# piotrmwojcik/GI-GS

Measured on AMD Instinct MI355X. Metric: train-step renders/sec (fwd+bwd, G-buffer+indirect) at 800x800; PSNR vs the CPU oracle, higher is better.
Workload: dtype f32; 1 GPU; C2 (configs[1] TensoIR lego stand-in): 300k surface Gaussians, 800x800, SH deg 2, GI step=16 start=8 delta=0.0625; P=300000, N=640000, M=9, hip_graphs=on, fused_glue=on, gi_march=proj, rasterizer=whole step = 2 hand-captured hipGraphs (fwd, bwd), asynchronous binning

## Files before the change

### gi-gs_amd/csrc/api.hip

```cpp
#include <cstdarg>
#include <cstdio>
#include <cstdlib>
#include <cstring>
#include <map>
#include <algorithm>
#include <new>
#include <mutex>
#include <vector>

#include "../../include/gigs_hip.h"
#include "gigs_common.h"

namespace {

thread_local char g_err[512] = "";

int fail(int code, const char* fmt, ...) {
  va_list ap;
  va_start(ap, fmt);
  vsnprintf(g_err, sizeof(g_err), fmt, ap);
  va_end(ap);
  return code;
}

// ... 110 lines not shown
  hipEventCreate(&e);
  return e;
}

struct StageScope {
  hipStream_t s;
  int stage;
  bool on;
  hipEvent_t a, b;
  StageScope(int stage_, hipStream_t s_) : s(s_), stage(stage_), on(false) {
    std::lock_guard<std::mutex> lk(g_prof_mu);
    if (!g_prof_on) return;
    on = true;
    a = prof_event();
    b = prof_event();
    hipEventRecord(a, s);
  }
  ~StageScope() {
    if (!on) return;
    hipEventRecord(b, s);
    std::lock_guard<std::mutex> lk(g_prof_mu);
    g_prof_recs.push_back({stage, a, b});
  }
};

}

namespace gigs {
const Options& default_options() {
  static const Options o = options_from_env();
  return o;
}
const Ctx& default_ctx() {
  static const Ctx c = {default_options(), 0u, nullptr, nullptr, 0, nullptr, nullptr};
  return c;
}
}

extern "C" {
__attribute__((visibility("hidden"))) const gigs::Options* gigs_internal_options(const gigs_ctx* ctx) { return &ctx_of(ctx).opt; }
__attribute__((visibility("hidden"))) int gigs_internal_fail(int code, const char* msg) { return fail(code, "%s", msg); }
__attribute__((visibility("hidden"))) void gigs_internal_stage_begin(int stage, void* stream, void** token) {
  *token = new StageScope(stage, (hipStream_t)stream);
}
__attribute__((visibility("hidden"))) void gigs_internal_stage_end(void* token) { delete (StageScope*)token; }
}

extern "C" {

const char* gigs_last_error(void) { return g_err; }
const char* gigs_build_arch(void) { return "gfx950"; }

size_t gigs_required_geom(int P) {
  if (P < 0) { fail(GIGS_ERR_INVALID, "P < 0"); return 0; }
  return gigs::required_bytes<gigs::GeomState>((size_t)P, scan_size_cached(P));
}
size_t gigs_required_image(int width, int height) {
  const size_t N = (size_t)width * height;
  const size_t T = (size_t)((width + GIGS_BLOCK_X - 1) / GIGS_BLOCK_X) * ((height + GIGS_BLOCK_Y - 1) / GIGS_BLOCK_Y);
  return gigs::required_bytes<gigs::ImageState>(N, T);
}
size_t gigs_required_binning(int R) {
  if (R < 0) { fail(GIGS_ERR_INVALID, "R < 0"); return 0; }
  return gigs::required_bytes<gigs::BinningState>((size_t)R, sort_size_cached(R));
}

long long gigs_geom_offset(int P, int which) {
// ... 47 lines not shown
  if (!ctx) return fail(GIGS_ERR_INVALID, "gigs_ctx_set_options: the default context is immutable, create one");
  if (!in || in->struct_bytes < (int)sizeof(gigs_options)) return fail(GIGS_ERR_INVALID, "gigs_ctx_set_options: set struct_bytes = sizeof(gigs_options)");
  if (in->gi_march != 0 && in->gi_march != 4) return fail(GIGS_ERR_INVALID, "gi_march must be 0 (exact) or 4 (proj)");
  if (in->gi_tile_log2w < 0 || in->gi_tile_log2w > 6) return fail(GIGS_ERR_INVALID, "gi_tile_log2w must be 0..6");
  if (in->long_lists < -1 || in->long_lists > 1) return fail(GIGS_ERR_INVALID, "long_lists must be -1, 0 or 1");
  if (in->bucket_target < 256 || in->bucket_max_mean < 0 || in->bin_bands < 0 || in->bin_bands > 64)
    return fail(GIGS_ERR_INVALID, "bucket_target >= 256, bucket_max_mean >= 0, 0 <= bin_bands <= 64");
  if (in->spec_max8 < 0 || in->spec_max16 < in->spec_max8) return fail(GIGS_ERR_INVALID, "0 <= spec_max8 <= spec_max16");
  if (in->shade_lds_floats < 0 || in->shade_bwd_blocks < 0) return fail(GIGS_ERR_INVALID, "shade_lds_floats, shade_bwd_blocks >= 0");
  if (in->spec_sparse_permille < 0 || in->spec_sparse_permille > 1000) return fail(GIGS_ERR_INVALID, "0 <= spec_sparse_permille <= 1000");
  gigs::Options& o = reinterpret_cast<gigs::Ctx*>(ctx)->opt;
  o.binning_legacy = in->binning_legacy != 0; o.bucket_max_mean = in->bucket_max_mean; o.long_lists = in->long_lists;
  o.bucket_target = in->bucket_target; o.bin_bands = in->bin_bands; o.blend_cull = in->blend_cull != 0; o.pre_bwd_sh_skip = in->pre_bwd_sh_skip != 0;
  o.gi_march = in->gi_march; o.gi_cert = in->gi_cert != 0; o.gi_interleave = in->gi_interleave != 0;
  o.gi_tile_log2w = in->gi_tile_log2w; o.gi_zero_rays = in->gi_zero_rays != 0; o.spec_max8 = in->spec_max8;
  o.spec_max16 = in->spec_max16; o.shade_lds_floats = in->shade_lds_floats; o.shade_bwd_blocks = in->shade_bwd_blocks;
  o.shade_bwd_rows = in->shade_bwd_rows != 0; o.spec_sparse = in->spec_sparse != 0; o.spec_sparse_permille = in->spec_sparse_permille;
  return 0;
}
int gigs_ctx_set_reuse_binning(gigs_ctx* ctx, int on) {
  if (!ctx) return fail(GIGS_ERR_INVALID, "gigs_ctx_set_reuse_binning: the default context is immutable, create one");
  reinterpret_cast<gigs::Ctx*>(ctx)->reuse_binning = on != 0;
  return 0;
}
int gigs_ctx_set_split_sh(gigs_ctx* ctx, const float* sh_rest) {
  if (!ctx) return fail(GIGS_ERR_INVALID, "gigs_ctx_set_split_sh: the default context is immutable, create one");
  reinterpret_cast<gigs::Ctx*>(ctx)->sh_rest = sh_rest;
  return 0;
}
int gigs_ctx_set_materials_only(gigs_ctx* ctx, void* violations) {
  if (!ctx) return fail(GIGS_ERR_INVALID, "gigs_ctx_set_materials_only: the default context is immutable, create one");
  reinterpret_cast<gigs::Ctx*>(ctx)->materials_only = reinterpret_cast<unsigned*>(violations);
  return 0;
}
int gigs_ctx_set_blend_begin_event(gigs_ctx* ctx, void* hip_event) {
  if (!ctx) return fail(GIGS_ERR_INVALID, "gigs_ctx_set_blend_begin_event: the default context is immutable, create one");
  reinterpret_cast<gigs::Ctx*>(ctx)->blend_begin_event = hip_event;
  return 0;
}

__global__ void __launch_bounds__(64) stream_delay_kernel(unsigned ticks) {
  const unsigned long long t0 = wall_clock64();
  while (wall_clock64() - t0 < (unsigned long long)ticks) __builtin_amdgcn_s_sleep(8);
}

int gigs_stream_delay(unsigned nanoseconds, void* stream) {
  if (nanoseconds == 0) return 0;
  const unsigned ns = nanoseconds > 1000000u ? 1000000u : nanoseconds;
  hipLaunchKernelGGL(stream_delay_kernel, dim3(1), dim3(64), 0, (hipStream_t)stream, (ns + 9u) / 10u);
  return hipGetLastError() == hipSuccess ? 0 : gigs_internal_fail(GIGS_ERR_HIP, "stream_delay: launch failed");
}

int gigs_ctx_set_async_binning(gigs_ctx* ctx, int r_capacity, unsigned* device_counters) {
  if (!ctx) return fail(GIGS_ERR_INVALID, "gigs_ctx_set_async_binning: the default context is immutable, create one");
  gigs::Ctx* c = reinterpret_cast<gigs::Ctx*>(ctx);
  c->async_capacity = r_capacity > 0 ? (unsigned)r_capacity : 0u;
  c->async_counters = r_capacity > 0 ? device_counters : nullptr;
  return 0;
}

void gigs_profile_begin(void) {
  std::lock_guard<std::mutex> lk(g_prof_mu);
  for (auto& r : g_prof_recs) { g_prof_pool.push_back(r.a); g_prof_pool.push_back(r.b); }
  g_prof_recs.clear();
  g_prof_on = true;
}
// ... 32 lines not shown
                 const float* rotations, const float* cov3D_precomp, const float* viewmatrix,
                 const float* projmatrix, const float* cam_pos, float tan_fovx, float tan_fovy,
                 int prefiltered, int argmax_depth, int inference, float* out_color,
                 float* out_opacity, float* out_depth, float* out_normal, float* out_normal_view,
                 float* out_pos, float* out_albedo, float* out_roughness, float* out_metallic,
                 int* radii, int debug, void* stream) {
  (void)prefiltered;
  hipStream_t s = (hipStream_t)stream;
  const gigs::Ctx& cx = ctx_of(ctx);
  const gigs::Options& opt = cx.opt;
  if (P < 0 || width <= 0 || height <= 0) return fail(GIGS_ERR_INVALID, "bad P / image size");
  if (P == 0) return 0;
  if (!geometryBuffer || !binningBuffer || !imageBuffer) return fail(GIGS_ERR_INVALID, "null allocation callback");
  if (!means3D || !opacities || !normal || !albedo || !roughness || !metallic || !viewmatrix ||
      !projmatrix || !cam_pos || !background)
    return fail(GIGS_ERR_INVALID, "null required input");
  if (!shs && !colors_precomp) return fail(GIGS_ERR_INVALID, "provide SHs or precomputed colors");
  if (!cov3D_precomp && (!scales || !rotations)) return fail(GIGS_ERR_INVALID, "provide scales+rotations or cov3D_precomp");
  if (!colors_precomp && (M <= 0 || (D + 1) * (D + 1) > M || D > 3)) return fail(GIGS_ERR_INVALID, "SH degree %d needs (D+1)^2 <= M=%d, D <= 3", D, M);

  gigs::FwdArgs a;
  a.P = P; a.D = D; a.M = M; a.W = width; a.H = height;
  a.gx = (width + GIGS_BLOCK_X - 1) / GIGS_BLOCK_X;
  a.gy = (height + GIGS_BLOCK_Y - 1) / GIGS_BLOCK_Y;
  a.focal_y = height / (2.0f * tan_fovy);
  a.focal_x = width / (2.0f * tan_fovx);
  a.tan_fovx = tan_fovx; a.tan_fovy = tan_fovy; a.scale_modifier = scale_modifier;
  a.means3D = means3D; a.shs = shs; a.colors_precomp = colors_precomp; a.opacities = opacities;
  a.normal = normal; a.albedo = albedo; a.roughness = roughness; a.metallic = metallic;
  a.scales = scales; a.rotations = rotations; a.cov3D_precomp = cov3D_precomp;
  a.viewmatrix = viewmatrix; a.projmatrix = projmatrix; a.cam_pos = cam_pos; a.background = background;
  a.argmax_depth = argmax_depth; a.inference = inference;
  a.shs_rest = (shs && !colors_precomp && M > 1) ? cx.sh_rest : nullptr;

  const size_t scan_sz = scan_size_cached(P);
  const size_t geom_bytes = gigs::required_bytes<gigs::GeomState>((size_t)P, scan_sz);
  char* geom_chunk = geometryBuffer(geom_bytes, geom_user);
  if (!geom_chunk) return fail(GIGS_ERR_ALLOC, "geometry buffer allocation of %zu bytes failed", geom_bytes);
  gigs::GeomState geom = gigs::GeomState::fromChunk(geom_chunk, (size_t)P, scan_sz);
  if (radii == nullptr) radii = geom.internal_radii;

  const size_t N = (size_t)width * height, T = (size_t)a.gx * a.gy;
  const size_t img_bytes = gigs::required_bytes<gigs::ImageState>(N, T);
  char* img_chunk = imageBuffer(img_bytes, image_user);
  if (!img_chunk) return fail(GIGS_ERR_ALLOC, "image buffer allocation of %zu bytes failed", img_bytes);
  gigs::ImageState img = gigs::ImageState::fromChunk(img_chunk, N, T);

  {
    StageScope sc(kPreprocess, s);
    gigs::launch_preprocess_fwd(a, geom, radii, s);
  }
  STAGE_CHECK("preprocess");
  int num_rendered = 0;
  gigs::BinningState bin;
  const unsigned async_cap = cx.async_capacity;
  const bool bucket = !opt.binning_legacy && T <= (size_t)gigs::kBinMaxTiles;
  if (async_cap > 0 && !bucket) return fail(GIGS_ERR_INVALID, "asynchronous binning needs the tile-bucketed path (options.binning_legacy = 0, <= %d tiles)", gigs::kBinMaxTiles);
  auto long_lists = [&](size_t est_mean) {
    if (opt.long_lists >= 0) return opt.long_lists == 1;
    return est_mean > (size_t)opt.bucket_max_mean;
  };
  bool dense = false;
  if (cx.reuse_binning) {
    if (async_cap == 0 || !bucket)
      return fail(GIGS_ERR_INVALID, "reuse_binning needs asynchronous binning (gigs_ctx_set_async_binning) on the tile-bucketed path");
    num_rendered = (int)async_cap;
// ... 74 lines not shown
  }
  STAGE_CHECK("identifyTileRanges");
  }
  if (void* ev = cx.blend_begin_event) HIP_TRY(hipEventRecord((hipEvent_t)ev, s));
  {
    StageScope sc(kBlendFwd, s);
    gigs::launch_blend_fwd(a, geom, bin, img, out_color, out_opacity, out_depth, out_normal,
                           out_normal_view, out_pos, out_albedo, out_roughness, out_metallic, opt.blend_cull,
                           (size_t)num_rendered, s, cx.reuse_binning != 0);
  }
  STAGE_CHECK("render");
  return num_rendered;
}

namespace {
struct LiteChunk { char* base; size_t bytes; };
char* lite_chunk_alloc(size_t n, void* user) {
  LiteChunk* c = static_cast<LiteChunk*>(user);
  return n <= c->bytes ? c->base : nullptr;
}
}

int gigs_lite_forward(gigs_ctx* ctx, gigs_alloc_fn geometryBuffer, void* geom_user, gigs_alloc_fn binningBuffer, void* binning_user,
                      gigs_alloc_fn imageBuffer, void* image_user, int P, int D, int M, const float* background, int width,
                      int height, const float* means3D, const float* shs, const float* colors_precomp, const float* opacities,
                      const float* scales, float scale_modifier, const float* rotations, const float* cov3D_precomp,
                      const float* viewmatrix, const float* projmatrix, const float* cam_pos, float tan_fovx, float tan_fovy,
                      int prefiltered, int argmax_depth, float* out_color, float* out_opacity, float* out_depth, int* radii,
                      int debug, void* stream) {
  if (P < 0 || width <= 0 || height <= 0) return fail(GIGS_ERR_INVALID, "bad P / image size");
  if (P == 0) return 0;
  if (!geometryBuffer || !binningBuffer || !imageBuffer) return fail(GIGS_ERR_INVALID, "null allocation callback");
  if (!out_color || !out_opacity || !out_depth) return fail(GIGS_ERR_INVALID, "null output");
  const size_t N = (size_t)width * height;
  const size_t geom_bytes = gigs_required_geom(P), img_bytes = gigs_required_image(width, height);
  const size_t geom_extra = 8 * (size_t)P * sizeof(float) + gigs::kAlign, img_extra = 14 * N * sizeof(float) + gigs::kAlign;
  char* gb = geometryBuffer(geom_bytes + geom_extra, geom_user);
  char* ib = imageBuffer(img_bytes + img_extra, image_user);
  if (!gb || !ib) return fail(GIGS_ERR_ALLOC, "lite_forward: scratch allocation failed");
  auto up = [](char* p) { return reinterpret_cast<char*>((reinterpret_cast<uintptr_t>(p) + gigs::kAlign - 1) & ~(uintptr_t)(gigs::kAlign - 1)); };
  float* zeros = reinterpret_cast<float*>(up(gb + geom_bytes));
  float* spare = reinterpret_cast<float*>(up(ib + img_bytes));
  gigs::launch_zero_words(reinterpret_cast<uint32_t*>(zeros), 8 * (size_t)P, (hipStream_t)stream);
  LiteChunk gc{gb, geom_bytes}, ic{ib, img_bytes};
  return gigs_forward(ctx, lite_chunk_alloc, &gc, binningBuffer, binning_user, lite_chunk_alloc, &ic, P, D, M, background, width, height,
                      means3D, shs, colors_precomp, opacities, zeros, zeros + 3 * (size_t)P, zeros + 6 * (size_t)P,
                      zeros + 7 * (size_t)P, scales, scale_modifier, rotations, cov3D_precomp, viewmatrix, projmatrix, cam_pos,
                      tan_fovx, tan_fovy, prefiltered, argmax_depth, 0, out_color, out_opacity, out_depth, spare, spare + 3 * N,
                      spare + 6 * N, spare + 9 * N, spare + 12 * N, spare + 13 * N, radii, debug, stream);
}

int gigs_backward(gigs_ctx* ctx, int P, int D, int M, int R, const float* background, int width, int height,
                  const float* means3D, const float* shs, const float* colors_precomp,
                  const float* normal, const float* albedo, const float* roughness,
                  const float* metallic, const float* scales, const float* rotations,
                  const float* cov3D_precomp, const float* viewmatrix, const float* projmatrix,
                  const float* cam_pos, const int* radii, float scale_modifier, float tan_fovx,
                  float tan_fovy, char* geom_buffer, char* binning_buffer, char* image_buffer,
                  const float* dL_dpix_depth, const float* dL_dpix, const float* dL_dpix_opacity,
                  const float* dL_dpix_normal, const float* dL_dpix_albedo,
                  const float* dL_dpix_roughness, const float* dL_dpix_metallic, float* dL_dmean2D,
                  float* dL_dconic, float* dL_ddepth, float* dL_dopacity, float* dL_dnormal,
                  float* dL_dalbedo, float* dL_droughness, float* dL_dmetallic, float* dL_dcolor,
                  float* dL_dmean3D, float* dL_dcov3D, float* dL_dsh, float* dL_dscale,
                  float* dL_drot, int debug, void* stream) {
  (void)normal; (void)albedo; (void)roughness; (void)metallic;
  hipStream_t s = (hipStream_t)stream;
  if (P == 0) return 0;
  if (P < 0 || R < 0 || width <= 0 || height <= 0) return fail(GIGS_ERR_INVALID, "bad sizes");
  if (!geom_buffer || !binning_buffer || !image_buffer) return fail(GIGS_ERR_INVALID, "null scratch buffer");
  unsigned* const materials_only = ctx_of(ctx).materials_only;
  if (ctx_of(ctx).sh_rest && shs && M > 1 && !materials_only)
    return fail(GIGS_ERR_INVALID, "a split-SH forward (gigs_ctx_set_split_sh) has a materials-only backward only");
  if (!dL_dmean2D || !dL_dalbedo || !dL_droughness || !dL_dmetallic)
    return fail(GIGS_ERR_INVALID, "null gradient output");
  if (!materials_only && (!dL_dopacity || !dL_dnormal || !dL_dcolor || !dL_dmean3D || !dL_dcov3D || !dL_dscale || !dL_drot ||
                          (shs && !dL_dsh)))
    return fail(GIGS_ERR_INVALID, "null gradient output");

  gigs::BwdArgs a;
  a.P = P; a.D = D; a.M = M; a.R = R; a.W = width; a.H = height;
  a.gx = (width + GIGS_BLOCK_X - 1) / GIGS_BLOCK_X;
  a.gy = (height + GIGS_BLOCK_Y - 1) / GIGS_BLOCK_Y;
  a.focal_y = height / (2.0f * tan_fovy);
  a.focal_x = width / (2.0f * tan_fovx);
  a.tan_fovx = tan_fovx; a.tan_fovy = tan_fovy; a.scale_modifier = scale_modifier;
  a.means3D = means3D; a.shs = shs; a.colors_precomp = colors_precomp; a.scales = scales;
  a.rotations = rotations; a.cov3D_precomp = cov3D_precomp; a.viewmatrix = viewmatrix;
  a.projmatrix = projmatrix; a.cam_pos = cam_pos; a.background = background;
  a.dL_dpix_depth = dL_dpix_depth; a.dL_dpix = dL_dpix; a.dL_dpix_opacity = dL_dpix_opacity;
  a.dL_dpix_normal = dL_dpix_normal; a.dL_dpix_albedo = dL_dpix_albedo;
  a.dL_dpix_roughness = dL_dpix_roughness; a.dL_dpix_metallic = dL_dpix_metallic;
  a.dL_dmean2D = dL_dmean2D; a.dL_dconic = dL_dconic; a.dL_ddepth = dL_ddepth;
  a.dL_dopacity = dL_dopacity; a.dL_dnormal = dL_dnormal; a.dL_dalbedo = dL_dalbedo;
  a.dL_droughness = dL_droughness; a.dL_dmetallic = dL_dmetallic; a.dL_dcolor = dL_dcolor;
  a.dL_dmean3D = dL_dmean3D; a.dL_dcov3D = dL_dcov3D; a.dL_dsh = dL_dsh; a.dL_dscale = dL_dscale;
  a.dL_drot = dL_drot;

  const size_t N = (size_t)width * height, T = (size_t)a.gx * a.gy;
  char* gp = geom_buffer;
  gigs::GeomState geom = gigs::GeomState::fromChunk(gp, (size_t)P, scan_size_cached(P));
  char* bp = binning_buffer;
  gigs::BinningState bin = gigs::BinningState::fromChunk(bp, (size_t)R, 0);
  char* ip = image_buffer;
  gigs::ImageState img = gigs::ImageState::fromChunk(ip, N, T);
  a.radii = radii ? radii : geom.internal_radii;

  {
// ... 3 lines not shown
  STAGE_CHECK("render backward");
  {
    StageScope sc(kPreprocessBwd, s);
    gigs::launch_preprocess_bwd(a, geom, ctx_of(ctx).opt.pre_bwd_sh_skip, s, materials_only);
  }
  STAGE_CHECK("preprocess backward");
  return 0;
}

int gigs_mark_visible(int P, const float* means3D, const float* viewmatrix,
                      const float* projmatrix, uint8_t* present, void* stream) {
  (void)projmatrix;
  if (P == 0) return 0;
  if (P < 0 || !means3D || !viewmatrix || !present) return fail(GIGS_ERR_INVALID, "bad argument");
  gigs::launch_mark_visible(P, means3D, viewmatrix, present, (hipStream_t)stream);
  HIP_TRY(hipGetLastError());
  return 0;
}

int gigs_depth_to_normal(int width, int height, float focal_x, float focal_y,
                         const float* viewmatrix, const float* depth, float* normal,
                         float* depth_pos, void* stream) {
  if (width <= 0 || height <= 0 || !viewmatrix || !depth || !normal || !depth_pos)
    return fail(GIGS_ERR_INVALID, "bad argument");
  StageScope sc(kDepthToNormal, (hipStream_t)stream);
  gigs::launch_depth_to_normal(width, height, focal_x, focal_y, viewmatrix, depth, normal, depth_pos, (hipStream_t)stream);
  HIP_TRY(hipGetLastError());
  return 0;
}

int gigs_derive_normal(int width, int height, float focal_x, float focal_y, const float* viewmatrix, const float* depth,
                       float sigma_color, float sigma_x, float sigma_y, float* normal_from_depth, float* depth_pos_filter,
                       void* stream) {
  if (width <= 1 || height <= 1 || !viewmatrix || !depth || !normal_from_depth || !depth_pos_filter)
    return fail(GIGS_ERR_INVALID, "derive_normal: bad argument (images must be larger than 1x1)");
  StageScope sc(kDepthToNormal, (hipStream_t)stream);
  gigs::launch_derive_normal_fused(width, height, focal_x, focal_y, viewmatrix, sigma_color, sigma_x, sigma_y, depth,
                                   normal_from_depth, depth_pos_filter, (hipStream_t)stream);
  HIP_TRY(hipGetLastError());
  return 0;
}

size_t gigs_gi_scratch_bytes(int width, int height) {
  if (width <= 0 || height <= 0) return 0;
  return gigs::gi_scratch_bytes(width, height);
}

int gigs_ssao_ex(gigs_ctx* ctx, int width, int height, float focal_x, float focal_y, float radius, float bias,
                 float thick, float delta, int step, int start, const float* normal_view,
                 const float* pos, float* occlusion, void* scratch, void* stream) {
  if (width <= 0 || height <= 0 || !normal_view || !pos || !occlusion) return fail(GIGS_ERR_INVALID, "bad argument");
  if (width >= (1 << 15) || height >= (1 << 15)) return fail(GIGS_ERR_INVALID, "image side above 32767 pixels");
  StageScope sc(kSsao, (hipStream_t)stream);
  const int rc = gigs::launch_ssao(ctx_of(ctx).opt, width, height, focal_x, focal_y, radius, bias, thick, delta, step, start,
                                   normal_view, pos, occlusion, scratch, (hipStream_t)stream);
  if (rc == -1) return fail(GIGS_ERR_INVALID, "delta=%g gives an unbounded or oversized ray set", (double)delta);
  if (rc) return fail(GIGS_ERR_HIP, "ray table upload failed");
  HIP_TRY(hipGetLastError());
  return 0;
}
int gigs_ssao(int width, int height, float focal_x, float focal_y, float radius, float bias,
              float thick, float delta, int step, int start, const float* normal_view,
              const float* pos, float* occlusion, void* stream) {
  return gigs_ssao_ex(nullptr, width, height, focal_x, focal_y, radius, bias, thick, delta, step, start, normal_view, pos,
                      occlusion, nullptr, stream);
}

int gigs_ssr_ex(gigs_ctx* ctx, int width, int height, float focal_x, float focal_y, float radius, float bias,
                float thick, float delta, int step, int start, const float* normal_view,
                const float* pos, const float* rgb, const float* albedo, const float* roughness,
                const float* metallic, const float* F0, float* color, float* abd, void* scratch, void* stream) {
  if (width <= 0 || height <= 0 || !normal_view || !pos || !rgb || !albedo || !metallic || !F0 || !color || !abd)
    return fail(GIGS_ERR_INVALID, "bad argument");
  if (width >= (1 << 15) || height >= (1 << 15)) return fail(GIGS_ERR_INVALID, "image side above 32767 pixels");
  StageScope sc(kSsr, (hipStream_t)stream);
  const int rc = gigs::launch_ssr(ctx_of(ctx).opt, width, height, focal_x, focal_y, radius, bias, thick, delta, step, start,
                                  normal_view, pos, rgb, albedo, roughness, metallic, F0, color, abd, scratch,
                                  (hipStream_t)stream);
  if (rc == -1) return fail(GIGS_ERR_INVALID, "delta=%g gives an unbounded or oversized ray set", (double)delta);
  if (rc) return fail(GIGS_ERR_HIP, "ray table upload failed");
  HIP_TRY(hipGetLastError());
  return 0;
}
int gigs_ssr_multi(gigs_ctx* ctx, int n_lights, int width, int height, float focal_x, float focal_y, float radius, float bias,
                   float thick, float delta, int step, int start, const float* normal_view, const float* pos, const float* rgb,
                   const float* albedo, const float* roughness, const float* metallic, const float* F0, float* color,
                   float* abd, void* scratch, void* stream) {
  if (n_lights < 1 || n_lights > GIGS_MAX_LIGHTS)
    return fail(GIGS_ERR_INVALID, "ssr_multi: n_lights=%d outside 1..%d", n_lights, GIGS_MAX_LIGHTS);
  if (width <= 0 || height <= 0 || !normal_view || !pos || !rgb || !albedo || !metallic || !F0 || !color || !abd)
    return fail(GIGS_ERR_INVALID, "bad argument");
  if (width >= (1 << 15) || height >= (1 << 15)) return fail(GIGS_ERR_INVALID, "image side above 32767 pixels");
  StageScope sc(kSsr, (hipStream_t)stream);
  (void)roughness;
  const int rc = gigs::launch_ssr_multi(ctx_of(ctx).opt, n_lights, width, height, focal_x, focal_y, radius, bias, thick, delta,
                                        step, start, normal_view, pos, rgb, albedo, metallic, F0, color, abd, scratch,
                                        (hipStream_t)stream);
  if (rc == -1) return fail(GIGS_ERR_INVALID, "delta=%g gives an unbounded or oversized ray set", (double)delta);
  if (rc) return fail(GIGS_ERR_HIP, "ray table upload failed");
  HIP_TRY(hipGetLastError());
  return 0;
}
int gigs_ssr_hits(gigs_ctx* ctx, int width, int height, float focal_x, float focal_y, float radius, float bias, float thick,
                  float delta, int step, int start, const float* normal_view, const float* pos, const float* rgb,
                  const float* albedo, const float* roughness, const float* metallic, const float* F0, float* color, float* abd,
                  int mode, unsigned* counts, const unsigned* offsets, void* entries, unsigned capacity, void* scratch,
                  void* stream) {
  if (width <= 0 || height <= 0 || !normal_view || !pos || !rgb || !albedo || !metallic || !F0 || !color || !abd)
    return fail(GIGS_ERR_INVALID, "bad argument");
  if (width >= (1 << 15) || height >= (1 << 15)) return fail(GIGS_ERR_INVALID, "image side above 32767 pixels");
  if ((mode != 1 && mode != 2) || (mode == 1 && !counts) || (mode == 2 && (!offsets || (!entries && capacity > 0))))
    return fail(GIGS_ERR_INVALID, "ssr_hits: mode 1 needs counts, mode 2 offsets and entries");
  StageScope sc(kSsr, (hipStream_t)stream);
  const int rc = gigs::launch_ssr(ctx_of(ctx).opt, width, height, focal_x, focal_y, radius, bias, thick, delta, step, start,
                                  normal_view, pos, rgb, albedo, roughness, metallic, F0, color, abd, scratch,
                                  (hipStream_t)stream, mode, counts, offsets, entries, capacity);
  if (rc == -1) return fail(GIGS_ERR_INVALID, "delta=%g gives an unbounded or oversized ray set", (double)delta);
  if (rc == -3) return fail(GIGS_ERR_INVALID, "ssr_hits: the hit list is recorded by the default march only (gi_march = proj, start < step)");
  if (rc) return fail(GIGS_ERR_HIP, "ray table upload failed");
  HIP_TRY(hipGetLastError());
  return 0;
}

int gigs_ssr_apply(int width, int height, float delta, const unsigned* offsets, const void* entries, const float* normal_view,
                   const float* pos, const float* rgb, const float* albedo, const float* metallic, const float* F0,
                   float* color, float* abd, void* stream) {
  if (width <= 0 || height <= 0 || !offsets || !normal_view || !pos || !rgb || !albedo || !metallic || !F0 || !color || !abd)
    return fail(GIGS_ERR_INVALID, "bad argument");
  StageScope sc(kSsr, (hipStream_t)stream);
  const int rc = gigs::launch_ssr_apply(width, height, delta, offsets, entries, normal_view, pos, rgb, albedo, metallic, F0, color,
                                        abd, (hipStream_t)stream);
  if (rc == -1) return fail(GIGS_ERR_INVALID, "delta=%g gives an unbounded or oversized ray set", (double)delta);
  if (rc) return fail(GIGS_ERR_HIP, "ray table upload failed");
  HIP_TRY(hipGetLastError());
  return 0;
}

size_t gigs_ssr_apply_multi_scratch_bytes(int n_lights, int width, int height) {
  if (n_lights < 1 || n_lights > GIGS_MAX_LIGHTS || width <= 0 || height <= 0) return 0;
  return gigs::ssr_apply_multi_scratch_bytes(n_lights, width, height);
}
int gigs_ssr_apply_multi(int n_lights, int width, int height, float delta, const unsigned* offsets, const void* entries,
                         const float* normal_view, const float* pos, const float* rgb, const float* albedo,
                         const float* metallic, const float* F0, float* color, float* abd, void* scratch, void* stream) {
  if (n_lights < 1 || n_lights > GIGS_MAX_LIGHTS)
    return fail(GIGS_ERR_INVALID, "ssr_apply_multi: n_lights=%d outside 1..%d", n_lights, GIGS_MAX_LIGHTS);
  if (width <= 0 || height <= 0 || !offsets || !normal_view || !pos || !rgb || !albedo || !metallic || !F0 || !color || !abd)
    return fail(GIGS_ERR_INVALID, "bad argument");
  if ((size_t)offsets % 16 != 0 || (size_t)scratch % 16 != 0)
// ... 65 lines not shown
```

### gi-gs_amd/csrc/blend.hip

```cpp
#include <cstdlib>
#include "gigs_common.h"

namespace gigs {

typedef float f32x2 __attribute__((ext_vector_type(2)));

__device__ __forceinline__ unsigned long long ballot64(bool p) { return __builtin_amdgcn_ballot_w64(p); }

constexpr int kLongTile = 2048;

template <int kCtrl, int kRowMask = 0xf, int kBankMask = 0xf>
__device__ __forceinline__ float dpp_mov0(float v) {
  return __int_as_float(__builtin_amdgcn_update_dpp(0, __float_as_int(v), kCtrl, kRowMask, kBankMask, false));
}
template <int N>
__device__ __forceinline__ void wave_sum_n(float* v);
template <>
__device__ __forceinline__ void wave_sum_n<1>(float* v) {
  asm("s_nop 4\n\t"
      "v_add_f32_dpp %0, %0, %0 quad_perm:[1,0,3,2] row_mask:0xf bank_mask:0xf bound_ctrl:1\n\t"
      "s_nop 1\n\t"
      "v_add_f32_dpp %0, %0, %0 quad_perm:[2,3,0,1] row_mask:0xf bank_mask:0xf bound_ctrl:1\n\t"
      "s_nop 1\n\t"
      "v_add_f32_dpp %0, %0, %0 row_ror:4 row_mask:0xf bank_mask:0xf bound_ctrl:1\n\t"
// ... 257 lines not shown
        const float4 r4 = sw[4 * 64 + bit];
        const f32x2 w2 = {weight, weight};
        C01 += f32x2{r2.x, r2.y} * w2; C2P0 += f32x2{r2.z, r2.w} * w2;
        N01 += f32x2{r3.x, r3.y} * w2; N2P1 += f32x2{r3.z, r3.w} * w2;
        A01 += f32x2{r4.x, r4.y} * w2; A2P2 += f32x2{r4.z, r4.w} * w2;
        RM += f32x2{r0.z, r0.w} * w2;
        O += weight;
        if (argmax_depth) {
          if (weight > max_weight) {
            e0 = r2.w; e1 = r3.w; e2 = r4.w;
            max_weight = weight;
          }
        }
        T = test_T;
        last_contributor = (uint32_t)(base + bit + 1);
      }
    }
    wave_done = ballot64(!done) == 0ull;
    __builtin_amdgcn_wave_barrier();
    if (valid) hit[base + lane] = (uint8_t)((hits >> lane) & 1ull);
  }
  for (int i = base + lane; i < n; i += 64) hit[i] = 0;

  const float C0 = C01.x, C1 = C01.y, C2 = C2P0.x, P0 = C2P0.y, N0 = N01.x, N1 = N01.y, N2 = N2P1.x, P1 = N2P1.y;
  const float A0 = A01.x, A1 = A01.y, A2 = A2P2.x, P2 = A2P2.y, Rr = RM.x, Mm = RM.y;
  if (inside) {
    const size_t HW = (size_t)H * W;
    final_T[pix_id] = T;
    n_contrib[pix_id] = last_contributor;
    const v3 nv = normalize3(xform_vec_4x3({N0, N1, N2}, viewmatrix));
    o.normal_view[pix_id] = nv.x;
    o.normal_view[HW + pix_id] = nv.y;
    o.normal_view[2 * HW + pix_id] = nv.z;
    o.color[pix_id] = C0 + T * bg_color[0];
    o.color[HW + pix_id] = C1 + T * bg_color[1];
    o.color[2 * HW + pix_id] = C2 + T * bg_color[2];
    o.normal[pix_id] = N0; o.normal[HW + pix_id] = N1; o.normal[2 * HW + pix_id] = N2;
    o.albedo[pix_id] = A0; o.albedo[HW + pix_id] = A1; o.albedo[2 * HW + pix_id] = A2;
    o.roughness[pix_id] = inference ? (Rr + T) : Rr;
    o.metallic[pix_id] = Mm;
    if ((double)O > 1e-6) {
      o.depth[pix_id] = argmax_depth ? e2 : P2 / O;
      o.pos[pix_id] = argmax_depth ? e0 : P0 / O;
      o.pos[HW + pix_id] = argmax_depth ? e1 : P1 / O;
      o.pos[2 * HW + pix_id] = argmax_depth ? e2 : P2 / O;
    } else {
      o.depth[pix_id] = 0.0f;
      o.pos[pix_id] = 0.0f;
      o.pos[HW + pix_id] = 0.0f;
      o.pos[2 * HW + pix_id] = 0.0f;
    }
    o.opacity[pix_id] = O;
  }
}

void launch_blend_fwd(const FwdArgs& a, const GeomState& g, const BinningState& b,
                      const ImageState& im, float* out_color, float* out_opacity,
                      float* out_depth, float* out_normal, float* out_normal_view, float* out_pos,
                      float* out_albedo, float* out_roughness, float* out_metallic, int cull, size_t hit_stride,
                      hipStream_t s, bool reused_lists) {
  BlendOut o{out_color, out_opacity, out_depth, out_normal, out_normal_view,
             out_pos, out_albedo, out_roughness, out_metallic};
  hipLaunchKernelGGL(blend_fwd_kernel, dim3(a.gx * a.gy), dim3(GIGS_TILE), 0, s, a.W, a.H, a.gx,
                     im.ranges, b.point_list, g.brec, a.viewmatrix, a.background, im.n_contrib,
                     im.final_T, o, a.argmax_depth, a.inference, b.hit_mask, hit_stride, cull, im.tile_order,
                     reused_lists ? (const uint32_t*)im.bin_counters : (const uint32_t*)nullptr,
                     make_uint2((unsigned)a.P, (unsigned)hit_stride));
}

struct BlendGradIn {
  const float *depth, *color, *opacity, *normal, *albedo, *roughness, *metallic;
};

__global__ void __launch_bounds__(GIGS_TILE)
blend_bwd_kernel(int W, int H, unsigned gx, const uint2* __restrict__ ranges,
                 const uint32_t* __restrict__ point_list, const float4* __restrict__ brec,
                 const float* __restrict__ bg_color, const float* __restrict__ final_Ts,
                 const uint32_t* __restrict__ n_contrib, BlendGradIn gi, float* __restrict__ grec,
                 const uint8_t* __restrict__ hit_mask, size_t hit_stride, const uint32_t* __restrict__ tile_order) {
  __shared__ float4 s_rec[4][3 * 64];
  __shared__ __align__(16) float s_sum[4][2][GIGS_GREC];

  const unsigned tile = tile_order[blockIdx.x];
  const unsigned ty = tile / gx, tx = tile - ty * gx;
  const int tid = threadIdx.x, wave = tid >> 6, lane = tid & 63;
// ... 224 lines not shown
```

### gi-gs_amd/csrc/gi.hip

```cpp
#include <cmath>
#include <cstdlib>
#include <cstring>
#include <mutex>
#include <type_traits>
#include <vector>

#include "gigs_common.h"
#include "pixel_ops.h"

namespace gigs {

constexpr float kPiF = 3.14159265358979323846f;

__device__ __forceinline__ v3 get_position(int x, int y, float cx, float cy, float fx, float fy,
                                           float depth) {
  const v3 dir = {((float)x - cx) / fx, ((float)y - cy) / fy, 1.0f};
  return dir * depth;
}

__global__ void __launch_bounds__(256)
depth_to_normal_kernel(int W, int H, float fx, float fy, const float* __restrict__ vm,
                       const float* __restrict__ depth_map, float* __restrict__ normal_out,
                       float* __restrict__ depth_pos) {
  const int x = blockIdx.x * 16 + (threadIdx.x & 15);
// ... 1063 lines not shown
    }
#pragma unroll
    for (int o = 32; o > 0; o >>= 1) {
      mn = fminf(mn, __shfl_xor(mn, o));
      mx = fmaxf(mx, __shfl_xor(mx, o));
    }
  } else {
    mn = -__builtin_inff();
    mx = __builtin_inff();
  }
  if (threadIdx.x == 0) {
    float t_hi = (mx - ck.lo_k) / (1.0f - 0x1p-16f);
    t_hi = t_hi + fabsf(t_hi) * 0x1p-20f + 1e-30f;
    float t_lo = (mn - ck.hi_k) / (1.0f + 0x1p-16f);
    t_lo = t_lo - fabsf(t_lo) * 0x1p-20f - 1e-30f;
    if (!(mx == mx) || !(mn == mn)) { t_hi = __builtin_inff(); t_lo = -__builtin_inff(); }
    tab[(size_t)by * (bw + 1) + bx] = make_float2(t_lo, t_hi);
  }
}

constexpr int kCertMaxBytes = 40 * 1024;
static size_t cert_table_bytes(int W, int H, int sh) {
  return (size_t)(((W + (1 << sh) - 1) >> sh) + 2) * (((H + (1 << sh) - 1) >> sh) + 2) * sizeof(float2);
}
static int cert_shift_for(int W, int H) {
  for (int sh = 4; sh <= 6; sh++)
    if (cert_table_bytes(W, H, sh) <= (size_t)kCertMaxBytes) return sh;
  return 0;
}
size_t gi_scratch_bytes(int W, int H) {
  const int sh = cert_shift_for(W, H);
  return sh ? cert_table_bytes(W, H, sh) : 0;
}
static size_t prepare_cert(const Options& o, GiParams& p, int mode, const float* pos, void* scratch, hipStream_t s) {
  p.cert_shift = p.cert_w = p.cert_h = 0;
  p.cert_d0 = cert_consts(p.bias, p.thick).d0;
  if (!scratch || mode != 4 || !o.gi_cert) return 0;
  const int sh = cert_shift_for(p.W, p.H);
  if (!sh) return 0;
  p.cert_shift = sh;
  p.cert_w = (p.W + (1 << sh) - 1) >> sh;
  p.cert_h = (p.H + (1 << sh) - 1) >> sh;
  hipLaunchKernelGGL(gi_minmax_kernel, dim3(p.cert_w + 1, p.cert_h + 1), dim3(64), 0, s, p.W, p.H, sh, p.cert_w, p.cert_h,
                     cert_consts(p.bias, p.thick), pos + 2 * (size_t)p.H * p.W, (float2*)scratch);
  return cert_table_bytes(p.W, p.H, sh);
}

#ifndef GIGS_GI_DEFAULT_MODE
#define GIGS_GI_DEFAULT_MODE 4
#endif
static int gi_march_mode(const Options& o, int step, int start) {
  int mode = (o.gi_march == 0 || o.gi_march == 4) ? o.gi_march : GIGS_GI_DEFAULT_MODE;
  if (step - start > 64 - kGiGroup || step <= 0) mode = 0;
  return mode;
}
template <March kMarch> using MarchTag = std::integral_constant<March, kMarch>;
template <class F>
static void gi_dispatch_march(int mode, bool pow2, size_t cert, F&& f) {
  if (mode == 4) {
    if (cert) f(MarchTag<March::kProjCert>{}, cert);
    else f(MarchTag<March::kProj>{}, (size_t)0);
  } else {
    if (pow2) f(MarchTag<March::kExactPow2>{}, (size_t)0);
    else f(MarchTag<March::kExact>{}, (size_t)0);
  }
}
static dim3 gi_grid(const GiParams& p) {
  const int tw = 1 << p.tile_log2w, th = 64 >> p.tile_log2w;
  return dim3((p.W + tw - 1) / tw, (p.H + th - 1) / th);
}

int launch_ssao(const Options& o, int W, int H, float fx, float fy, float radius, float bias, float thick,
                float delta, int step, int start, const float* normal, const float* pos,
                float* occlusion, void* scratch, hipStream_t s) {
  RayTable t;
  const int rc = get_ray_table(delta, s, t);
  if (rc) return rc;
// ... 38 lines not shown
                           const float* F0, float* color, float* abd, void* scratch, hipStream_t s) {
  RayTable t;
  const int rc = get_ray_table(delta, s, t);
  if (rc) return rc;
  const size_t HW = (size_t)W * H, plane = 3 * HW;
  const dim3 grid((unsigned)((HW + 255) / 256));
  auto pass = [&](auto tag, int l0) {
    constexpr int kLights = decltype(tag)::value;
    const float* src = rgb + l0 * plane;
    if constexpr (kLights > 1) {
      hipLaunchKernelGGL(ssr_pack_kernel<kLights>, grid, dim3(256), 0, s, HW, src, (float4*)scratch);
      src = (const float*)scratch;
    }
    hipLaunchKernelGGL(ssr_apply_kernel<kLights>, grid, dim3(256), 0, s, W, H, t.nrays, t.dev, offsets, (const uint2*)entries,
                       normal, pos, src, albedo, metallic, F0, color + l0 * plane, abd + l0 * plane);
  };
  for (int l0 = 0; l0 < n_lights;) {
    const int n = n_lights - l0;
    int took;
    if (kSsrApplyLights == 8 && n >= 8) { pass(std::integral_constant<int, 8>{}, l0); took = 8; }
    else if (n >= 4) { pass(std::integral_constant<int, 4>{}, l0); took = 4; }
    else if (n == 3) { pass(std::integral_constant<int, 3>{}, l0); took = 3; }
    else if (n == 2) { pass(std::integral_constant<int, 2>{}, l0); took = 2; }
    else { pass(std::integral_constant<int, 1>{}, l0); took = 1; }
    l0 += took;
  }
  return 0;
}

int launch_ssr(const Options& o, int W, int H, float fx, float fy, float radius, float bias, float thick,
               float delta, int step, int start, const float* normal, const float* pos,
               const float* rgb, const float* albedo, const float* ,
               const float* metallic, const float* F0, float* color, float* abd, void* scratch, hipStream_t s,
               int hits_mode, unsigned* hit_counts, const unsigned* hit_offsets, void* hit_entries, unsigned hit_capacity) {
  RayTable t;
  const int rc = get_ray_table(delta, s, t);
  if (rc) return rc;
  bool pow2;
  GiParams p = make_params(o, W, H, fx, fy, radius, bias, thick, step, start, t,  true, pow2);
  if (W >= (1 << 15) || H >= (1 << 15)) return -2;
  const dim3 grid = gi_grid(p);
  const int mode = gi_march_mode(o, step, start);
  const size_t cert = (start < step) ? prepare_cert(o, p, mode, pos, scratch, s) : 0;
  const float2* tab = (const float2*)scratch;
  const SsrHits hits = {hit_counts, hit_offsets, (uint2*)hit_entries, hit_capacity};
  if (hits_mode != 0 && (mode != 4 || (hits_mode != 1 && hits_mode != 2) || !(start < step))) return -3;
  gi_dispatch_march(mode, pow2, cert, [&](auto m, size_t lds) {
    constexpr March kMarch = decltype(m)::value;
    auto launch = [&](auto kernel) {
      hipLaunchKernelGGL(kernel, grid, dim3(256), lds, s, p, t.dev, normal, pos, rgb, albedo, metallic, F0, color, abd, tab, hits);
    };
    if constexpr (march_is_proj(kMarch)) {
      if (hits_mode == 1) return launch(ssr_kernel<kMarch, 1>);
      if (hits_mode == 2) return launch(ssr_kernel<kMarch, 2>);
    }
    launch(ssr_kernel<kMarch>);
  });
  return 0;
}

template <int kLights>
static void launch_ssr_chunk(const GiParams& p, dim3 grid, int mode, bool pow2, size_t cert, const float2* tab,
                             const float4* rays, const float* normal, const float* pos, const float* rgb, const float* albedo,
                             const float* metallic, const float* F0, float* color, float* abd, hipStream_t s) {
  const SsrHits hits = {nullptr, nullptr, nullptr, 0};
  gi_dispatch_march(mode, pow2, cert, [&](auto m, size_t lds) {
    hipLaunchKernelGGL((ssr_kernel<decltype(m)::value, 0, kLights>), grid, dim3(256), lds, s, p, rays, normal, pos, rgb, albedo,
                       metallic, F0, color, abd, tab, hits);
  });
}

int launch_ssr_multi(const Options& o, int n_lights, int W, int H, float fx, float fy, float radius, float bias, float thick,
                     float delta, int step, int start, const float* normal, const float* pos, const float* rgb,
                     const float* albedo, const float* metallic, const float* F0, float* color, float* abd, void* scratch,
                     hipStream_t s) {
  RayTable t;
  const int rc = get_ray_table(delta, s, t);
  if (rc) return rc;
  bool pow2;
  GiParams p = make_params(o, W, H, fx, fy, radius, bias, thick, step, start, t,  true, pow2);
  if (W >= (1 << 15) || H >= (1 << 15)) return -2;
  const dim3 grid = gi_grid(p);
  const int mode = gi_march_mode(o, step, start);
  const size_t cert = (start < step) ? prepare_cert(o, p, mode, pos, scratch, s) : 0;
  const float2* tab = (const float2*)scratch;
  const size_t plane = (size_t)3 * W * H;
  for (int l0 = 0; l0 < n_lights; l0 += kSsrMaxLights) {
    const int n = min(kSsrMaxLights, n_lights - l0);
    const float* c_rgb = rgb + l0 * plane;
    float *c_color = color + l0 * plane, *c_abd = abd + l0 * plane;
    static_assert(kSsrMaxLights == 4, "one case per chunk size");
    switch (n) {
      case 1: launch_ssr_chunk<1>(p, grid, mode, pow2, cert, tab, t.dev, normal, pos, c_rgb, albedo, metallic, F0, c_color, c_abd, s); break;
      case 2: launch_ssr_chunk<2>(p, grid, mode, pow2, cert, tab, t.dev, normal, pos, c_rgb, albedo, metallic, F0, c_color, c_abd, s); break;
      case 3: launch_ssr_chunk<3>(p, grid, mode, pow2, cert, tab, t.dev, normal, pos, c_rgb, albedo, metallic, F0, c_color, c_abd, s); break;
      default: launch_ssr_chunk<4>(p, grid, mode, pow2, cert, tab, t.dev, normal, pos, c_rgb, albedo, metallic, F0, c_color, c_abd, s);
    }
  }
  return 0;
}

__device__ __forceinline__ bool load_taps(const float* __restrict__ src, int H, int W, int y, int x,
                                          float* v) {
  bool has_nan = false;
  int k = 0;
#pragma unroll
  for (int dy = -1; dy <= 1; dy++)
#pragma unroll
    for (int dx = -1; dx <= 1; dx++) {
      const int yy = y + dy, xx = x + dx;
      const float t = (yy < 0 || yy >= H || xx < 0 || xx >= W) ? 0.0f : src[(size_t)yy * W + xx];
      has_nan |= (t != t);
      v[k++] = t;
    }
  return has_nan;
}

// ... 79 lines not shown
#pragma unroll
      for (int c = 0; c < C; c++) num[c] += tap[c] * k;
      den += k;
    }
#pragma unroll
  for (int c = 0; c < C; c++) out[c * HW + (size_t)y * W + x] = num[c] / den;
}

void launch_bilateral3x3(int C, int H, int W, float sigma_color, float sx, float sy,
                         const float* in, float* out, hipStream_t s) {
  BilatK kk;
  auto k1d = [](float sigma, float* k) {
    float sum = 0;
    for (int i = 0; i < 3; i++) {
      const float xv = (float)(i - 1);
      k[i] = expf(-(xv * xv) / (2.0f * sigma * sigma));
      sum += k[i];
    }
    for (int i = 0; i < 3; i++) k[i] /= sum;
  };
  k1d(sy, kk.ky);
  k1d(sx, kk.kx);
  kk.color_scale = -0.5f / (sigma_color * sigma_color);
  dim3 grid((W + 63) / 64, (H + 3) / 4, 1);
  if (C == 1) hipLaunchKernelGGL(bilateral3x3_kernel<1>, grid, dim3(256), 0, s, H, W, kk, in, out);
  else if (C == 3) hipLaunchKernelGGL(bilateral3x3_kernel<3>, grid, dim3(256), 0, s, H, W, kk, in, out);
}

#ifndef GIGS_DN_H
#define GIGS_DN_H 4
#endif
constexpr int kDnW = 32, kDnH = GIGS_DN_H, kDnThreads = kDnW * kDnH;

__global__ void __launch_bounds__(kDnThreads)
derive_normal_fused_kernel(int W, int H, float fx, float fy, const float* __restrict__ vm, BilatK kk,
                           const float* __restrict__ depth_raw, float* __restrict__ normal_out,
                           float* __restrict__ pos_filter_out) {
  __shared__ float s_d[kDnH + 8][kDnW + 8];
  __shared__ float s_f[kDnH + 6][kDnW + 6];
  __shared__ float s_n[3][kDnH + 2][kDnW + 2];
  __shared__ float s_p[3][kDnH + 2][kDnW + 2];
  const int x0 = blockIdx.x * kDnW, y0 = blockIdx.y * kDnH;
  const size_t HW = (size_t)H * W;

  for (int i = threadIdx.x; i < (kDnH + 8) * (kDnW + 8); i += kDnThreads) {
    const int ty = i / (kDnW + 8), tx = i - ty * (kDnW + 8);
    const int gx = x0 - 4 + tx, gy = y0 - 4 + ty;
    s_d[ty][tx] = (gx < 0 || gx >= W || gy < 0 || gy >= H) ? 0.0f : depth_raw[(size_t)gy * W + gx];
  }
  __syncthreads();

  for (int i = threadIdx.x; i < (kDnH + 6) * (kDnW + 6); i += kDnThreads) {
    const int ty = i / (kDnW + 6), tx = i - ty * (kDnW + 6);
    const int gx = x0 - 3 + tx, gy = y0 - 3 + ty;
    float r = 0.0f;
    if (!(gx < 0 || gx >= W || gy < 0 || gy >= H)) {
      float v[9];
      bool has_nan = false;
      int k = 0;
#pragma unroll
      for (int dy = -1; dy <= 1; dy++)
#pragma unroll
        for (int dx = -1; dx <= 1; dx++) {
          const float t = s_d[ty + 1 + dy][tx + 1 + dx];
          has_nan |= (t != t);
          v[k++] = t;
        }
      r = has_nan ? __builtin_nanf("") : median9(v);
    }
    s_f[ty][tx] = r;
  }
  __syncthreads();

  for (int i = threadIdx.x; i < (kDnH + 2) * (kDnW + 2); i += kDnThreads) {
    const int ty = i / (kDnW + 2), tx = i - ty * (kDnW + 2);
    const int x = x0 - 1 + tx, y = y0 - 1 + ty;
    v3 nrm = {0.0f, 0.0f, 0.0f}, pos = {0.0f, 0.0f, 0.0f};
    if (!(x < 0 || x >= W || y < 0 || y >= H) && !(x <= 0 || x >= W - 1 || y <= 0 || y >= H - 1)) {
#define DP(dx, dy) s_f[ty + 2 + (dy)][tx + 2 + (dx)]
      const float depth_thresh = 0.01f;
      const float depth = DP(0, 0);
      const float cx = float(W) / 2.0f, cy = float(H) / 2.0f;
      pos = get_position(x, y, cx, cy, fx, fy, depth);
      bool ok = !(depth < depth_thresh);
      const int pad = 2;
      for (int dx = -pad; ok && dx < pad + 1; ++dx) {
        if (x + dx < 0 || x + dx > W - 1) { ok = false; break; }
        for (int dy = -pad; dy < pad + 1; ++dy) {
          if (y + dy < 0 || y + dy > H - 1) { ok = false; break; }
          if (DP(dx, dy) < depth_thresh) { ok = false; break; }
        }
      }
      if (ok) {
        const v3 pos_aa = get_position(x, y - 1, cx, cy, fx, fy, DP(0, -1));
        const v3 pos_bb = get_position(x + 1, y, cx, cy, fx, fy, DP(1, 0));
        const v3 pos_cc = get_position(x, y + 1, cx, cy, fx, fy, DP(0, 1));
        const v3 pos_dd = get_position(x - 1, y, cx, cy, fx, fy, DP(-1, 0));
        const v3 pos_ab = get_position(x + 1, y - 1, cx, cy, fx, fy, DP(1, -1));
        const v3 pos_bc = get_position(x + 1, y + 1, cx, cy, fx, fy, DP(1, 1));
        const v3 pos_cd = get_position(x - 1, y + 1, cx, cy, fx, fy, DP(-1, 1));
        const v3 pos_da = get_position(x - 1, y - 1, cx, cy, fx, fy, DP(-1, -1));
        const v3 edge_a = pos_da - pos_ab, edge_b = pos_ab - pos_bc, edge_c = pos_bc - pos_cd, edge_d = pos_cd - pos_da;
        const v3 edge_ac = pos_cc - pos_aa, edge_bd = pos_dd - pos_bb;
        const v3 edge_cdab = pos_ab - pos_cd, edge_bcad = pos_da - pos_bc;
        const v3 n1 = cross3(edge_a, edge_d), n2 = cross3(edge_d, edge_c), n3 = cross3(edge_c, edge_b);
        const v3 n4 = cross3(edge_b, edge_a), n5 = cross3(edge_ac, edge_bd), n6 = cross3(edge_bcad, edge_cdab);
        const v3 sum = normalize3(n1) + normalize3(n2) + normalize3(n3) + normalize3(n4) + normalize3(n5) + normalize3(n6);
        const float inv6 = 1.0f / 6.0f;
        const v3 normal = sum * inv6;
        nrm = {vm[0] * normal.x + vm[1] * normal.y + vm[2] * normal.z, vm[4] * normal.x + vm[5] * normal.y + vm[6] * normal.z,
               vm[8] * normal.x + vm[9] * normal.y + vm[10] * normal.z};
      }
#undef DP
    }
    s_n[0][ty][tx] = nrm.x; s_n[1][ty][tx] = nrm.y; s_n[2][ty][tx] = nrm.z;
    s_p[0][ty][tx] = pos.x; s_p[1][ty][tx] = pos.y; s_p[2][ty][tx] = pos.z;
  }
  __syncthreads();

  const int lx = threadIdx.x & (kDnW - 1), ly = threadIdx.x / kDnW;
  const int x = x0 + lx, y = y0 + ly;
  if (x >= W || y >= H) return;
  const size_t p = (size_t)y * W + x;
  {
    float ctr[3], num[3] = {0.0f, 0.0f, 0.0f};
#pragma unroll
    for (int c = 0; c < 3; c++) ctr[c] = s_n[c][ly + 1][lx + 1];
    float den = 0.0f;
#pragma unroll
    for (int dy = -1; dy <= 1; dy++)
#pragma unroll
      for (int dx = -1; dx <= 1; dx++) {
        int yy = y + dy, xx = x + dx;
        yy = yy < 0 ? -yy : (yy >= H ? 2 * H - 2 - yy : yy);
        xx = xx < 0 ? -xx : (xx >= W ? 2 * W - 2 - xx : xx);
        float tap[3], dist = 0.0f;
#pragma unroll
        for (int c = 0; c < 3; c++) {
          tap[c] = s_n[c][yy - y0 + 1][xx - x0 + 1];
          dist += fabsf(tap[c] - ctr[c]);
        }
        const float color_k = expf(kk.color_scale * (dist * dist));
        const float k = (kk.ky[dy + 1] * kk.kx[dx + 1]) * color_k;
#pragma unroll
        for (int c = 0; c < 3; c++) num[c] += tap[c] * k;
        den += k;
      }
#pragma unroll
    for (int c = 0; c < 3; c++) normal_out[c * HW + p] = num[c] / den;
  }
#pragma unroll
  for (int c = 0; c < 3; c++) {
    float v[9];
    bool has_nan = false;
    int k = 0;
#pragma unroll
    for (int dy = -1; dy <= 1; dy++)
#pragma unroll
      for (int dx = -1; dx <= 1; dx++) {
        const float t = s_p[c][ly + 1 + dy][lx + 1 + dx];
        has_nan |= (t != t);
        v[k++] = t;
      }
    pos_filter_out[c * HW + p] = has_nan ? __builtin_nanf("") : median9(v);
  }
}

void launch_derive_normal_fused(int W, int H, float fx, float fy, const float* viewmatrix, float sigma_color, float sx,
                                float sy, const float* depth_raw, float* normal_out, float* pos_filter_out, hipStream_t s) {
  BilatK kk;
  auto k1d = [](float sigma, float* k) {
    float sum = 0;
    for (int i = 0; i < 3; i++) {
      const float xv = (float)(i - 1);
      k[i] = expf(-(xv * xv) / (2.0f * sigma * sigma));
      sum += k[i];
    }
    for (int i = 0; i < 3; i++) k[i] /= sum;
  };
  k1d(sy, kk.ky);
  k1d(sx, kk.kx);
  kk.color_scale = -0.5f / (sigma_color * sigma_color);
  hipLaunchKernelGGL(derive_normal_fused_kernel, dim3((W + kDnW - 1) / kDnW, (H + kDnH - 1) / kDnH), dim3(kDnThreads), 0, s, W, H, fx,
                     fy, viewmatrix, kk, depth_raw, normal_out, pos_filter_out);
}

__global__ void __launch_bounds__(256)
selftest_div2_kernel(int n, const float* __restrict__ nx, const float* __restrict__ ny,
                     const float* __restrict__ d, float* __restrict__ out_fast, float* __restrict__ out_ref,
                     int* __restrict__ out_round) {
  const int i = blockIdx.x * 256 + threadIdx.x;
  if (i >= n) return;
  const float big = fmaxf(fmaxf(fabsf(nx[i]), fabsf(ny[i])), fabsf(d[i]));
  const float small = fminf(fabsf(nx[i]), fabsf(ny[i]));
  const f32x2 q = div2_exact(f32x2{nx[i], ny[i]}, d[i], big < 0x1p60f && small > 0x1p-60f);
  out_fast[2 * i] = q.x;
  out_fast[2 * i + 1] = q.y;
  out_ref[2 * i] = nx[i] / d[i];
  out_ref[2 * i + 1] = ny[i] / d[i];
  out_round[2 * i] = round_to_int(nx[i]);
  out_round[2 * i + 1] = f2i(roundf(nx[i]));
}

__global__ void __launch_bounds__(256) selftest_round_kernel(unsigned long long* __restrict__ bad) {
  unsigned long long local = 0;
  for (unsigned long long b = (unsigned long long)blockIdx.x * 256 + threadIdx.x; b < (1ull << 32);
       b += (unsigned long long)gridDim.x * 256) {
    const float t = __uint_as_float((unsigned)b);
    const int a = f2i(roundf(t)), r = round_pix(t);
    const bool same = a == r || (a < 0 && r < 0) || (a >= 32767 && r >= 32767);
    local += same ? 0 : 1;
  }
  if (local) atomicAdd(bad, local);
}

}

// ... 15 lines not shown
```

### gi-gs_amd/csrc/gigs_common.h

```cpp
#pragma once
#include <hip/hip_runtime.h>
#include <stdint.h>

#define GIGS_BLOCK_X 16
#define GIGS_BLOCK_Y 16
#define GIGS_TILE (GIGS_BLOCK_X * GIGS_BLOCK_Y)
#define GIGS_BREC_F4 5
#define GIGS_GREC 20

namespace gigs {

struct v3 { float x, y, z; };
struct v4 { float x, y, z, w; };

__device__ __forceinline__ v3 operator+(v3 a, v3 b) { return {a.x + b.x, a.y + b.y, a.z + b.z}; }
__device__ __forceinline__ v3 operator-(v3 a, v3 b) { return {a.x - b.x, a.y - b.y, a.z - b.z}; }
__device__ __forceinline__ v3 operator*(v3 a, float s) { return {a.x * s, a.y * s, a.z * s}; }
__device__ __forceinline__ float dot3(v3 a, v3 b) { return a.x * b.x + a.y * b.y + a.z * b.z; }
__device__ __forceinline__ v3 cross3(v3 a, v3 b) {
  return {a.y * b.z - a.z * b.y, a.z * b.x - a.x * b.z, a.x * b.y - a.y * b.x};
}
__device__ __forceinline__ v3 normalize3(v3 v) {
  float inv = 1.0f / sqrtf(dot3(v, v));
  return v * inv;
// ... 163 lines not shown
  char* p = nullptr;
  S::fromChunk(p, a...);
  return reinterpret_cast<size_t>(p) + kAlign;
}

struct Options {
  int binning_legacy;
  int bucket_max_mean;
  int long_lists;
  int bucket_target;
  int bin_bands;
  int blend_cull;
  int pre_bwd_sh_skip;
  int gi_march;
  int gi_cert;
  int gi_interleave;
  int gi_tile_log2w;
  int gi_zero_rays;
  int spec_max8, spec_max16;
  int shade_lds_floats;
  int shade_bwd_blocks;
  int shade_bwd_rows;
  int spec_sparse;
  int spec_sparse_permille;
};
struct Ctx {
  Options opt;
  unsigned async_capacity;
  unsigned* async_counters;
  void* blend_begin_event;
  int reuse_binning;
  unsigned* materials_only;
  const float* sh_rest;
};
const Options& default_options();
const Ctx& default_ctx();

struct FwdArgs {
  int P, D, M, W, H;
  unsigned gx, gy;
  float focal_x, focal_y, tan_fovx, tan_fovy, scale_modifier;
  const float *means3D, *shs, *colors_precomp, *opacities, *normal, *albedo, *roughness,
      *metallic, *scales, *rotations, *cov3D_precomp, *viewmatrix, *projmatrix, *cam_pos,
      *background;
  int argmax_depth, inference;
  const float* shs_rest;
};

void launch_preprocess_fwd(const FwdArgs& a, const GeomState& g, int* radii, hipStream_t s);
void launch_zero_words(uint32_t* p, size_t n, hipStream_t s);
void launch_bin_count(int P, const int* radii, unsigned gx, unsigned gy, const GeomState& g, const ImageState& img, hipStream_t s);
void launch_bin_prefix(int P, int T, unsigned capacity, const ImageState& img, unsigned* user_counters, hipStream_t s);
void launch_bin_scatter(int P, const int* radii, unsigned gx, unsigned gy, unsigned capacity, unsigned bands, const GeomState& g,
                        const BinningState& b, const ImageState& img, hipStream_t s);
int launch_bin_sort(int T, int P, bool long_lists, unsigned bucket_target, unsigned capacity, const BinningState& b, const ImageState& img,
                    hipStream_t s);
size_t long_space_bytes(size_t T, size_t R);
void launch_mark_visible(int P, const float* means3D, const float* viewmatrix, uint8_t* present,
                         hipStream_t s);
hipError_t scan_tiles(const GeomState& g, int P, hipStream_t s);
size_t scan_temp_bytes(int P);
size_t sort_temp_bytes(int R);
void launch_duplicate(int P, const int* radii, unsigned gx, unsigned gy, const GeomState& g,
                      const BinningState& b, hipStream_t s);
hipError_t sort_pairs(const BinningState& b, int R, int end_bit, hipStream_t s);
void launch_tile_ranges(int R, const BinningState& b, uint2* ranges, hipStream_t s);
void launch_tile_order(int T, const uint2* ranges, uint32_t* tile_order, hipStream_t s);
void launch_blend_fwd(const FwdArgs& a, const GeomState& g, const BinningState& b,
                      const ImageState& im, float* out_color, float* out_opacity,
                      float* out_depth, float* out_normal, float* out_normal_view, float* out_pos,
                      float* out_albedo, float* out_roughness, float* out_metallic, int cull, size_t hit_stride,
                      hipStream_t s, bool reused_lists = false);

struct BwdArgs {
  int P, D, M, R, W, H;
  unsigned gx, gy;
  float focal_x, focal_y, tan_fovx, tan_fovy, scale_modifier;
  const float *means3D, *shs, *colors_precomp, *scales, *rotations, *cov3D_precomp, *viewmatrix,
      *projmatrix, *cam_pos, *background;
  const int* radii;
  const float *dL_dpix_depth, *dL_dpix, *dL_dpix_opacity, *dL_dpix_normal, *dL_dpix_albedo,
      *dL_dpix_roughness, *dL_dpix_metallic;
  float *dL_dmean2D, *dL_dconic, *dL_ddepth, *dL_dopacity, *dL_dnormal, *dL_dalbedo,
      *dL_droughness, *dL_dmetallic, *dL_dcolor, *dL_dmean3D, *dL_dcov3D, *dL_dsh, *dL_dscale,
      *dL_drot;
};
void launch_blend_bwd(const BwdArgs& a, const GeomState& g, const BinningState& b,
                      const ImageState& im, hipStream_t s);
void launch_preprocess_bwd(const BwdArgs& a, const GeomState& g, int sh_skip, hipStream_t s, unsigned* materials_only = nullptr);

void launch_depth_to_normal(int W, int H, float fx, float fy, const float* viewmatrix,
                            const float* depth, float* normal, float* depth_pos, hipStream_t s);
int launch_ssao(const Options& o, int W, int H, float fx, float fy, float radius, float bias, float thick,
                float delta, int step, int start, const float* normal, const float* pos,
                float* occlusion, void* scratch, hipStream_t s);
size_t gi_scratch_bytes(int W, int H);
int launch_ssr(const Options& o, int W, int H, float fx, float fy, float radius, float bias, float thick,
               float delta, int step, int start, const float* normal, const float* pos,
               const float* rgb, const float* albedo, const float* roughness,
               const float* metallic, const float* F0, float* color, float* abd, void* scratch, hipStream_t s,
               int hits_mode = 0, unsigned* hit_counts = nullptr, const unsigned* hit_offsets = nullptr,
               void* hit_entries = nullptr, unsigned hit_capacity = 0);
int launch_ssr_multi(const Options& o, int n_lights, int W, int H, float fx, float fy, float radius, float bias, float thick,
                     float delta, int step, int start, const float* normal, const float* pos, const float* rgb,
                     const float* albedo, const float* metallic, const float* F0, float* color, float* abd, void* scratch,
                     hipStream_t s);
int launch_ssr_apply(int W, int H, float delta, const unsigned* offsets, const void* entries, const float* normal,
                     const float* pos, const float* rgb, const float* albedo, const float* metallic, const float* F0,
                     float* color, float* abd, hipStream_t s);
int launch_ssr_apply_multi(int n_lights, int W, int H, float delta, const unsigned* offsets, const void* entries,
                           const float* normal, const float* pos, const float* rgb, const float* albedo, const float* metallic,
                           const float* F0, float* color, float* abd, void* scratch, hipStream_t s);
size_t ssr_apply_multi_scratch_bytes(int n_lights, int W, int H);
void launch_median3x3(int C, int H, int W, const float* in, float* out, hipStream_t s);
void launch_median3x3_bwd(int C, int H, int W, const float* in, const float* gout, float* gin,
                          hipStream_t s);
void launch_bilateral3x3(int C, int H, int W, float sigma_color, float sx, float sy,
                         const float* in, float* out, hipStream_t s);
void launch_derive_normal_fused(int W, int H, float fx, float fy, const float* viewmatrix, float sigma_color, float sx,
                                float sy, const float* depth_raw, float* normal_out, float* pos_filter_out, hipStream_t s);

}
```

### gi-gs_amd/csrc/preprocess.hip

```cpp
#include "gigs_common.h"

namespace gigs {

#define SHC0 0.28209479177387814f
#define SHC1 0.4886025119029199f
#define SHC2_0 1.0925484305920792f
#define SHC2_1 -1.0925484305920792f
#define SHC2_2 0.31539156525252005f
#define SHC2_3 -1.0925484305920792f
#define SHC2_4 0.5462742152960396f
#define SHC3_0 -0.5900435899266435f
#define SHC3_1 2.890611442640554f
#define SHC3_2 -0.4570457994644658f
#define SHC3_3 0.3731763325901154f
#define SHC3_4 -0.4570457994644658f
#define SHC3_5 1.445305721320277f
#define SHC3_6 -0.5900435899266435f

constexpr int kPreBlock = 256;

__host__ __device__ __forceinline__ int sh_stride(int M) { return (3 * M) | 1; }

__device__ __forceinline__ void stage_sh(const float* __restrict__ shs, float* sh_lds,
                                         size_t first, int nG, int M) {
// ... 58 lines not shown

__device__ __forceinline__ Cov2D cov2d(v3 mean, float fx, float fy, float tan_fovx, float tan_fovy,
                                       const float* cov3D, const float* vm) {
  Cov2D s;
  v3 t = xform_point_4x3(mean, vm);
  s.limx = 1.3f * tan_fovx;
  s.limy = 1.3f * tan_fovy;
  s.txtz = t.x / t.z;
  s.tytz = t.y / t.z;
  t.x = fminf(s.limx, fmaxf(-s.limx, s.txtz)) * t.z;
  t.y = fminf(s.limy, fmaxf(-s.limy, s.tytz)) * t.z;
  s.t = t;
  m3 J = make_m3(fx / t.z, 0.0f, -(fx * t.x) / (t.z * t.z), 0.0f, fy / t.z,
                 -(fy * t.y) / (t.z * t.z), 0.0f, 0.0f, 0.0f);
  s.Wm = make_m3(vm[0], vm[4], vm[8], vm[1], vm[5], vm[9], vm[2], vm[6], vm[10]);
  s.T = mul3(s.Wm, J);
  s.Vrk = make_m3(cov3D[0], cov3D[1], cov3D[2], cov3D[1], cov3D[3], cov3D[4], cov3D[2], cov3D[4],
                  cov3D[5]);
  s.cov = mul3(mul3(transpose3(s.T), transpose3(s.Vrk)), s.T);
  return s;
}

__device__ __forceinline__ m3 quat_to_R(float r, float x, float y, float z) {
  return make_m3(1.f - 2.f * (y * y + z * z), 2.f * (x * y - r * z), 2.f * (x * z + r * y),
                 2.f * (x * y + r * z), 1.f - 2.f * (x * x + z * z), 2.f * (y * z - r * x),
                 2.f * (x * z - r * y), 2.f * (y * z + r * x), 1.f - 2.f * (x * x + y * y));
}

__global__ void __launch_bounds__(kPreBlock)
preprocess_fwd_kernel(FwdArgs a, GeomState g, int* __restrict__ radii) {
  extern __shared__ __align__(16) float sh_lds[];
  const int idx = blockIdx.x * kPreBlock + threadIdx.x;
  const int P = a.P;
  const bool use_sh = (a.colors_precomp == nullptr);
  if (use_sh) {
    const size_t first = (size_t)blockIdx.x * kPreBlock;
    const int nG = min(kPreBlock, P - (int)first);
    if (a.shs_rest) stage_sh_split(a.shs, a.shs_rest, sh_lds, first, nG, a.M);
    else stage_sh(a.shs, sh_lds, first, nG, a.M);
    __syncthreads();
  }
  if (idx >= P) return;

  radii[idx] = 0;
  g.tiles_touched[idx] = 0;
  {
    float4* gz = reinterpret_cast<float4*>(g.grec + (size_t)idx * GIGS_GREC);
    const float4 z4 = make_float4(0.0f, 0.0f, 0.0f, 0.0f);
    gz[0] = z4; gz[1] = z4; gz[2] = z4; gz[3] = z4; gz[4] = z4;
  }

  const v3 p_orig = ld3(a.means3D + 3 * (size_t)idx);
  const v3 p_view = xform_point_4x3(p_orig, a.viewmatrix);
  if (p_view.z <= 0.2f) return;

  const v4 p_hom = xform_point_4x4(p_orig, a.projmatrix);
  const float p_w = 1.0f / (p_hom.w + 0.0000001f);
  const float p_proj_x = p_hom.x * p_w, p_proj_y = p_hom.y * p_w;

  float c3[6];
  if (a.cov3D_precomp != nullptr) {
#pragma unroll
    for (int i = 0; i < 6; i++) c3[i] = a.cov3D_precomp[6 * (size_t)idx + i];
  } else {
    const v3 sc = ld3(a.scales + 3 * (size_t)idx);
    const float4 q = reinterpret_cast<const float4*>(a.rotations)[idx];
    m3 S = make_m3(1, 0, 0, 0, 1, 0, 0, 0, 1);
// ... 36 lines not shown
    const float* cp = a.cam_pos;
    v3 dir = {p_orig.x - cp[0], p_orig.y - cp[1], p_orig.z - cp[2]};
    const float len = sqrtf(dir.x * dir.x + dir.y * dir.y + dir.z * dir.z);
    dir = {dir.x / len, dir.y / len, dir.z / len};
    v3 result = SH(0) * SHC0;
    if (a.D > 0) {
      const float x = dir.x, y = dir.y, z = dir.z;
      result = result - SH(1) * (SHC1 * y) + SH(2) * (SHC1 * z) - SH(3) * (SHC1 * x);
      if (a.D > 1) {
        const float xx = x * x, yy = y * y, zz = z * z;
        const float xy = x * y, yz = y * z, xz = x * z;
        result = result + SH(4) * (SHC2_0 * xy) + SH(5) * (SHC2_1 * yz) +
                 SH(6) * (SHC2_2 * (2.0f * zz - xx - yy)) + SH(7) * (SHC2_3 * xz) +
                 SH(8) * (SHC2_4 * (xx - yy));
        if (a.D > 2) {
          result = result + SH(9) * (SHC3_0 * y * (3.0f * xx - yy)) + SH(10) * (SHC3_1 * xy * z) +
                   SH(11) * (SHC3_2 * y * (4.0f * zz - xx - yy)) +
                   SH(12) * (SHC3_3 * z * (2.0f * zz - 3.0f * xx - 3.0f * yy)) +
                   SH(13) * (SHC3_4 * x * (4.0f * zz - xx - yy)) + SH(14) * (SHC3_5 * z * (xx - yy)) +
                   SH(15) * (SHC3_6 * x * (xx - 3.0f * yy));
        }
      }
    }
#undef SH
    result = {result.x + 0.5f, result.y + 0.5f, result.z + 0.5f};
    g.clamped[3 * (size_t)idx + 0] = (result.x < 0);
    g.clamped[3 * (size_t)idx + 1] = (result.y < 0);
    g.clamped[3 * (size_t)idx + 2] = (result.z < 0);
    col = {result.x < 0.0f ? 0.0f : result.x, result.y < 0.0f ? 0.0f : result.y,
           result.z < 0.0f ? 0.0f : result.z};
    g.rgb[3 * (size_t)idx + 0] = col.x;
    g.rgb[3 * (size_t)idx + 1] = col.y;
    g.rgb[3 * (size_t)idx + 2] = col.z;
  } else {
    col = ld3(a.colors_precomp + 3 * (size_t)idx);
  }

  const float opac = a.opacities[idx];
  g.depths[idx] = p_view.z;
  radii[idx] = f2i(my_radius);
  reinterpret_cast<float2*>(g.means2D)[idx] = make_float2(pix, piy);
  reinterpret_cast<float4*>(g.conic_opacity)[idx] = make_float4(conx, cony, conz, opac);
  g.pos_view[3 * (size_t)idx + 0] = p_view.x;
  g.pos_view[3 * (size_t)idx + 1] = p_view.y;
  g.pos_view[3 * (size_t)idx + 2] = p_view.z;
  g.tiles_touched[idx] = (maxy - miny) * (maxx - minx);

  const v3 nrm = ld3(a.normal + 3 * (size_t)idx);
  const v3 alb = ld3(a.albedo + 3 * (size_t)idx);
  float4* rec = g.brec + (size_t)idx * GIGS_BREC_F4;
  rec[0] = make_float4(pix, piy, a.roughness[idx], a.metallic[idx]);
  rec[1] = make_float4(conx, cony, conz, opac);
  rec[2] = make_float4(col.x, col.y, col.z, p_view.x);
  rec[3] = make_float4(nrm.x, nrm.y, nrm.z, p_view.y);
  rec[4] = make_float4(alb.x, alb.y, alb.z, p_view.z);
}

void launch_preprocess_fwd(const FwdArgs& a, const GeomState& g, int* radii, hipStream_t s) {
  const int blocks = (a.P + kPreBlock - 1) / kPreBlock;
  const size_t lds = a.colors_precomp ? 0 : (size_t)kPreBlock * sh_stride(a.M) * sizeof(float);
  hipLaunchKernelGGL(preprocess_fwd_kernel, dim3(blocks), dim3(kPreBlock), lds, s, a, g, radii);
}

__global__ void __launch_bounds__(256)
mark_visible_kernel(int P, const float* __restrict__ means3D, const float* __restrict__ vm,
                    uint8_t* __restrict__ present) {
  const int idx = blockIdx.x * 256 + threadIdx.x;
  if (idx >= P) return;
  const v3 p = ld3(means3D + 3 * (size_t)idx);
  const v3 pv = xform_point_4x3(p, vm);
  present[idx] = !(pv.z <= 0.2f);
}

void launch_mark_visible(int P, const float* means3D, const float* viewmatrix, uint8_t* present,
                         hipStream_t s) {
  hipLaunchKernelGGL(mark_visible_kernel, dim3((P + 255) / 256), dim3(256), 0, s, P, means3D,
                     viewmatrix, present);
}

__device__ __forceinline__ v3 dnormvdv3(v3 v, v3 dv) {
  const float sum2 = v.x * v.x + v.y * v.y + v.z * v.z;
  const float invsum32 = 1.0f / sqrtf(sum2 * sum2 * sum2);
  v3 r;
  r.x = ((+sum2 - v.x * v.x) * dv.x - v.y * v.x * dv.y - v.z * v.x * dv.z) * invsum32;
  r.y = (-v.x * v.y * dv.x + (sum2 - v.y * v.y) * dv.y - v.z * v.y * dv.z) * invsum32;
  r.z = (-v.x * v.z * dv.x - v.y * v.z * dv.y + (sum2 - v.z * v.z) * dv.z) * invsum32;
  return r;
}

__global__ void __launch_bounds__(kPreBlock)
preprocess_bwd_kernel(BwdArgs a, GeomState g, int sh_always, unsigned* __restrict__ materials_only) {
  extern __shared__ __align__(16) float sh_lds[];
  const int idx = blockIdx.x * kPreBlock + threadIdx.x;
// ... 271 lines not shown
```

### gi-gs_amd/diff_gaussian_rasterization/__init__.py

```python
from __future__ import annotations

import ctypes as C
import contextlib
import os
import sys
import threading
from types import SimpleNamespace
from typing import NamedTuple, Optional, Tuple

import torch
import torch.nn as nn

_PKG_ROOT = os.path.dirname(os.path.dirname(os.path.abspath(__file__)))
if _PKG_ROOT not in sys.path:
    sys.path.insert(0, _PKG_ROOT)

import gigs_lib
from gigs_lib import GigsError

_lib = gigs_lib.lib()

NUM_CHANNELS = 3


# ... 5 lines not shown
    image_height: int
    image_width: int
    tanfovx: float
    tanfovy: float
    radius: float
    bias: float
    thick: float
    delta: float
    step: int
    start: int
    bg: torch.Tensor
    scale_modifier: float
    viewmatrix: torch.Tensor
    projmatrix: torch.Tensor
    sh_degree: int
    campos: torch.Tensor
    prefiltered: bool
    debug: bool
    inference: bool
    argmax_depth: bool


def _stream() -> int:
    return torch.cuda.current_stream().cuda_stream


class _Scopes(threading.local):
    pool = None
    after_blend = None
    prefetch_events = None
    grad_sink = None
    async_ = None
    view = None


_st = _Scopes()


class OutputPool:

    def __init__(self):
        self.buffers, self.counts = {}, {}

    def __enter__(self):
        self.counts = {}
        self._prev, _st.pool = _st.pool, self
        return self

    def __exit__(self, *exc):
        _st.pool = self._prev
        return False

    def get(self, tag, shape, dtype, device):
        k = self.counts.get(tag, 0)
        self.counts[tag] = k + 1
        key = (tag, k, tuple(shape), dtype, str(device))
        t = self.buffers.get(key)
        if t is None:
            t = self.buffers[key] = torch.empty(tuple(shape), dtype=dtype, device=device)
        return t




class after_blend:

# ... 307 lines not shown
            dL_dmeans3D, dL_dcov3D, dL_dsh, dL_dscales, dL_drotations)


def _mark_visible(means3D, viewmatrix, projmatrix):
    _need_gpu(means3D, "means3D")
    P = int(means3D.size(0))
    present = torch.zeros((P,), dtype=torch.bool, device=means3D.device)
    if P != 0:
        m, k0 = _fptr(means3D, "means3D")
        v, k1 = _fptr(viewmatrix, "viewmatrix")
        pr, k2 = _fptr(projmatrix, "projmatrix")
        with torch.cuda.device(means3D.device):
            gigs_lib.check(_lib.gigs_mark_visible(P, m, v, pr, present.data_ptr(), _stream()), "mark_visible")
    return present


def _depth_to_normal(width, height, focal_x, focal_y, viewmatrix, depthMap):
    _need_gpu(depthMap, "depthMap")
    dev = depthMap.device
    normalMap = _new("normal_from_depth", (3, height, width), dev)
    depth_pos = _new("depth_pos", (3, height, width), dev)
    v, k0 = _fptr(viewmatrix, "viewmatrix")
    d, k1 = _fptr(depthMap, "depthMap")
    with torch.cuda.device(dev):
        gigs_lib.check(_lib.gigs_depth_to_normal(int(width), int(height), float(focal_x), float(focal_y), v, d,
                                                 normalMap.data_ptr(), depth_pos.data_ptr(), _stream()),
                       "depth_to_normal")
    return normalMap, depth_pos


def _SSAO(width, height, focal_x, focal_y, radius, bias, thick, delta, step, start, out_normal, out_pos):
    _need_gpu(out_normal, "out_normal")
    dev = out_normal.device
    if _st.view is not None:
        slot, mode = _st.view
        if slot.occlusion is None or tuple(slot.occlusion.shape) != (1, height, width):
            if mode != "record":
                raise RuntimeError("view_cache('replay'): the slot holds no occlusion plane of this size")
            slot.occlusion = torch.empty((1, height, width), dtype=torch.float32, device=dev)
        if mode != "record":
            return slot.occlusion
        occlusion = slot.occlusion
    else:
        occlusion = _new("occlusion", (1, height, width), dev)
    n, k0 = _fptr(out_normal, "out_normal")
    ps, k1 = _fptr(out_pos, "out_pos")
    scratch = _gi_scratch(int(width), int(height), dev)
    with torch.cuda.device(dev):
        gigs_lib.check(_lib.gigs_ssao_ex(gigs_lib.ctx_ptr(), int(width), int(height), float(focal_x), float(focal_y), float(radius),
                                         float(bias), float(thick), float(delta), int(step), int(start), n, ps,
                                         occlusion.data_ptr(), None if scratch is None else scratch.data_ptr(), _stream()),
                       "SSAO")
    return occlusion


def _gi_scratch(width: int, height: int, dev):
    nbytes = int(_lib.gigs_gi_scratch_bytes(width, height))
    return torch.empty(nbytes, dtype=torch.uint8, device=dev) if nbytes else None


def _SSR(width, height, focal_x, focal_y, radius, bias, thick, delta, step, start, out_normal, out_pos,
         out_rgb, out_albedo, out_roughness, out_metallic, out_F0):
    _need_gpu(out_roughness, "out_roughness")
    dev = out_roughness.device
    color = torch.empty((3, height, width), dtype=torch.float32, device=dev)
    abd = torch.empty((3, height, width), dtype=torch.float32, device=dev)
    ptrs, keep = [], []
    for t, name in ((out_normal, "out_normal"), (out_pos, "out_pos"), (out_rgb, "out_rgb"),
                    (out_albedo, "out_albedo"), (out_roughness, "out_roughness"),
                    (out_metallic, "out_metallic"), (out_F0, "out_F0")):
        ptr, k = _fptr(t, name)
        ptrs.append(ptr)
        keep.append(k)
    scratch = _gi_scratch(int(width), int(height), dev)
    sp = None if scratch is None else scratch.data_ptr()
    W, H = int(width), int(height)
    a = (W, H, float(focal_x), float(focal_y), float(radius), float(bias), float(thick), float(delta), int(step), int(start))
    hit_list = (_st.view is not None and gigs_lib.current().option("gi_march") == 4 and int(start) < int(step)
                and os.environ.get("GIGS_SSR_HIT_LIST", "1") == "1")
    with torch.cuda.device(dev):
        if hit_list and _st.view[1] == "replay" and _st.view[0].ssr_loaded:
            slot = _st.view[0]
            normal_p, pos_p, rgb_p, albedo_p, _rough_p, metallic_p, F0_p = ptrs
            gigs_lib.check(_lib.gigs_ssr_apply(W, H, float(delta), slot.ssr_offsets.data_ptr(), slot.ssr_entries.data_ptr(),
                                               normal_p, pos_p, rgb_p, albedo_p, metallic_p, F0_p, color.data_ptr(),
                                               abd.data_ptr(), _stream()), "SSR (gather)")
        elif hit_list and _st.view[1] == "replay_rec":
            slot = _st.view[0]
            capturing = torch.cuda.is_current_stream_capturing()
            if not capturing:
                slot.ssr_prepare(W * H)
            if slot.ssr_offsets is None:
                raise RuntimeError("view_cache('replay_rec'): the hit-list buffers must be sized by an eager step before a capture")
            gigs_lib.check(_lib.gigs_ssr_hits(gigs_lib.ctx_ptr(), *a, *ptrs, color.data_ptr(), abd.data_ptr(), 1,
                                              slot.ssr_counts.data_ptr(), None, None, 0, sp, _stream()), "SSR (count)")
            torch.cumsum(slot.ssr_counts, 0, dtype=torch.int32, out=slot.ssr_offsets[1:])
            if not capturing:
                slot.ssr_prepare(W * H, total_hint=int(slot.ssr_offsets[-1]))
            gigs_lib.check(_lib.gigs_ssr_hits(gigs_lib.ctx_ptr(), *a, *ptrs, color.data_ptr(), abd.data_ptr(), 2, None,
                                              slot.ssr_offsets.data_ptr(), slot.ssr_entries.data_ptr(), slot.ssr_capacity, sp,
                                              _stream()), "SSR (fill)")
            slot.ssr_total_host.copy_(slot.ssr_offsets[-1:], non_blocking=True)
        else:
            gigs_lib.check(_lib.gigs_ssr_ex(gigs_lib.ctx_ptr(), *a, *ptrs, color.data_ptr(), abd.data_ptr(), sp, _stream()), "SSR")
    return color, abd


def _SSR_BACKWARD(*_args):
    raise NotImplementedError(
        "SSR_BACKWARD is unreachable in the reference (commented out at __init__.py:666-670); "
        "Gaussian_SSR's backward is grad_albedo = grad_out * abd")


# ... 157 lines not shown
        try:
            if raster_settings.debug:
                cpu_args = cpu_deep_copy_tuple(args)
                try:
                    res = _C.rasterize_gaussians_backward(*args)
                except Exception as ex:
                    torch.save(cpu_args, "snapshot_bw.dump")
                    print("\nAn error occured in backward. Writing snapshot_bw.dump for debugging.\n")
                    raise ex
            else:
                res = _rasterize_gaussians_backward(*args, image_size=(raster_settings.image_height,
                                                                       raster_settings.image_width))
        finally:
            _st.grad_sink = prev_sink
        (grad_means2D, grad_colors_precomp, grad_opacities, grad_normal, grad_albedo, grad_roughness,
         grad_metallic, grad_means3D, grad_cov3Ds_precomp, grad_sh, grad_scales, grad_rotations) = res
        return (grad_means3D, grad_means2D, grad_opacities, grad_normal, grad_albedo, grad_roughness,
                grad_metallic, grad_sh, grad_colors_precomp, grad_scales, grad_rotations,
                grad_cov3Ds_precomp, None)


class GaussianRasterizer(nn.Module):
    def __init__(self, raster_settings: GaussianRasterizationSettings):
        super().__init__()
        self.raster_settings = raster_settings

    def markVisible(self, positions: torch.Tensor) -> torch.Tensor:
        with torch.no_grad():
            raster_settings = self.raster_settings
            visible = _C.mark_visible(positions, raster_settings.viewmatrix, raster_settings.projmatrix)
        return visible

    def forward(self, means3D, means2D, opacities, normal, albedo, roughness, metallic, shs=None,
                colors_precomp=None, scales=None, rotations=None, cov3D_precomp=None, derive_normal=True):
        raster_settings = self.raster_settings

        if (shs is None and colors_precomp is None) or (shs is not None and colors_precomp is not None):
            raise Exception("Please provide excatly one of either SHs or precomputed colors!")

        if ((scales is None or rotations is None) and cov3D_precomp is None) or (
            (scales is not None or rotations is not None) and cov3D_precomp is not None
        ):
            raise Exception(
                "Please provide exactly one of either scale/rotation pair or precomputed 3D covariance!"
            )

        if shs is None:
            shs = torch.Tensor([])
        if colors_precomp is None:
            colors_precomp = torch.Tensor([])
        if scales is None:
            scales = torch.Tensor([])
        if rotations is None:
            rotations = torch.Tensor([])
        if cov3D_precomp is None:
            cov3D_precomp = torch.Tensor([])

        pre = ()
        if _st.after_blend is None and gigs_lib.prefetchers and means3D.is_cuda and not torch.cuda.is_current_stream_capturing():
            pre = [x for x in list(gigs_lib.prefetchers) if x.wants_prefetch()]
        if pre:
            pre = [x for x in pre if x.base.device == means3D.device]
        if pre:
            if _st.prefetch_events is None:
                _st.prefetch_events = {}
            if means3D.device not in _st.prefetch_events:
                _st.prefetch_events[means3D.device] = (torch.cuda.Event(), torch.cuda.Event())
            step_ev, blend_ev = _st.prefetch_events[means3D.device]
            step_ev.record(torch.cuda.current_stream(means3D.device))
            lib_scope = gigs_lib.use(gigs_lib.current().derive(blend_event=blend_ev))
        else:
            lib_scope = contextlib.nullcontext()
        with lib_scope:
            (color, radii, opacity_map, depth, out_normal, albedo_map, roughness_map, metallic_map,
             out_normal_view, _) = _RasterizeGaussians.apply(
                means3D, means2D, opacities, normal, albedo, roughness, metallic, shs, colors_precomp, scales,
                rotations, cov3D_precomp, raster_settings)
        for x in pre:
            x.prefetch(step_ev, blend_ev)
        if _st.after_blend is not None:
            _st.after_blend()

        focal_x = raster_settings.image_width / (2.0 * raster_settings.tanfovx)
        focal_y = raster_settings.image_height / (2.0 * raster_settings.tanfovy)
        W_, H_ = int(raster_settings.image_width), int(raster_settings.image_height)
        if derive_normal and W_ > 1 and H_ > 1 and os.environ.get("GIGS_FUSED_DERIVE", "1") == "1":
            normal_from_depth, depth_pos_filter = _derive_normal(W_, H_, focal_x, focal_y, raster_settings.viewmatrix,
                                                                 depth.detach())
        else:
            if derive_normal:
                depth_filter = filters.median_blur(depth.detach()[None, ...], (3, 3))[0]
                normal_from_depth, depth_pos = _C.depth_to_normal(
                    raster_settings.image_width, raster_settings.image_height, focal_x, focal_y,
                    raster_settings.viewmatrix, depth_filter)
            else:
                normal_from_depth = torch.zeros_like(out_normal)
                depth_pos = torch.zeros_like(out_normal)

            normal_from_depth = filters.bilateral_blur(normal_from_depth[None, ...], (3, 3), 1, (3, 3))[0]

            depth_pos_filter = filters.median_blur(depth_pos[None, ...], (3, 3))[0]
        occlusion = _C.SSAO(
            raster_settings.image_width, raster_settings.image_height, focal_x, focal_y,
            raster_settings.radius, raster_settings.bias, raster_settings.thick, raster_settings.delta,
            raster_settings.step, raster_settings.start, out_normal_view, depth_pos_filter)

        return (color, radii, opacity_map, depth, normal_from_depth, out_normal, occlusion, albedo_map,
                roughness_map, metallic_map, out_normal_view, depth_pos_filter)


def _derive_normal(width, height, focal_x, focal_y, viewmatrix, depth):
    _need_gpu(depth, "depth")
    d = depth.contiguous().float()
    dev = d.device
    normal = _new("normal_from_depth", (3, height, width), dev)
    pos = _new("depth_pos", (3, height, width), dev)
    vptr, vkeep = _fptr(viewmatrix, "viewmatrix")
    with torch.cuda.device(dev):
        gigs_lib.check(_lib.gigs_derive_normal(width, height, float(focal_x), float(focal_y), vptr, d.data_ptr(), 1.0, 3.0, 3.0,
                                               normal.data_ptr(), pos.data_ptr(), _stream()), "derive_normal")
    return normal, pos


class _SSR(torch.autograd.Function):
    @staticmethod
    def forward(ctx, image_width, image_height, focal_x, focal_y, radius, bias, thick, delta, step, start,
                normal, pos, rgb, albedo, roughness, metallic, F0):
        (color, abd) = _C.SSR(image_width, image_height, focal_x, focal_y, radius, bias, thick, delta, step,
                              start, normal, pos, rgb, albedo, roughness, metallic, F0)
        ctx.save_for_backward(roughness, metallic, abd)
        ctx.set_materialize_grads(False)
        return (color, abd)

    @staticmethod
    def backward(ctx, grad_out_color, grad_abd=None):
        roughness, metallic, abd = ctx.saved_tensors
        if grad_out_color is None:
            grad_albedo = torch.zeros_like(abd)
        else:
            g = grad_out_color.contiguous().float()
            grad_albedo = torch.empty_like(abd)
            with torch.cuda.device(abd.device):
                gigs_lib.check(_lib.gigs_ssr_backward(int(abd.shape[2]), int(abd.shape[1]), g.data_ptr(), abd.data_ptr(),
                                                      grad_albedo.data_ptr(), _stream()), "SSR backward")
        grad_roughness = torch.zeros_like(roughness)
        grad_metallic = torch.zeros_like(metallic)
        return (None, None, None, None, None, None, None, None, None, None, None, None, None,
                grad_albedo, grad_roughness, grad_metallic, None)


class Gaussian_SSR(nn.Module):
    def __init__(self, tanfovx, tanfovy, image_width, image_height, radius, bias, thick, delta, step, start):
        super().__init__()
# ... 19 lines not shown
```

### gi-gs_amd/gigs_lib.py

```python
from __future__ import annotations

import ctypes as C
import functools
import os
import threading

_HERE = os.path.dirname(os.path.abspath(__file__))
LIB_PATH = os.environ.get("GIGS_LIB", os.path.join(_HERE, "libgigs_hip.so"))

ALLOC_FN = C.CFUNCTYPE(C.c_void_p, C.c_size_t, C.c_void_p)

_f = C.c_void_p
_i = C.c_int
_fl = C.c_float

SIGNATURES = {
    "gigs_last_error": (C.c_char_p, []),
    "gigs_build_arch": (C.c_char_p, []),
    "gigs_required_geom": (C.c_size_t, [_i]),
    "gigs_required_image": (C.c_size_t, [_i, _i]),
    "gigs_required_binning": (C.c_size_t, [_i]),
    "gigs_forward": (_i, [C.c_void_p, ALLOC_FN, C.c_void_p, ALLOC_FN, C.c_void_p, ALLOC_FN, C.c_void_p,
                          _i, _i, _i, _f, _i, _i,
                          _f, _f, _f, _f, _f, _f, _f, _f,
# ... 80 lines not shown
    "gigs_cube_texture_bwd": (_i, [_i, _i, _f, _f, _f, _i, C.c_void_p]),
    "gigs_cube_taps": (_i, [_i, _i, _f, _f, _f, C.c_void_p]),
    "gigs_cube_texture_bwd_gather": (_i, [_i, _i, _i, _f, _f, _f, _i, _i, _f, _f, _f, C.c_void_p]),
    "gigs_latlong_to_cubemap": (_i, [_i, _i, _i, _i, _i, _f, _f, C.c_void_p]),
    "gigs_latlong_to_cubemap_rot": (_i, [_i, _i, _i, _i, _i, _f, _i, _f, _f, C.c_void_p]),
    "gigs_loss_scratch_floats": (C.c_size_t, [_i, _i, _i]),
    "gigs_l1_ssim_fwd": (_i, [_i, _i, _i, _f, _f, C.c_float, _f, _f, _f, _f, _f, C.c_void_p]),
    "gigs_l1_ssim_bwd": (_i, [_i, _i, _i, _f, _f, C.c_float, _f, _f, _f, _f, _f, C.c_void_p]),
    "gigs_image_metrics_scratch_bytes": (C.c_size_t, [_i, _i, _i]),
    "gigs_image_metrics": (_i, [_i, _i, _i, _f, _f, _f, _f, _f, _f, C.c_void_p]),
    "gigs_normal_angular_error": (_i, [_i, _i, _f, _f, _i, _f, _f, _f, C.c_void_p]),
    "gigs_lpips_vgg_weight_floats": (C.c_size_t, []),
    "gigs_lpips_vgg_pack": (_i, [C.POINTER(C.c_void_p), C.POINTER(C.c_void_p), C.POINTER(C.c_void_p), _f, C.c_void_p]),
    "gigs_lpips_vgg_scratch_bytes": (C.c_size_t, [_i, _i, _i]),
    "gigs_lpips_vgg": (_i, [_i, _i, _i, _f, _f, _i, _f, _f, _f, _f, C.POINTER(C.c_void_p), C.c_void_p]),
    "gigs_pack_images": (_i, [_i, _f, C.c_void_p]),
    "gigs_plane_minmax": (_i, [C.c_longlong, _f, _f, _f, C.c_void_p]),
    "gigs_png_filter": (_i, [_i, _f, C.c_void_p]),
    "gigs_tsdf_integrate": (_i, [C.c_void_p, _i, C.c_void_p, C.c_void_p]),
    "gigs_mesh_count": (_i, [C.c_void_p, _fl, _f, _f, C.c_void_p]),
    "gigs_mesh_write": (_i, [C.c_void_p, _fl, _f, _f, _i, _i, _f, _f, _f, _f, _f, _f, _f, C.c_void_p]),
    "gigs_tv_loss_fwd": (_i, [_i, _i, _i, _i, _f, _f, _f, _f, _f, C.c_void_p]),
    "gigs_tv_loss_bwd": (_i, [_i, _i, _i, _i, _f, _f, _f, _f, _f, C.c_void_p]),
    "gigs_masked_l1_fwd": (_i, [_i, _i, _i, _f, _f, _f, _f, _f, C.c_void_p]),
    "gigs_masked_l1_bwd": (_i, [_i, _i, _i, _f, _f, _f, _f, _f, _f, _f, C.c_void_p]),
    "gigs_adam_step": (_i, [_i, C.c_void_p, C.c_double, C.c_double, C.c_double, _i, C.c_void_p]),
    "gigs_adam_step_dyn": (_i, [_i, C.c_void_p, C.c_double, C.c_double, C.c_double, _i, _f, C.c_void_p]),
    "gigs_adam_scalars": (None, [C.c_double, _i, C.c_double, C.c_double, C.POINTER(C.c_float)]),
    "gigs_adam_step_watch": (_i, [_i, C.c_void_p, C.c_double, C.c_double, C.c_double, _i, _f, C.c_char_p, _f, C.c_void_p]),
    "gigs_adam_step_guarded": (_i, [_i, C.c_void_p, C.c_double, C.c_double, C.c_double, _i, _f, C.c_char_p, _f, _f, C.c_void_p]),
    "gigs_ctx_set_reuse_binning": (_i, [C.c_void_p, _i]),
    "gigs_ctx_set_materials_only": (_i, [C.c_void_p, C.c_void_p]),
    "gigs_ctx_set_split_sh": (_i, [C.c_void_p, C.c_void_p]),
    "gigs_activate_fwd": (_i, [_i, _i, C.c_void_p, C.c_void_p, C.c_void_p]),
    "gigs_activate_bwd": (_i, [_i, _i, C.c_void_p, C.c_void_p, C.c_void_p, C.c_void_p]),
    "gigs_densify_stats": (_i, [_i, _f, _f, _f, _f, _f, _f, _f, C.c_void_p]),
    "gigs_densify_stats_guarded": (_i, [_i, _f, _f, _f, _f, _f, _f, _f, _f, C.c_void_p]),
    "gigs_gather_rows": (_i, [_i, C.c_void_p, C.c_longlong, C.c_longlong, _f, _f, C.c_void_p]),
    "gigs_dist2_scratch_bytes": (C.c_size_t, [_i]),
    "gigs_dist2": (_i, [_i, _f, _f, _f, C.c_size_t, C.c_void_p]),
    "gigs_geom_offset": (C.c_longlong, [_i, _i]),
    "gigs_binning_offset": (C.c_longlong, [_i, _i]),
    "gigs_image_offset": (C.c_longlong, [_i, _i, _i]),
    "gigs_selftest_div2": (_i, [_i, _f, _f, _f, _f, _f, _f, C.c_void_p]),
    "gigs_selftest_round": (_i, [_f, C.c_void_p]),
    "gigs_ctx_set_blend_begin_event": (_i, [C.c_void_p, C.c_void_p]),
    "gigs_stream_delay": (_i, [C.c_uint, C.c_void_p]),
    "gigs_ctx_set_async_binning": (_i, [C.c_void_p, _i, C.c_void_p]),
    "gigs_ctx_create": (C.c_void_p, []),
    "gigs_ctx_destroy": (None, [C.c_void_p]),
    "gigs_ctx_get_options": (_i, [C.c_void_p, C.c_void_p]),
    "gigs_ctx_set_options": (_i, [C.c_void_p, C.c_void_p]),
    "gigs_profile_begin": (None, []),
    "gigs_profile_end": (_i, [C.POINTER(C.c_float), C.POINTER(C.c_int), _i]),
    "gigs_profile_stage_name": (C.c_char_p, [_i]),
}

class ShadeExt(C.Structure):
    _fields_ = [("planar", C.c_int), ("rough_scale", C.c_float), ("rough_bias", C.c_float),
                ("out_F0", C.c_void_p), ("out_linear", C.c_void_p), ("out_roughness", C.c_void_p),
                ("g_albedo_mul_a", C.c_void_p), ("g_albedo_mul_b", C.c_void_p),
                ("g_roughness_add", C.c_void_p), ("g_metallic_add", C.c_void_p),
                ("g_scale", C.c_void_p), ("lamb_mask", C.c_void_p), ("lamb_acc4", C.c_void_p)]


class Options(C.Structure):
# ... 84 lines not shown


def check(rc: int, what: str) -> int:
    if rc < 0:
        msg = lib().gigs_last_error().decode("utf-8", "replace")
        raise GigsError(f"{what} failed ({rc}): {msg}")
    return rc


class profile:

    def __enter__(self):
        lib().gigs_profile_begin()
        self.stages = {}
        return self

    def __exit__(self, *exc):
        n = 64
        ms = (C.c_float * n)()
        cnt = (C.c_int * n)()
        k = lib().gigs_profile_end(ms, cnt, n)
        for i in range(min(k, n)):
            if cnt[i]:
                self.stages[lib().gigs_profile_stage_name(i).decode()] = (float(ms[i]), int(cnt[i]))
        return False


class Context:

    _cache: dict = {}
    _lock = threading.Lock()

    def __init__(self, opts: tuple, async_capacity: int, async_counters, blend_event, reuse_binning: bool = False,
                 materials_only=None, sh_rest=None):
        l = lib()
        self.opts, self.async_capacity = tuple(opts), int(async_capacity)
        self.async_counters, self.blend_event = async_counters, blend_event
        self.reuse_binning = bool(reuse_binning)
        self.materials_only = materials_only
        self.sh_rest = sh_rest
        self.ptr = l.gigs_ctx_create()
        if not self.ptr:
            raise GigsError("gigs_ctx_create failed")
        o = Options()
        o.struct_bytes = C.sizeof(Options)
        for n, v in zip(OPTION_NAMES, self.opts):
            setattr(o, n, int(v))
        check(l.gigs_ctx_set_options(self.ptr, C.byref(o)), "gigs_ctx_set_options")
        if self.async_capacity > 0:
            check(l.gigs_ctx_set_async_binning(self.ptr, self.async_capacity,
                                               None if async_counters is None else async_counters.data_ptr()),
                  "gigs_ctx_set_async_binning")
        if blend_event is not None:
            check(l.gigs_ctx_set_blend_begin_event(self.ptr, blend_event.cuda_event), "gigs_ctx_set_blend_begin_event")
        if self.reuse_binning:
            check(l.gigs_ctx_set_reuse_binning(self.ptr, 1), "gigs_ctx_set_reuse_binning")
        if materials_only is not None:
            check(l.gigs_ctx_set_materials_only(self.ptr, materials_only.data_ptr()), "gigs_ctx_set_materials_only")
        if sh_rest is not None:
            check(l.gigs_ctx_set_split_sh(self.ptr, sh_rest.data_ptr()), "gigs_ctx_set_split_sh")

    def __del__(self):
        try:
            if self.ptr:
                lib().gigs_ctx_destroy(self.ptr)
                self.ptr = None
        except Exception:
            pass

    @classmethod
    def get(cls, opts: tuple, async_capacity: int = 0, async_counters=None, blend_event=None, reuse_binning=False,
            materials_only=None, sh_rest=None) -> "Context":
        key = (tuple(int(v) for v in opts), int(async_capacity),
               None if async_counters is None else async_counters.data_ptr(), None if blend_event is None else id(blend_event),
               bool(reuse_binning), None if materials_only is None else materials_only.data_ptr(),
               None if sh_rest is None else (sh_rest.data_ptr(), tuple(sh_rest.shape)))
        with cls._lock:
            c = cls._cache.get(key)
            if c is None:
                if len(cls._cache) > 512:
                    cls._cache.clear()
                c = cls._cache[key] = cls(key[0], async_capacity, async_counters, blend_event, reuse_binning, materials_only, sh_rest)
        return c

    @classmethod
    def release(cls, tensors) -> None:
        ids = {id(t) for t in tensors if t is not None}
        with cls._lock:
            for k in [k for k, c in cls._cache.items()
                      if any(id(t) in ids for t in (c.async_counters, c.materials_only, c.sh_rest) if t is not None)]:
                del cls._cache[k]

    def derive(self, async_binning=None, blend_event="keep", reuse_binning=None, materials_only="keep", sh_rest="keep",
               **options) -> "Context":
        opts = list(self.opts)
        for k, v in options.items():
            if k == "gi_march" and isinstance(v, str):
                if v not in _GI_MARCH_VALUES:
                    raise ValueError(f"gi_march {v!r}: one of {sorted(_GI_MARCH_VALUES)}")
                v = _GI_MARCH_VALUES[v]
            opts[OPTION_NAMES.index(k)] = int(v)
        cap, cnt = self.async_capacity, self.async_counters
        if async_binning is False:
            cap, cnt = 0, None
        elif async_binning is not None:
            cap, cnt = async_binning
        ev = self.blend_event if isinstance(blend_event, str) else blend_event
        mo = self.materials_only if isinstance(materials_only, str) else materials_only
        rest = self.sh_rest if isinstance(sh_rest, str) else sh_rest
        return Context.get(tuple(opts), cap, cnt, ev, self.reuse_binning if reuse_binning is None else reuse_binning, mo, rest)

    def option(self, name: str) -> int:
        return self.opts[OPTION_NAMES.index(name)]


_default_opts = None
_tls = threading.local()

import weakref

prefetchers = weakref.WeakSet()


def default_options() -> tuple:
    global _default_opts
    if _default_opts is None:
        o = Options()
        o.struct_bytes = C.sizeof(Options)
        check(lib().gigs_ctx_get_options(None, C.byref(o)), "gigs_ctx_get_options")
        _default_opts = tuple(getattr(o, n) for n in OPTION_NAMES)
    return _default_opts


def current() -> Context:
    c = getattr(_tls, "ctx", None)
    if c is None:
        c = _tls.ctx = Context.get(default_options())
    return c


def ctx_ptr():
    return current().ptr

# ... 35 lines not shown
```

### gi-gs_amd/pipeline.py

```python
from __future__ import annotations

import contextlib
import math
import os
import weakref
from typing import Dict, Optional

import torch
import torch.nn.functional as F

import gigs_lib

from diff_gaussian_rasterization import (AsyncBinning, BinningOverflow, GaussianRasterizationSettings, GaussianRasterizer,
                                         Gaussian_SSR, OutputPool, _C as _ops, after_blend, filters)


def linear_to_srgb(linear: torch.Tensor) -> torch.Tensor:
    eps = torch.finfo(torch.float32).eps
    srgb0 = 323 / 25 * linear
    srgb1 = (211 * torch.clamp(linear, min=eps) ** (5 / 12) - 11) / 200
    return torch.where(linear <= 0.0031308, srgb0, srgb1)


def srgb_to_linear(srgb: torch.Tensor) -> torch.Tensor:
# ... 14 lines not shown

def make_settings(cam: Dict, sh_degree: int, bg: torch.Tensor, gi: Dict, device, inference=False,
                  debug=False) -> GaussianRasterizationSettings:
    as_t = lambda a: a if isinstance(a, torch.Tensor) else torch.as_tensor(a, device=device)
    return GaussianRasterizationSettings(
        image_height=int(cam["image_height"]), image_width=int(cam["image_width"]), tanfovx=cam["tanfovx"],
        tanfovy=cam["tanfovy"], radius=gi["radius"], bias=gi["bias"], thick=gi["thick"], delta=gi["delta"],
        step=gi["step"], start=gi["start"], bg=bg, scale_modifier=1.0, viewmatrix=as_t(cam["viewmatrix"]),
        projmatrix=as_t(cam["projmatrix"]), sh_degree=sh_degree, campos=as_t(cam["campos"]), prefiltered=False,
        debug=debug, inference=inference, argmax_depth=False)


def _collect_idle():
    import gc
    torch.cuda.synchronize()
    gc.collect()
    torch.cuda.synchronize()


def graphed(callable_, sample_args):
    import gc
    _collect_idle()
    was_enabled = gc.isenabled()
    gc.disable()
    try:
        return torch.cuda.make_graphed_callables(callable_, sample_args, allow_unused_input=True)
    finally:
        if was_enabled:
            gc.enable()


def gbuffer_post(normal_map_from_depth: torch.Tensor, normal_map: torch.Tensor, out_normal_view: torch.Tensor,
                 viewmatrix: torch.Tensor, opacity_map: Optional[torch.Tensor] = None, pad_normal: bool = False):
    normal_from_depth_mask = (normal_map_from_depth != 0).all(0)
    normal_mask = (normal_map != 0).all(0, keepdim=True)
    if pad_normal:
        if opacity_map is None:
            raise ValueError("pad_normal=True needs the opacity map")
        opacity_map = torch.where(opacity_map < 0.004, torch.zeros_like(opacity_map), opacity_map)
        opacity_map = torch.where(opacity_map > 1.0 - 0.004, torch.ones_like(opacity_map), opacity_map)
        normal_bg = torch.tensor([0.0, 0.0, 1.0], device=normal_map.device)
        normal_map = normal_map * opacity_map + (1.0 - opacity_map) * normal_bg[:, None, None]
        mask_from_depth = (normal_map_from_depth == 0.0).all(0, keepdim=True).float()
        normal_map_from_depth = normal_map_from_depth * (1.0 - mask_from_depth) + mask_from_depth * normal_bg[:, None, None]
    normal_map_from_depth = torch.where(torch.norm(normal_map_from_depth, dim=0, keepdim=True) > 0,
                                        F.normalize(normal_map_from_depth, dim=0, p=2), normal_map_from_depth)
    normal_map = torch.where(torch.norm(normal_map, dim=0, keepdim=True) > 0, F.normalize(normal_map, dim=0, p=2),
                             normal_map)
    normal_map = filters.median_blur(normal_map[None, ...], (3, 3))[0]
    R = viewmatrix[:3, :3]
    normals_view = -(normal_map.permute(1, 2, 0) @ R).permute(2, 0, 1)
    out_normal_view = torch.where(torch.norm(out_normal_view, dim=0, keepdim=True) > 0,
                                  F.normalize(out_normal_view, dim=0, p=2), out_normal_view)
    out_normal_view = filters.median_blur(out_normal_view[None, ...], (3, 3))[0]
    if pad_normal:
        return normal_map_from_depth, normal_from_depth_mask, normals_view, normal_mask, out_normal_view, opacity_map
    return normal_map_from_depth, normal_from_depth_mask, normals_view, normal_mask, out_normal_view


class _GbufferPostFused(torch.autograd.Function):

    @staticmethod
    def forward(ctx, normal_map_from_depth, normal_map, out_normal_view, viewmatrix):
        import gigs_lib
        lib = gigs_lib.lib()
        if not normal_map.is_cuda:
            raise RuntimeError("gbuffer_post needs CUDA/HIP tensors: gigs-hip has no CPU path")
        f = lambda t: t.contiguous().float()
        nfd, nm, onv_in, vm = f(normal_map_from_depth), f(normal_map), f(out_normal_view), f(viewmatrix)
        _, H, W = nm.shape
        dev = nm.device
        new = lambda *s: torch.empty(s, dtype=torch.float32, device=dev)
        nfd_out, normals_view, onv = new(3, H, W), new(3, H, W), new(3, H, W)
        nfd_mask = torch.empty((H, W), dtype=torch.uint8, device=dev)
        mask = torch.empty((1, H, W), dtype=torch.uint8, device=dev)
        with torch.cuda.device(dev):
            s = torch.cuda.current_stream().cuda_stream
            gigs_lib.check(lib.gigs_normalize_mask(H, W, nfd.data_ptr(), nfd_out.data_ptr(), nfd_mask.data_ptr(), s),
                           "normalize_mask")
            gigs_lib.check(lib.gigs_gbuffer_post(H, W, nm.data_ptr(), onv_in.data_ptr(), vm.data_ptr(),
                                                 normals_view.data_ptr(), mask.data_ptr(), None, onv.data_ptr(), s),
                           "gbuffer_post")
        ctx.save_for_backward(nm, vm)
        ctx.set_materialize_grads(False)
        nfd_mask_b, mask_b = nfd_mask.bool(), mask.bool()
        ctx.mark_non_differentiable(nfd_out, nfd_mask_b, mask_b, onv)
        return nfd_out, nfd_mask_b, normals_view, mask_b, onv

    @staticmethod
    def backward(ctx, _g_nfd, _g_nfd_mask, g_normals_view, _g_mask, _g_onv):
        import gigs_lib
        lib = gigs_lib.lib()
        nm, vm = ctx.saved_tensors
        _, H, W = nm.shape
        if g_normals_view is None:
            return None, None, None, None
        g = g_normals_view.contiguous().float()
        scratch, g_nm = torch.empty_like(nm), torch.empty_like(nm)
        with torch.cuda.device(nm.device):
            gigs_lib.check(lib.gigs_gbuffer_post_bwd(H, W, nm.data_ptr(), vm.data_ptr(), g.data_ptr(), scratch.data_ptr(),
                                                     g_nm.data_ptr(), torch.cuda.current_stream().cuda_stream),
                           "gbuffer_post_bwd")
        return None, g_nm, None, None


def gbuffer_post_fused(normal_map_from_depth: torch.Tensor, normal_map: torch.Tensor, out_normal_view: torch.Tensor,
                       viewmatrix: torch.Tensor):
    return _GbufferPostFused.apply(normal_map_from_depth, normal_map, out_normal_view, viewmatrix)


def rasterize(cam: Dict, g: Dict[str, torch.Tensor], sh_degree: int, bg: torch.Tensor, gi: Dict,
              inference: bool = False, derive_normal: bool = True, debug=False, means2D: Optional[torch.Tensor] = None):
    means3D = g["means3D"]
    screenspace_points = means2D if means2D is not None else torch.zeros_like(means3D, requires_grad=True)
    st = make_settings(cam, sh_degree, bg, gi, means3D.device, inference=inference, debug=debug)
    out = GaussianRasterizer(st)(
        means3D=means3D, means2D=screenspace_points, opacities=g["opacities"], normal=g["normal"], shs=g["shs"],
        albedo=g["albedo"], roughness=g["roughness"], metallic=g["metallic"], scales=g["scales"],
        rotations=g["rotations"], derive_normal=derive_normal)
    return out, screenspace_points, st


def render(cam: Dict, g: Dict[str, torch.Tensor], sh_degree: int, bg: torch.Tensor, gi: Dict,
           inference: bool = False, derive_normal: bool = True, debug=False, fused_post: bool = False,
           pad_normal: bool = False) -> Dict[str, torch.Tensor]:
    ((rendered_image, radii, opacity_map, depth_map, normal_map_from_depth, normal_map, occlusion_map, albedo_map,
      roughness_map, metallic_map, out_normal_view, depth_pos), screenspace_points, st) = rasterize(
        cam, g, sh_degree, bg, gi, inference=inference, derive_normal=derive_normal, debug=debug)
    if pad_normal:
        (normal_map_from_depth, normal_from_depth_mask, normals_view, normal_mask, out_normal_view, opacity_map) = gbuffer_post(
            normal_map_from_depth, normal_map, out_normal_view, st.viewmatrix, opacity_map=opacity_map, pad_normal=True)
    else:
        (normal_map_from_depth, normal_from_depth_mask, normals_view, normal_mask, out_normal_view) = (
            gbuffer_post_fused if fused_post else gbuffer_post)(normal_map_from_depth, normal_map, out_normal_view, st.viewmatrix)
    return {
        "render": rendered_image, "viewspace_points": screenspace_points, "visibility_filter": radii > 0,
        "radii": radii, "opacity_map": opacity_map, "depth_map": depth_map,
        "normal_map_from_depth": normal_map_from_depth, "normal_from_depth_mask": normal_from_depth_mask,
        "normal_map": normals_view, "normal_mask": normal_mask, "albedo_map": albedo_map,
        "roughness_map": roughness_map, "metallic_map": metallic_map, "occlusion_map": occlusion_map,
        "out_normal_view": out_normal_view, "depth_pos": depth_pos,
    }


RASTER_KEYS = ("means3D", "opacities", "normal", "albedo", "roughness", "metallic", "shs", "scales", "rotations")


class DenseScene(RuntimeError):
    """Raised by the graph-capturing steppers only under long_lists = 0 (gigs_options; GIGS_LONG_LISTS=0) for a scene that averages more instances per
    tile than one workgroup sorts in LDS: the caller then keeps the synchronous path.  By default dense scenes (3 M
    Gaussians at the Mip-NeRF360 images_4 sizes: 7 000 instances per tile) are NOT declined: the library partitions
    their long tile lists by sampled splitters (csrc/binning.hip) and they take the asynchronous, captured path."""
# ... 457 lines not shown
    def __init__(self, light, brdf_lut: torch.Tensor, metallic: bool = True, indirect: bool = True,
                 tone: bool = False, gamma: bool = False):
        super().__init__()
        self.light = light
        self.register_buffer("brdf_lut", brdf_lut, persistent=False)
        self.metallic, self.indirect, self.tone, self.gamma = metallic, indirect, tone, gamma

    def forward(self, normal_map_from_depth, normal_map_raw, out_normal_view_raw, albedo_map, roughness_raw,
                metallic_map, occlusion_map, viewmatrix, view_dirs):
        from pbr import pbr_shading
        (_, _, normals_view, normal_mask, out_normal_view) = gbuffer_post(
            normal_map_from_depth, normal_map_raw, out_normal_view_raw, viewmatrix)
        roughness_map = roughness_raw * (1.0 - 0.04) + 0.04
        occlusion = (occlusion_map if self.indirect else torch.ones_like(roughness_map)).permute(1, 2, 0)
        self.light.build_mips()
        pbr_result = pbr_shading(light=self.light, normals=normals_view.permute(1, 2, 0).detach(), view_dirs=view_dirs,
                                 mask=normal_mask.permute(1, 2, 0), albedo=albedo_map.permute(1, 2, 0),
                                 roughness=roughness_map.permute(1, 2, 0),
                                 metallic=metallic_map.permute(1, 2, 0) if self.metallic else None, tone=self.tone,
                                 gamma=self.gamma, occlusion=occlusion.detach(), brdf_lut=self.brdf_lut)
        render_direct = pbr_result["render_rgb"].permute(2, 0, 1)
        render_direct = torch.where(normal_mask, render_direct, torch.zeros_like(render_direct))
        if self.metallic:
            F0 = (1.0 - metallic_map) * 0.04 + albedo_map * metallic_map
            metallic_out = metallic_map
        else:
            F0 = torch.ones_like(albedo_map) * 0.04
            metallic_out = torch.zeros_like(roughness_map)
        linear_rgb = srgb_to_linear(render_direct).detach()
        return (render_direct, roughness_map, metallic_out, F0, linear_rgb, out_normal_view.detach(),
                normal_mask.to(roughness_map.dtype))


def stage2_loss(render_direct, IRR_linear, gt_image, normal_mask_f, roughness_map, metallic_map):
    IRR = linear_to_srgb(IRR_linear)
    IRR = filters.median_blur(IRR[None, ...], (3, 3))[0]
    render_rgb = render_direct + IRR
    loss = torch.abs(render_rgb - gt_image).mean()
    cnt = normal_mask_f.sum()
    lamb_loss = ((1.0 - roughness_map) * normal_mask_f).sum() / cnt + (metallic_map * normal_mask_f).sum() / cnt
    return loss + lamb_loss * 0.001, render_rgb.detach()


class _Stepper:

    def __init__(self):
        self.whole, self._wholes = None, {}
        self._dense = False

    def _graph_step(self, cam, raw, gt_image, view_dirs, update=True):
        if os.environ.get("GIGS_STEP_GRAPH", "1") != "1" or self._dense:
            return None
        try:
            return self._replay_whole(cam, raw, gt_image, view_dirs, update=update)
        except DenseScene:
            self._dense = True
            for w in self._wholes.values():
                w.close()
            self.whole = None
            self._wholes.clear()
            return None

    def _replay_whole(self, cam, raw, gt_image, view_dirs, update=True):
        cfg = camera_model(cam)
        if self.whole is None or self.whole.cfg != cfg:
            self.whole = self._wholes.get(cfg)
# ... 23 lines not shown
        if not self.optimizers:
            return
        if self.before_update is not None:
            self.before_update()
        for o in self.optimizers:
            o.step()
        for leaf in self._leaves(raw):
            leaf.grad = None
        if self.post_update is not None:
            with torch.no_grad():
                self.post_update()

    def close(self) -> None:
        for w in list(self._wholes.values()):
            w.close()
        if self.whole is not None:
            self.whole.close()
        if torch.cuda.is_available():
            torch.cuda.synchronize()

    def __enter__(self):
        return self

    def __exit__(self, *exc):
        self.close()
        return False


class Stage2Step(_Stepper):

    def __init__(self, light, brdf_lut, gi: Dict, sh_degree: int, metallic: bool = True, indirect: bool = True,
                 gamma: bool = False, tone: bool = False, graphs: bool = False, fused: bool = False,
                 prepare=None, regularizer=None, optimizers=None, post_update=None, before_update=None,
                 geometry_cache: bool = False, materials_only: bool = False):
        super().__init__()
        self.prepare, self.regularizer, self.optimizers = prepare, regularizer, list(optimizers or [])
        self.post_update, self.before_update = post_update, before_update
        self.gi, self.sh_degree, self.metallic = gi, sh_degree, metallic
        self.fused, self.light, self.brdf_lut = fused, light, brdf_lut
        self.flags = dict(metallic=metallic, indirect=indirect, gamma=gamma, tone=tone)
        self.back = self.mips = self.side = self.blend_begin = None
        self.lights_ready = self.raster_done = None
        self.pool = OutputPool() if (fused and graphs) else None
        self._abin = None
        self.front = Stage2Front(light, brdf_lut, metallic=metallic, indirect=indirect, tone=tone, gamma=gamma)
        self.loss_fn = stage2_loss
        self.graphs = graphs
        self._captured = False
        self._defer_backward = False
        self._static_bg = self._static_m2d = None
        self.geometry_cache, self.geom_cache = bool(geometry_cache), None
        self.materials_only = bool(materials_only)

    def _capture(self, front_args, loss_args):
        def clone(args):
            return tuple(a.detach().clone().requires_grad_(a.requires_grad) for a in args)
        self.front = graphed(self.front, clone(front_args))
        self.loss_fn = graphed(self.loss_fn, clone(loss_args))
        self._captured = True

    def _make_inner(self):
        return Stage2Step(self.light, self.brdf_lut, self.gi, self.sh_degree, graphs=False, fused=True,
                          regularizer=self.regularizer, **self.flags)

    def _leaves(self, g):
        out, seen = [], set()
        for t in list(g.values()) + list(self.light.parameters()):
            for leaf in _grad_leaves(t):
                if id(leaf) not in seen:
                    seen.add(id(leaf))
                    out.append(leaf)
        return out

    def __call__(self, cam: Dict, g: Dict[str, torch.Tensor], gt_image: torch.Tensor, view_dirs: torch.Tensor,
                 extra_loss=None, update: bool = True):
        raw = g
        if self.fused and self.graphs and extra_loss is None:
            out = self._graph_step(cam, raw, gt_image, view_dirs, update=update)
            if out is not None:
                return out
        regen = (lambda: self.prepare(raw)) if self.prepare is not None else None
        if regen is not None:
            g = regen()
        res = self._step(cam, g, gt_image, view_dirs, extra_loss, regen)
        if update:
            self._eager_update(raw)
        return res

    def _replay_whole(self, cam, raw, gt_image, view_dirs, update=True):
        if self.geometry_cache:
            if not update:
                raise ValueError("Stage2Step: update=False is not available with the frozen-geometry cache")
            return self._cached_geometry_step(cam, raw, gt_image, view_dirs)
        return super()._replay_whole(cam, raw, gt_image, view_dirs, update=update)

    def _cached_geometry_step(self, cam, raw, gt_image, view_dirs):
# ... 1 lines not shown
            self.geom_cache = GeometryCache(next(iter(raw.values())).device)
        cache = self.geom_cache
        cfg = camera_model(cam)
        vkey = cache.view_key(cam)
        mode = cache.mode(vkey, raw)
        for _ in range(3):
            key = (cfg, mode)
            whole = self._wholes.get(key)
            if whole is None:
                if len(self._wholes) >= 8:
                    return None
                whole = self._wholes[key] = WholeStepGraph(self, cam, raw, cache=cache, mode=mode)
            self.whole = whole
            out = whole(cam, raw, gt_image, view_dirs, vkey=vkey)
            if out is not None:
                return out
            mode = "record"
        raise RuntimeError("Stage2Step: the frozen-geometry step kept being invalidated")

    def _step(self, cam, g, gt_image, view_dirs, extra_loss=None, regen=None):
        dev = g["means3D"].device
        background = self._static_bg if self._static_bg is not None else torch.zeros(3, device=dev)
        if self.fused and self.blend_begin is None:
            self.blend_begin = torch.cuda.Event()
            self.blend_begin.record()
        lights = []
        hook = after_blend((lambda: lights.extend(self._fused_begin())) if self.fused else None)
        abin = self._eager_async(cam, g) if (self.fused and self.graphs and not self._dense) else None
        pre_grads = _snapshot_grads(self._leaves(g)) if abin is not None else None
        with hook, (abin if abin is not None else contextlib.nullcontext()):
            ev_ctx = (gigs_lib.use(gigs_lib.current().derive(blend_event=self.blend_begin)) if self.fused
                      else contextlib.nullcontext())
            with ev_ctx, (self.pool if self.pool is not None else contextlib.nullcontext()):
                out = rasterize(cam, g, self.sh_degree, background, self.gi, means2D=self._static_m2d)
        if abin is not None:
            abin.snapshot()
        ((_, radii, _, _, normal_map_from_depth, normal_map, occlusion_map, albedo_map, roughness_map, metallic_map,
          out_normal_view, depth_pos), screenspace_points, st) = out
        H, W = cam["image_height"], cam["image_width"]
        gi = self.gi
        if self.fused:
            res = self._fused_step(cam, gt_image, view_dirs, st, radii, screenspace_points, normal_map, out_normal_view,
                                   albedo_map, roughness_map, metallic_map, occlusion_map, depth_pos, lights,
                                   extra_loss)
            if abin is not None:
                try:
                    res["num_rendered"] = abin.check()
                except BinningOverflow as ex:
                    self._abin = AsyncBinning(grown_capacity(ex.needed), dev)
                    _restore_grads(pre_grads)
                    return self._step(cam, regen() if regen is not None else g, gt_image, view_dirs, extra_loss, regen)
            return res
        front_args = (normal_map_from_depth, normal_map, out_normal_view, albedo_map, roughness_map, metallic_map,
                      occlusion_map.detach(), st.viewmatrix, view_dirs)
        if self.graphs and not self._captured:
            with torch.no_grad():
                o = self.front(*front_args)
            la = (o[0].clone().requires_grad_(True), torch.zeros_like(o[0]).requires_grad_(True), gt_image,
                  o[6], o[1].clone().requires_grad_(True), o[2].clone().requires_grad_(True))
            self._capture(front_args, la)
        (render_direct, roughness_f, metallic_f, F0, linear_rgb, onv, normal_mask_f) = self.front(*front_args)
        ssr = Gaussian_SSR(cam["tanfovx"], cam["tanfovy"], W, H, gi["radius"], gi["bias"], gi["thick"], gi["delta"],
                           gi["step"], gi["start"])
        (IRR, _) = ssr(onv, depth_pos.detach(), linear_rgb, albedo_map, roughness_f, metallic_f, F0)
        loss, render_rgb = self.loss_fn(render_direct, IRR, gt_image, normal_mask_f, roughness_f, metallic_f)
        if extra_loss is not None:
            loss = loss + extra_loss(normal_map, albedo_map, roughness_map, metallic_map)
# ... 25 lines not shown
            self.dummy = torch.zeros(1, device=self.light.base.device)
            if self.graphs:
                with torch.no_grad():
                    self.mips(self.dummy)
                self.mips = graphed(self.mips, (self.dummy,))
        self.side.wait_event(self.blend_begin)
        import pbr.light as pbr_light
        with torch.cuda.stream(self.side), pbr_light.build_on_current_stream():
            out = self.mips(self.dummy)
            if self.lights_ready is None:
                self.lights_ready = torch.cuda.Event()
            self.lights_ready.record()
        return out

    def _fused_step(self, cam, gt_image, view_dirs, st, radii, screenspace_points, normal_map, out_normal_view,
                    albedo_map, roughness_map, metallic_map, occlusion_map, depth_pos, lights, extra_loss=None):
        from stage2_fused import Stage2FusedBack
        H, W = cam["image_height"], cam["image_width"]
        main = torch.cuda.current_stream()
        if self.regularizer is not None:
            if self.raster_done is None:
                self.raster_done = torch.cuda.Event()
            self.raster_done.record()
        if self.lights_ready is not None:
            main.wait_event(self.lights_ready)
        else:
            main.wait_stream(self.side)
        for t in lights:
            t.record_stream(main)
        args = (normal_map.detach(), out_normal_view.detach(), albedo_map, roughness_map, metallic_map,
                occlusion_map.detach(), depth_pos.detach(), st.viewmatrix, view_dirs, gt_image, *lights)
        if self.back is None:
            cfg = dict(H=H, W=W, gi=self.gi, focal_x=W / (2.0 * cam["tanfovx"]), focal_y=H / (2.0 * cam["tanfovy"]),
                       **self.flags)
            self.back = Stage2FusedBack(self.brdf_lut, cfg)
            if self.graphs:
                pooled = set(t.untyped_storage().data_ptr() for t in self.pool.buffers.values()) if self.pool else set()
                pooled |= set(t.untyped_storage().data_ptr() for t in lights)
                sample = tuple(a.detach().requires_grad_(a.requires_grad) if a.untyped_storage().data_ptr() in pooled
                               else a.detach().clone().requires_grad_(a.requires_grad) for a in args)
                self.back = graphed(self.back, sample)
        loss, render_rgb, render_direct, IRR = self.back(*args)
        if extra_loss is not None:
            loss = loss + extra_loss(normal_map, albedo_map, roughness_map, metallic_map)
        if self.regularizer is not None:
            maps = dict(normal_map=normal_map, albedo_map=albedo_map, roughness_map=roughness_map, metallic_map=metallic_map,
                        gt_image=gt_image)
            self.side.wait_event(self.raster_done)
            with torch.cuda.stream(self.side):
                reg = self.regularizer(maps)
            for t in maps.values():
                t.record_stream(self.side)
            main.wait_stream(self.side)
            reg.record_stream(main)
            loss = loss + reg
        res = dict(loss=loss.detach(), render_rgb=render_rgb, render_direct=render_direct, IRR=IRR,
                   viewspace_points=screenspace_points, radii=radii)
        if self._defer_backward:
            res["_loss"] = loss
            return res
        loss.backward()
        return res

    def close(self) -> None:
        super().close()
        if self.geom_cache is not None:
            self.geom_cache.invalidate()
# ... 114 lines not shown
```

### gi-gs_amd/relight.py

```python
from __future__ import annotations

import ctypes as C
from typing import Dict, List, Optional, Sequence

import torch

import gigs_lib
import pipeline
from diff_gaussian_rasterization import Gaussian_SSR, _C as _ops, _gi_scratch, filters
from pbr import CubemapLight, get_brdf_lut, pbr_shading
from pbr.shade import _ptr_array

_lib = gigs_lib.lib()


def latlong_to_cubemap(latlong_map: torch.Tensor, res: List[int]) -> torch.Tensor:
    if not latlong_map.is_cuda:
        raise RuntimeError("latlong_map must be a CUDA/HIP tensor: gigs-hip has no CPU path")
    lat = latlong_map.contiguous().float()
    Hl, Wl, Cn = lat.shape
    cube = torch.empty((6, int(res[0]), int(res[1]), Cn), dtype=torch.float32, device=lat.device)
    with torch.cuda.device(lat.device):
        gigs_lib.check(_lib.gigs_latlong_to_cubemap(int(res[0]), int(res[1]), Hl, Wl, Cn, lat.data_ptr(), cube.data_ptr(),
                                                    torch.cuda.current_stream().cuda_stream), "latlong_to_cubemap")
    return cube


def make_light(hdri: torch.Tensor, res: int = 256) -> CubemapLight:
    light = CubemapLight(base_res=res, device=hdri.device)
    light.base.data = latlong_to_cubemap(hdri, [res, res])
    light.eval()
    return light


MAX_ROTATIONS = 1024


def rotation_about(axis: Sequence[float], angle: float) -> torch.Tensor:
    a = torch.as_tensor(axis, dtype=torch.float64).reshape(3)
    n = float(a.norm())
    if not n > 0.0:
        raise ValueError("rotation_about: the axis has no direction")
# ... 58 lines not shown
    faces = ((one, -gy, -gx), (-one, -gy, gx), (gx, one, gy), (gx, -one, -gy), (gx, -gy, one), (-gx, -gy, -one))
    return torch.stack([torch.stack(f, dim=-1) for f in faces])


@torch.no_grad()
def rotate_light(light: CubemapLight, rotations) -> List[CubemapLight]:
    from pbr.texture import cube_texture_precise
    base = light.base.detach()
    dirs = cube_texel_dirs(int(base.shape[1]), base.device)
    out = []
    for r in _rotations_f32(rotations, base.device):
        out.append(_light_of(cube_texture_precise(base, dirs @ r)))
    return out


class _ViewGraph:

    def _init_view(self, gi: Dict, sh_degree: int, metallic: bool, graphs: bool) -> None:
        self.gi, self.sh_degree, self.metallic = gi, sh_degree, bool(metallic)
        self.graphs = bool(graphs)
        self._graph = self._graph_key = self._bin = None
        self._capacity = 0
        self._scratch = {}

    def _buf(self, name, shape, dtype, dev):
        t = self._scratch.get(name)
        if t is None or tuple(t.shape) != tuple(shape) or t.device != dev:
            t = self._scratch[name] = torch.empty(shape, dtype=dtype, device=dev)
        return t

    def _gbuffer(self, cam, g):
        dev = g["means3D"].device
        background = torch.zeros(3, device=dev)
        (out, _, st) = pipeline.rasterize(cam, g, self.sh_degree, background, self.gi, inference=True, derive_normal=True)
        (_, radii, _, depth_map, _, normal_map, occlusion, albedo_map, roughness_map, metallic_map, out_normal_view,
         depth_pos) = out
        H, W = cam["image_height"], cam["image_width"]
        new = lambda name, *shape: self._buf(name, shape, torch.float32, dev)
        normals_view, onv = new("normals_view", 3, H, W), new("onv", 3, H, W)
        mask_u8 = self._buf("mask_u8", (H, W), torch.uint8, dev)
        mask_f = new("mask_f", 1, H, W)
        p = lambda t: None if t is None else t.data_ptr()
        vm = st.viewmatrix.contiguous().float()
        with torch.cuda.device(dev):
            s = torch.cuda.current_stream().cuda_stream
            gigs_lib.check(_lib.gigs_gbuffer_post(H, W, p(normal_map), p(out_normal_view), p(vm), p(normals_view), p(mask_u8),
                                                  p(mask_f), p(onv), s), "gbuffer_post")
            if self.metallic:
                F0 = torch.full_like(albedo_map, 0.04)
                metallic_in = torch.zeros_like(roughness_map)
            else:
                F0 = torch.addcmul(torch.full_like(albedo_map, (1.0 - float(self.metallic)) * 0.04), albedo_map, metallic_map)
                metallic_in = metallic_map
        return dict(radii=radii, depth_map=depth_map, occlusion=occlusion, albedo_map=albedo_map,
                    roughness_map=roughness_map, metallic_map=metallic_map, depth_pos=depth_pos, normals_view=normals_view,
                    onv=onv, mask_u8=mask_u8, mask_f=mask_f, F0=F0, metallic_in=metallic_in)

    def _replay(self, cam, g, inputs, core, names, key_extra=None, on_capture=None):
        from diff_gaussian_rasterization import AsyncBinning, BinningOverflow
        key = (pipeline.camera_model(cam), tuple(sorted((k, v.data_ptr()) for k, v in g.items())), key_extra)
        for _ in range(4):
            if self._graph is None or self._graph_key != key:
                if self._capacity <= 0:
                    self._capacity = pipeline.first_capacity(cam, g, self.sh_degree, inference=True)
                self._bin = AsyncBinning(self._capacity, g["means3D"].device)
                scalars = {k: v for k, v in cam.items() if not isinstance(v, torch.Tensor)}

# ... 110 lines not shown
                b["occlusion"], b["F0"], b["metallic_in"])
        if alpha_mask is not None:
            render_rgb = render_rgb * alpha_mask
        return dict(render_rgb=render_rgb, render_direct=render_direct, IRR=IRR, occlusion=b["occlusion"],
                    depth_map=b["depth_map"], normal_map=b["normals_view"], normal_mask=b["mask_u8"].bool()[None],
                    radii=b["radii"])

    def _shade_ssr(self, cam, view_dirs, normals_view, mask_u8, mask_f, onv, depth_pos, albedo_shade, albedo_map,
                   roughness_map, metallic_map, occlusion, F0, metallic_in, parts=False):
        dev = albedo_map.device
        gi = self.gi
        H, W = cam["image_height"], cam["image_width"]
        new = lambda name, *shape: self._buf(name, shape, torch.float32, dev)
        render_direct, linear_rgb = torch.empty((3, H, W), device=dev), new("linear_rgb", 3, H, W)
        render_rgb, acc, loss = torch.empty((3, H, W), device=dev), new("acc", 4 + 4 * 256), new("loss", 1)
        diffuse_rgb, specular_rgb = (torch.empty((3, H, W), device=dev) for _ in range(2)) if parts else (None, None)
        p = lambda t: None if t is None else t.data_ptr()
        light = self.light
        spec = [s.contiguous() for s in light.specular]
        spec_ptr = _ptr_array(spec)
        spec_res = (C.c_int * len(spec))(*[int(s.shape[1]) for s in spec])
        lut = self.brdf_lut
        ext = gigs_lib.ShadeExt(planar=1, rough_scale=1.0, rough_bias=0.0, out_linear=p(linear_rgb))
        vd = view_dirs.contiguous().float()
        with torch.cuda.device(dev):
            s = torch.cuda.current_stream().cuda_stream
            gigs_lib.check(_lib.gigs_shade_fwd_ex(
                gigs_lib.ctx_ptr(), H, W, p(normals_view), p(vd), p(albedo_shade), p(roughness_map), p(mask_u8), p(occlusion),
                p(metallic_map) if self.metallic else None, None, p(light.diffuse), int(light.diffuse.shape[1]), len(spec),
                spec_ptr, spec_res, p(lut), int(lut.shape[-2]), int(lut.shape[-3]), int(self.tone), int(self.gamma),
                p(render_direct), p(diffuse_rgb), p(specular_rgb), None, C.addressof(ext), s), "shade_fwd_ex")
            IRR, _ = _ops.SSR(W, H, W / (2.0 * cam["tanfovx"]), H / (2.0 * cam["tanfovy"]), gi["radius"], gi["bias"],
                              gi["thick"], gi["delta"], gi["step"], gi["start"], onv, depth_pos, linear_rgb, albedo_map,
                              roughness_map, metallic_in, F0)
            gigs_lib.check(_lib.gigs_stage2_loss_fwd(H, W, p(render_direct), p(IRR), p(render_direct), p(mask_f),
                                                     p(roughness_map), p(metallic_in), p(render_rgb), p(acc), p(loss), s),
                           "stage2_loss_fwd")
        if parts:
            return render_direct, IRR, render_rgb, diffuse_rgb, specular_rgb
        return render_direct, IRR, render_rgb


MAX_LIGHTS = 16
_MULTI_NAMES = ("render_rgb", "render_direct", "IRR", "occlusion", "depth_map", "normal_map", "normal_mask", "radii")


class MultiRelighter(_ViewGraph):

    def __init__(self, lights: Sequence[CubemapLight], gi: Dict, sh_degree: int, metallic: bool = False,
                 tone: bool = False, gamma: bool = False, graphs: bool = False, brdf_lut: Optional[torch.Tensor] = None):
        lights = list(lights)
        if not 1 <= len(lights) <= MAX_LIGHTS:
            raise ValueError(f"MultiRelighter: 1..{MAX_LIGHTS} lights, got {len(lights)}")
        _check_lights("MultiRelighter", lights)
        self.lights = lights
        self.tone, self.gamma = bool(tone), bool(gamma)
        self._init_view(gi, sh_degree, metallic, graphs)
        dev = lights[0].base.device
        self.brdf_lut = (brdf_lut if brdf_lut is not None else get_brdf_lut()).to(dev)
        _build_lights("MultiRelighter", lights)

    @torch.no_grad()
    def __call__(self, cam: Dict, g: Dict[str, torch.Tensor], view_dirs: torch.Tensor,
                 alpha_mask: Optional[torch.Tensor] = None, albedo_ratio: Optional[Sequence[float]] = None) -> Dict:
        if self.graphs:
            try:
                def core(c, vd):
# ... 266 lines not shown
```

### gi-gs_amd/stage2_fused.py

```python
from __future__ import annotations

import ctypes as C
from typing import Dict

import torch

import gigs_lib
from diff_gaussian_rasterization import _C as _ops
from pbr.shade import _ptr_array

_lib = gigs_lib.lib()


def _p(t):
    return None if t is None else t.data_ptr()


def _stream() -> int:
    return torch.cuda.current_stream().cuda_stream


class _Stage2Fused(torch.autograd.Function):

    @staticmethod
    def forward(ctx, cfg, normal_map, out_normal_view, albedo_map, roughness_map, metallic_map, occlusion_map,
                depth_pos, viewmatrix, view_dirs, gt_image, lut, diffuse, *specular):
        dev = albedo_map.device
        if not albedo_map.is_cuda:
            raise RuntimeError("stage2_fused needs CUDA/HIP tensors: gigs-hip has no CPU path")
        ctx.set_materialize_grads(False)
        H, W = int(cfg["H"]), int(cfg["W"])
        f = lambda t: None if t is None else t.contiguous().float()
        normal_map, out_normal_view, albedo_map = f(normal_map), f(out_normal_view), f(albedo_map)
        roughness_map, metallic_map, depth_pos = f(roughness_map), f(metallic_map), f(depth_pos)
        occlusion = f(occlusion_map) if cfg["indirect"] else None
        viewmatrix, view_dirs, gt_image, lut, diffuse = f(viewmatrix), f(view_dirs), f(gt_image), f(lut), f(diffuse)
        specular = [f(s) for s in specular]
        use_metallic = bool(cfg["metallic"])

        new = lambda *shape: torch.empty(shape, dtype=torch.float32, device=dev)
        normals_view, onv = new(3, H, W), new(3, H, W)
        mask_u8 = torch.empty((H, W), dtype=torch.uint8, device=dev)
        mask_f = new(1, H, W)
        render_direct, F0, linear_rgb, rough_f = new(3, H, W), new(3, H, W), new(3, H, W), new(1, H, W)
        render_rgb, acc4, loss = new(3, H, W), new(4 + 4 * 256), new(1)
        spec_ptr = _ptr_array(specular)
        spec_res = (C.c_int * len(specular))(*[int(s.shape[1]) for s in specular])
        ext = gigs_lib.ShadeExt(planar=1, rough_scale=1.0 - 0.04, rough_bias=0.04, out_F0=_p(F0), out_linear=_p(linear_rgb),
                                out_roughness=_p(rough_f))
        gi = cfg["gi"]
        with torch.cuda.device(dev):
            s = _stream()
            gigs_lib.check(_lib.gigs_gbuffer_post(H, W, _p(normal_map), _p(out_normal_view), _p(viewmatrix),
                                                  _p(normals_view), _p(mask_u8), _p(mask_f), _p(onv), s), "gbuffer_post")
            gigs_lib.check(_lib.gigs_shade_fwd_ex(
                gigs_lib.ctx_ptr(), H, W, _p(normals_view), _p(view_dirs), _p(albedo_map), _p(roughness_map), _p(mask_u8), _p(occlusion),
                _p(metallic_map) if use_metallic else None, None, _p(diffuse), int(diffuse.shape[1]), len(specular),
                spec_ptr, spec_res, _p(lut), int(lut.shape[-2]), int(lut.shape[-3]), int(bool(cfg["tone"])),
                int(bool(cfg["gamma"])), _p(render_direct), None, None, None, C.addressof(ext), s), "shade_fwd_ex")
            metallic_f = metallic_map if use_metallic else torch.zeros_like(rough_f)
            IRR, abd = _ops.SSR(W, H, cfg["focal_x"], cfg["focal_y"], gi["radius"], gi["bias"], gi["thick"], gi["delta"],
                                gi["step"], gi["start"], onv, depth_pos, linear_rgb, albedo_map, rough_f, metallic_f, F0)
            d_direct_u, d_irr_u = new(3, H, W), new(3, H, W)
            gigs_lib.check(_lib.gigs_stage2_loss_fwd_grad(H, W, _p(render_direct), _p(IRR), _p(gt_image), _p(mask_f),
                                                          _p(rough_f), _p(metallic_f), _p(render_rgb), _p(acc4), _p(loss),
                                                          _p(d_direct_u), _p(d_irr_u), s), "stage2_loss_fwd_grad")
        ctx.save_for_backward(normals_view, view_dirs, albedo_map, roughness_map, mask_u8, mask_f, occlusion,
                              metallic_map if use_metallic else None, lut, diffuse, d_direct_u, d_irr_u, abd,
                              acc4, *specular)
        ctx.cfg = cfg
        ctx.lib_ctx = gigs_lib.current()
        ctx.need_light = (ctx.needs_input_grad[12], [ctx.needs_input_grad[13 + i] for i in range(len(specular))])
        loss = loss.reshape(())
        ctx.mark_non_differentiable(render_rgb, render_direct, IRR)
        return loss, render_rgb, render_direct, IRR

    @staticmethod
    @gigs_lib.with_forward_context
    def backward(ctx, g_loss, *_unused):
        (normals_view, view_dirs, albedo_map, roughness_map, mask_u8, mask_f, occlusion, metallic_map, lut, diffuse,
         d_direct_u, d_irr_u, abd, acc4, *specular) = ctx.saved_tensors
        cfg = ctx.cfg
        dev = albedo_map.device
        H, W = int(cfg["H"]), int(cfg["W"])
        new = lambda *shape: torch.empty(shape, dtype=torch.float32, device=dev)
        if g_loss is None:
            g_loss = torch.zeros((), dtype=torch.float32, device=dev)
        g_loss = g_loss.contiguous().float()
        d_albedo, d_rough = new(3, H, W), new(1, H, W)
        d_metal = new(1, H, W) if metallic_map is not None else None
        need_d, need_s = ctx.need_light
        sizes = [diffuse.numel() if need_d else 0] + [s.numel() if n else 0 for s, n in zip(specular, need_s)]
        slab = torch.zeros(sum(sizes), dtype=torch.float32, device=dev)
        views, off = [], 0
        for n, ref in zip(sizes, [diffuse] + list(specular)):
# ... 41 lines not shown
```

### include/gigs_hip.h

```cpp
#ifndef GIGS_HIP_H_
#define GIGS_HIP_H_

#include <stddef.h>
#include <stdint.h>

#ifdef __cplusplus
extern "C" {
#endif

#define GIGS_OK 0
#define GIGS_ERR_INVALID (-1)
#define GIGS_ERR_HIP (-2)
#define GIGS_ERR_ALLOC (-3)

typedef char* (*gigs_alloc_fn)(size_t nbytes, void* user);

const char* gigs_last_error(void);
const char* gigs_build_arch(void);

typedef struct gigs_ctx gigs_ctx;
typedef struct gigs_options {
  int struct_bytes;
  int binning_legacy;
  int bucket_max_mean;
// ... 338 lines not shown
int gigs_densify_stats_guarded(int P, const float* viewspace_grad, const int* radii, float* xyz_gradient_accum,
                               float* xyz_gradient_accum_abs, float* xyz_gradient_accum_abs_max, float* denom,
                               float* max_radii2D, const int* skip, void* stream);
int gigs_gather_rows(int n_tensors, const gigs_gather_tensor* tensors, long long n_rows_out, long long n_rows_in,
                     const int* src_index, const uint8_t* zero_row, void* stream);

size_t gigs_dist2_scratch_bytes(int P);
int gigs_dist2(int P, const float* points, float* mean_dists, void* scratch, size_t scratch_bytes, void* stream);

long long gigs_geom_offset(int P, int which);
long long gigs_binning_offset(int num_rendered, int which);
long long gigs_image_offset(int width, int height, int which);

int gigs_selftest_div2(int n, const float* nx, const float* ny, const float* d, float* out_fast,
                       float* out_ref, int* out_round, void* stream);
int gigs_selftest_round(unsigned long long* mismatches, void* stream);

int gigs_lite_forward(gigs_ctx* ctx, gigs_alloc_fn geometryBuffer, void* geom_user, gigs_alloc_fn binningBuffer, void* binning_user,
                      gigs_alloc_fn imageBuffer, void* image_user, int P, int D, int M, const float* background, int width,
                      int height, const float* means3D, const float* shs, const float* colors_precomp, const float* opacities,
                      const float* scales, float scale_modifier, const float* rotations, const float* cov3D_precomp,
                      const float* viewmatrix, const float* projmatrix, const float* cam_pos, float tan_fovx, float tan_fovy,
                      int prefiltered, int argmax_depth, float* out_color, float* out_opacity, float* out_depth, int* radii,
                      int debug, void* stream);

int gigs_ssr_backward(int width, int height, const float* grad_color, const float* abd, float* grad_albedo, void* stream);

int gigs_ctx_set_reuse_binning(gigs_ctx* ctx, int on);

int gigs_ctx_set_materials_only(gigs_ctx* ctx, void* violations);

int gigs_ctx_set_split_sh(gigs_ctx* ctx, const float* sh_rest);

int gigs_ctx_set_blend_begin_event(gigs_ctx* ctx, void* hip_event);

int gigs_stream_delay(unsigned nanoseconds, void* stream);

int gigs_ctx_set_async_binning(gigs_ctx* ctx, int r_capacity, unsigned* device_counters);

void gigs_profile_begin(void);
int gigs_profile_end(float* total_ms, int* launches, int n);
const char* gigs_profile_stage_name(int stage);

#ifdef __cplusplus
}
#endif
#endif
```

Baseline: 353.9 renders/s.

## Skip unused colour output, depth-normal derivation and repeated GI cert table build

Adds a lean mode, on by default in the stage-2 step, that drops work whose results are never read in the training step. The blend kernel skips writing the colour and opacity planes. Depth-to-normal derivation runs a template variant that computes only the filtered positions, with a smaller halo. The SSR minmax certificate table is built once and reused across SSR calls on the same depth via gi_table_for and a ctx flag, instead of being rebuilt each call. The risk is a stale certificate table if the reuse key misses a depth change, and colour or opacity gradients are now rejected in that mode.

```diff
diff --git a/gi-gs_amd/csrc/api.hip b/gi-gs_amd/csrc/api.hip
--- a/gi-gs_amd/csrc/api.hip
+++ b/gi-gs_amd/csrc/api.hip
@@ -166,7 +166,7 @@
   return o;
 }
 const Ctx& default_ctx() {
-  static const Ctx c = {default_options(), 0u, nullptr, nullptr, 0, nullptr, nullptr};
+  static const Ctx c = {default_options(), 0u, nullptr, nullptr, 0, nullptr, nullptr, 0, 0};
   return c;
 }
 }
@@ -280,6 +280,28 @@
   if (!ctx) return fail(GIGS_ERR_INVALID, "gigs_ctx_set_materials_only: the default context is immutable, create one");
   reinterpret_cast<gigs::Ctx*>(ctx)->materials_only = reinterpret_cast<unsigned*>(violations);
   return 0;
+}
+int gigs_ctx_set_gi_table_current(gigs_ctx* ctx, int on) {
+  if (!ctx) return fail(GIGS_ERR_INVALID, "gigs_ctx_set_gi_table_current: the default context is immutable, create one");
+  reinterpret_cast<gigs::Ctx*>(ctx)->gi_table_current = on != 0;
+  return 0;
+}
+int gigs_ctx_set_color_unread(gigs_ctx* ctx, int on) {
+  if (!ctx) return fail(GIGS_ERR_INVALID, "gigs_ctx_set_color_unread: the default context is immutable, create one");
+  reinterpret_cast<gigs::Ctx*>(ctx)->color_unread = on != 0;
+  return 0;
+}
+int gigs_stream_capture_id(void* stream, unsigned long long* id) {
+  if (!id) return fail(GIGS_ERR_INVALID, "gigs_stream_capture_id: null output");
+  hipStreamCaptureStatus status = hipStreamCaptureStatusNone;
+  unsigned long long cid = 0;
+  const hipError_t e = hipStreamGetCaptureInfo((hipStream_t)stream, &status, &cid);
+  if (e != hipSuccess) {
+    (void)hipGetLastError();
+    return fail(GIGS_ERR_HIP, "hipStreamGetCaptureInfo failed: %s", hipGetErrorString(e));
+  }
+  *id = status == hipStreamCaptureStatusNone ? 0ull : cid;
+  return status == hipStreamCaptureStatusNone ? 0 : 1;
 }
 int gigs_ctx_set_blend_begin_event(gigs_ctx* ctx, void* hip_event) {
   if (!ctx) return fail(GIGS_ERR_INVALID, "gigs_ctx_set_blend_begin_event: the default context is immutable, create one");
@@ -378,6 +400,8 @@
   a.viewmatrix = viewmatrix; a.projmatrix = projmatrix; a.cam_pos = cam_pos; a.background = background;
   a.argmax_depth = argmax_depth; a.inference = inference;
   a.shs_rest = (shs && !colors_precomp && M > 1) ? cx.sh_rest : nullptr;
+  a.color_unread = cx.color_unread;
+  if (a.color_unread) out_color = out_opacity = nullptr;
 
   const size_t scan_sz = scan_size_cached(P);
   const size_t geom_bytes = gigs::required_bytes<gigs::GeomState>((size_t)P, scan_sz);
@@ -518,6 +542,7 @@
   if (P == 0) return 0;
   if (!geometryBuffer || !binningBuffer || !imageBuffer) return fail(GIGS_ERR_INVALID, "null allocation callback");
   if (!out_color || !out_opacity || !out_depth) return fail(GIGS_ERR_INVALID, "null output");
+  if (ctx_of(ctx).color_unread) return fail(GIGS_ERR_INVALID, "lite_forward returns the colour: not with gigs_ctx_set_color_unread");
   const size_t N = (size_t)width * height;
   const size_t geom_bytes = gigs_required_geom(P), img_bytes = gigs_required_image(width, height);
   const size_t geom_extra = 8 * (size_t)P * sizeof(float) + gigs::kAlign, img_extra = 14 * N * sizeof(float) + gigs::kAlign;
@@ -560,6 +585,8 @@
     return fail(GIGS_ERR_INVALID, "a split-SH forward (gigs_ctx_set_split_sh) has a materials-only backward only");
   if (!dL_dmean2D || !dL_dalbedo || !dL_droughness || !dL_dmetallic)
     return fail(GIGS_ERR_INVALID, "null gradient output");
+  if (ctx_of(ctx).color_unread && (dL_dpix || dL_dpix_opacity))
+    return fail(GIGS_ERR_INVALID, "a colour-unread forward (gigs_ctx_set_color_unread) has no colour or opacity gradient to take");
   if (!materials_only && (!dL_dopacity || !dL_dnormal || !dL_dcolor || !dL_dmean3D || !dL_dcov3D || !dL_dscale || !dL_drot ||
                           (shs && !dL_dsh)))
     return fail(GIGS_ERR_INVALID, "null gradient output");
@@ -629,7 +656,7 @@
 int gigs_derive_normal(int width, int height, float focal_x, float focal_y, const float* viewmatrix, const float* depth,
                        float sigma_color, float sigma_x, float sigma_y, float* normal_from_depth, float* depth_pos_filter,
                        void* stream) {
-  if (width <= 1 || height <= 1 || !viewmatrix || !depth || !normal_from_depth || !depth_pos_filter)
+  if (width <= 1 || height <= 1 || !viewmatrix || !depth || !depth_pos_filter)
     return fail(GIGS_ERR_INVALID, "derive_normal: bad argument (images must be larger than 1x1)");
   StageScope sc(kDepthToNormal, (hipStream_t)stream);
   gigs::launch_derive_normal_fused(width, height, focal_x, focal_y, viewmatrix, sigma_color, sigma_x, sigma_y, depth,
@@ -673,7 +700,7 @@
   StageScope sc(kSsr, (hipStream_t)stream);
   const int rc = gigs::launch_ssr(ctx_of(ctx).opt, width, height, focal_x, focal_y, radius, bias, thick, delta, step, start,
                                   normal_view, pos, rgb, albedo, roughness, metallic, F0, color, abd, scratch,
-                                  (hipStream_t)stream);
+                                  (hipStream_t)stream, 0, nullptr, nullptr, nullptr, 0, ctx_of(ctx).gi_table_current != 0);
   if (rc == -1) return fail(GIGS_ERR_INVALID, "delta=%g gives an unbounded or oversized ray set", (double)delta);
   if (rc) return fail(GIGS_ERR_HIP, "ray table upload failed");
   HIP_TRY(hipGetLastError());
@@ -692,7 +719,7 @@
   (void)roughness;
   const int rc = gigs::launch_ssr_multi(ctx_of(ctx).opt, n_lights, width, height, focal_x, focal_y, radius, bias, thick, delta,
                                         step, start, normal_view, pos, rgb, albedo, metallic, F0, color, abd, scratch,
-                                        (hipStream_t)stream);
+                                        (hipStream_t)stream, ctx_of(ctx).gi_table_current != 0);
   if (rc == -1) return fail(GIGS_ERR_INVALID, "delta=%g gives an unbounded or oversized ray set", (double)delta);
   if (rc) return fail(GIGS_ERR_HIP, "ray table upload failed");
   HIP_TRY(hipGetLastError());
@@ -711,7 +738,8 @@
   StageScope sc(kSsr, (hipStream_t)stream);
   const int rc = gigs::launch_ssr(ctx_of(ctx).opt, width, height, focal_x, focal_y, radius, bias, thick, delta, step, start,
                                   normal_view, pos, rgb, albedo, roughness, metallic, F0, color, abd, scratch,
-                                  (hipStream_t)stream, mode, counts, offsets, entries, capacity);
+                                  (hipStream_t)stream, mode, counts, offsets, entries, capacity,
+                                  ctx_of(ctx).gi_table_current != 0);
   if (rc == -1) return fail(GIGS_ERR_INVALID, "delta=%g gives an unbounded or oversized ray set", (double)delta);
   if (rc == -3) return fail(GIGS_ERR_INVALID, "ssr_hits: the hit list is recorded by the default march only (gi_march = proj, start < step)");
   if (rc) return fail(GIGS_ERR_HIP, "ray table upload failed");
diff --git a/gi-gs_amd/csrc/blend.hip b/gi-gs_amd/csrc/blend.hip
--- a/gi-gs_amd/csrc/blend.hip
+++ b/gi-gs_amd/csrc/blend.hip
@@ -313,9 +313,11 @@
     o.normal_view[pix_id] = nv.x;
     o.normal_view[HW + pix_id] = nv.y;
     o.normal_view[2 * HW + pix_id] = nv.z;
-    o.color[pix_id] = C0 + T * bg_color[0];
-    o.color[HW + pix_id] = C1 + T * bg_color[1];
-    o.color[2 * HW + pix_id] = C2 + T * bg_color[2];
+    if (o.color) {
+      o.color[pix_id] = C0 + T * bg_color[0];
+      o.color[HW + pix_id] = C1 + T * bg_color[1];
+      o.color[2 * HW + pix_id] = C2 + T * bg_color[2];
+    }
     o.normal[pix_id] = N0; o.normal[HW + pix_id] = N1; o.normal[2 * HW + pix_id] = N2;
     o.albedo[pix_id] = A0; o.albedo[HW + pix_id] = A1; o.albedo[2 * HW + pix_id] = A2;
     o.roughness[pix_id] = inference ? (Rr + T) : Rr;
@@ -331,7 +333,7 @@
       o.pos[HW + pix_id] = 0.0f;
       o.pos[2 * HW + pix_id] = 0.0f;
     }
-    o.opacity[pix_id] = O;
+    if (o.opacity) o.opacity[pix_id] = O;
   }
 }
 
diff --git a/gi-gs_amd/csrc/gi.hip b/gi-gs_amd/csrc/gi.hip
--- a/gi-gs_amd/csrc/gi.hip
+++ b/gi-gs_amd/csrc/gi.hip
@@ -1119,7 +1119,8 @@
   const int sh = cert_shift_for(W, H);
   return sh ? cert_table_bytes(W, H, sh) : 0;
 }
-static size_t prepare_cert(const Options& o, GiParams& p, int mode, const float* pos, void* scratch, hipStream_t s) {
+static size_t prepare_cert(const Options& o, GiParams& p, int mode, const float* pos, void* scratch, hipStream_t s,
+                           bool table_current = false) {
   p.cert_shift = p.cert_w = p.cert_h = 0;
   p.cert_d0 = cert_consts(p.bias, p.thick).d0;
   if (!scratch || mode != 4 || !o.gi_cert) return 0;
@@ -1128,8 +1129,9 @@
   p.cert_shift = sh;
   p.cert_w = (p.W + (1 << sh) - 1) >> sh;
   p.cert_h = (p.H + (1 << sh) - 1) >> sh;
-  hipLaunchKernelGGL(gi_minmax_kernel, dim3(p.cert_w + 1, p.cert_h + 1), dim3(64), 0, s, p.W, p.H, sh, p.cert_w, p.cert_h,
-                     cert_consts(p.bias, p.thick), pos + 2 * (size_t)p.H * p.W, (float2*)scratch);
+  if (!table_current)
+    hipLaunchKernelGGL(gi_minmax_kernel, dim3(p.cert_w + 1, p.cert_h + 1), dim3(64), 0, s, p.W, p.H, sh, p.cert_w, p.cert_h,
+                       cert_consts(p.bias, p.thick), pos + 2 * (size_t)p.H * p.W, (float2*)scratch);
   return cert_table_bytes(p.W, p.H, sh);
 }
 
@@ -1234,7 +1236,8 @@
                float delta, int step, int start, const float* normal, const float* pos,
                const float* rgb, const float* albedo, const float* ,
                const float* metallic, const float* F0, float* color, float* abd, void* scratch, hipStream_t s,
-               int hits_mode, unsigned* hit_counts, const unsigned* hit_offsets, void* hit_entries, unsigned hit_capacity) {
+               int hits_mode, unsigned* hit_counts, const unsigned* hit_offsets, void* hit_entries, unsigned hit_capacity,
+               bool table_current) {
   RayTable t;
   const int rc = get_ray_table(delta, s, t);
   if (rc) return rc;
@@ -1243,7 +1246,7 @@
   if (W >= (1 << 15) || H >= (1 << 15)) return -2;
   const dim3 grid = gi_grid(p);
   const int mode = gi_march_mode(o, step, start);
-  const size_t cert = (start < step) ? prepare_cert(o, p, mode, pos, scratch, s) : 0;
+  const size_t cert = (start < step) ? prepare_cert(o, p, mode, pos, scratch, s, table_current) : 0;
   const float2* tab = (const float2*)scratch;
   const SsrHits hits = {hit_counts, hit_offsets, (uint2*)hit_entries, hit_capacity};
   if (hits_mode != 0 && (mode != 4 || (hits_mode != 1 && hits_mode != 2) || !(start < step))) return -3;
@@ -1275,7 +1278,7 @@
 int launch_ssr_multi(const Options& o, int n_lights, int W, int H, float fx, float fy, float radius, float bias, float thick,
                      float delta, int step, int start, const float* normal, const float* pos, const float* rgb,
                      const float* albedo, const float* metallic, const float* F0, float* color, float* abd, void* scratch,
-                     hipStream_t s) {
+                     hipStream_t s, bool table_current) {
   RayTable t;
   const int rc = get_ray_table(delta, s, t);
   if (rc) return rc;
@@ -1284,7 +1287,7 @@
   if (W >= (1 << 15) || H >= (1 << 15)) return -2;
   const dim3 grid = gi_grid(p);
   const int mode = gi_march_mode(o, step, start);
-  const size_t cert = (start < step) ? prepare_cert(o, p, mode, pos, scratch, s) : 0;
+  const size_t cert = (start < step) ? prepare_cert(o, p, mode, pos, scratch, s, table_current) : 0;
   const float2* tab = (const float2*)scratch;
   const size_t plane = (size_t)3 * W * H;
   for (int l0 = 0; l0 < n_lights; l0 += kSsrMaxLights) {
@@ -1430,27 +1433,30 @@
 #endif
 constexpr int kDnW = 32, kDnH = GIGS_DN_H, kDnThreads = kDnW * kDnH;
 
+template <bool kNormal>
 __global__ void __launch_bounds__(kDnThreads)
 derive_normal_fused_kernel(int W, int H, float fx, float fy, const float* __restrict__ vm, BilatK kk,
                            const float* __restrict__ depth_raw, float* __restrict__ normal_out,
                            float* __restrict__ pos_filter_out) {
-  __shared__ float s_d[kDnH + 8][kDnW + 8];
-  __shared__ float s_f[kDnH + 6][kDnW + 6];
-  __shared__ float s_n[3][kDnH + 2][kDnW + 2];
+  constexpr int kHf = kNormal ? 3 : 1;
+  constexpr int kHd = kHf + 1;
+  __shared__ float s_d[kDnH + 2 * kHd][kDnW + 2 * kHd];
+  __shared__ float s_f[kDnH + 2 * kHf][kDnW + 2 * kHf];
+  __shared__ float s_n[kNormal ? 3 : 1][kNormal ? kDnH + 2 : 1][kNormal ? kDnW + 2 : 1];
   __shared__ float s_p[3][kDnH + 2][kDnW + 2];
   const int x0 = blockIdx.x * kDnW, y0 = blockIdx.y * kDnH;
   const size_t HW = (size_t)H * W;
 
-  for (int i = threadIdx.x; i < (kDnH + 8) * (kDnW + 8); i += kDnThreads) {
-    const int ty = i / (kDnW + 8), tx = i - ty * (kDnW + 8);
-    const int gx = x0 - 4 + tx, gy = y0 - 4 + ty;
+  for (int i = threadIdx.x; i < (kDnH + 2 * kHd) * (kDnW + 2 * kHd); i += kDnThreads) {
+    const int ty = i / (kDnW + 2 * kHd), tx = i - ty * (kDnW + 2 * kHd);
+    const int gx = x0 - kHd + tx, gy = y0 - kHd + ty;
     s_d[ty][tx] = (gx < 0 || gx >= W || gy < 0 || gy >= H) ? 0.0f : depth_raw[(size_t)gy * W + gx];
   }
   __syncthreads();
 
-  for (int i = threadIdx.x; i < (kDnH + 6) * (kDnW + 6); i += kDnThreads) {
-    const int ty = i / (kDnW + 6), tx = i - ty * (kDnW + 6);
-    const int gx = x0 - 3 + tx, gy = y0 - 3 + ty;
+  for (int i = threadIdx.x; i < (kDnH + 2 * kHf) * (kDnW + 2 * kHf); i += kDnThreads) {
+    const int ty = i / (kDnW + 2 * kHf), tx = i - ty * (kDnW + 2 * kHf);
+    const int gx = x0 - kHf + tx, gy = y0 - kHf + ty;
     float r = 0.0f;
     if (!(gx < 0 || gx >= W || gy < 0 || gy >= H)) {
       float v[9];
@@ -1475,11 +1481,12 @@
     const int x = x0 - 1 + tx, y = y0 - 1 + ty;
     v3 nrm = {0.0f, 0.0f, 0.0f}, pos = {0.0f, 0.0f, 0.0f};
     if (!(x < 0 || x >= W || y < 0 || y >= H) && !(x <= 0 || x >= W - 1 || y <= 0 || y >= H - 1)) {
-#define DP(dx, dy) s_f[ty + 2 + (dy)][tx + 2 + (dx)]
+#define DP(dx, dy) s_f[ty + kHf - 1 + (dy)][tx + kHf - 1 + (dx)]
       const float depth_thresh = 0.01f;
       const float depth = DP(0, 0);
       const float cx = float(W) / 2.0f, cy = float(H) / 2.0f;
       pos = get_position(x, y, cx, cy, fx, fy, depth);
+      if constexpr (kNormal) {
       bool ok = !(depth < depth_thresh);
       const int pad = 2;
       for (int dx = -pad; ok && dx < pad + 1; ++dx) {
@@ -1509,9 +1516,10 @@
         nrm = {vm[0] * normal.x + vm[1] * normal.y + vm[2] * normal.z, vm[4] * normal.x + vm[5] * normal.y + vm[6] * normal.z,
                vm[8] * normal.x + vm[9] * normal.y + vm[10] * normal.z};
       }
+      }
 #undef DP
     }
-    s_n[0][ty][tx] = nrm.x; s_n[1][ty][tx] = nrm.y; s_n[2][ty][tx] = nrm.z;
+    if constexpr (kNormal) { s_n[0][ty][tx] = nrm.x; s_n[1][ty][tx] = nrm.y; s_n[2][ty][tx] = nrm.z; }
     s_p[0][ty][tx] = pos.x; s_p[1][ty][tx] = pos.y; s_p[2][ty][tx] = pos.z;
   }
   __syncthreads();
@@ -1520,7 +1528,7 @@
   const int x = x0 + lx, y = y0 + ly;
   if (x >= W || y >= H) return;
   const size_t p = (size_t)y * W + x;
-  {
+  if constexpr (kNormal) {
     float ctr[3], num[3] = {0.0f, 0.0f, 0.0f};
 #pragma unroll
     for (int c = 0; c < 3; c++) ctr[c] = s_n[c][ly + 1][lx + 1];
@@ -1579,8 +1587,13 @@
   k1d(sy, kk.ky);
   k1d(sx, kk.kx);
   kk.color_scale = -0.5f / (sigma_color * sigma_color);
-  hipLaunchKernelGGL(derive_normal_fused_kernel, dim3((W + kDnW - 1) / kDnW, (H + kDnH - 1) / kDnH), dim3(kDnThreads), 0, s, W, H, fx,
-                     fy, viewmatrix, kk, depth_raw, normal_out, pos_filter_out);
+  const dim3 grid((W + kDnW - 1) / kDnW, (H + kDnH - 1) / kDnH);
+  if (normal_out)
+    hipLaunchKernelGGL(derive_normal_fused_kernel<true>, grid, dim3(kDnThreads), 0, s, W, H, fx, fy, viewmatrix, kk, depth_raw,
+                       normal_out, pos_filter_out);
+  else
+    hipLaunchKernelGGL(derive_normal_fused_kernel<false>, grid, dim3(kDnThreads), 0, s, W, H, fx, fy, viewmatrix, kk, depth_raw,
+                       normal_out, pos_filter_out);
 }
 
 __global__ void __launch_bounds__(256)
diff --git a/gi-gs_amd/csrc/gigs_common.h b/gi-gs_amd/csrc/gigs_common.h
--- a/gi-gs_amd/csrc/gigs_common.h
+++ b/gi-gs_amd/csrc/gigs_common.h
@@ -219,6 +219,8 @@
   int reuse_binning;
   unsigned* materials_only;
   const float* sh_rest;
+  int gi_table_current;
+  int color_unread;
 };
 const Options& default_options();
 const Ctx& default_ctx();
@@ -232,6 +234,7 @@
       *background;
   int argmax_depth, inference;
   const float* shs_rest;
+  int color_unread;
 };
 
 void launch_preprocess_fwd(const FwdArgs& a, const GeomState& g, int* radii, hipStream_t s);
@@ -287,11 +290,11 @@
                const float* rgb, const float* albedo, const float* roughness,
                const float* metallic, const float* F0, float* color, float* abd, void* scratch, hipStream_t s,
                int hits_mode = 0, unsigned* hit_counts = nullptr, const unsigned* hit_offsets = nullptr,
-               void* hit_entries = nullptr, unsigned hit_capacity = 0);
+               void* hit_entries = nullptr, unsigned hit_capacity = 0, bool table_current = false);
 int launch_ssr_multi(const Options& o, int n_lights, int W, int H, float fx, float fy, float radius, float bias, float thick,
                      float delta, int step, int start, const float* normal, const float* pos, const float* rgb,
                      const float* albedo, const float* metallic, const float* F0, float* color, float* abd, void* scratch,
-                     hipStream_t s);
+                     hipStream_t s, bool table_current = false);
 int launch_ssr_apply(int W, int H, float delta, const unsigned* offsets, const void* entries, const float* normal,
                      const float* pos, const float* rgb, const float* albedo, const float* metallic, const float* F0,
                      float* color, float* abd, hipStream_t s);
diff --git a/gi-gs_amd/csrc/preprocess.hip b/gi-gs_amd/csrc/preprocess.hip
--- a/gi-gs_amd/csrc/preprocess.hip
+++ b/gi-gs_amd/csrc/preprocess.hip
@@ -114,7 +114,7 @@
   extern __shared__ __align__(16) float sh_lds[];
   const int idx = blockIdx.x * kPreBlock + threadIdx.x;
   const int P = a.P;
-  const bool use_sh = (a.colors_precomp == nullptr);
+  const bool use_sh = (a.colors_precomp == nullptr) && !a.color_unread;
   if (use_sh) {
     const size_t first = (size_t)blockIdx.x * kPreBlock;
     const int nG = min(kPreBlock, P - (int)first);
@@ -217,6 +217,15 @@
     g.rgb[3 * (size_t)idx + 0] = col.x;
     g.rgb[3 * (size_t)idx + 1] = col.y;
     g.rgb[3 * (size_t)idx + 2] = col.z;
+  } else if (a.color_unread) {
+    col = {0.0f, 0.0f, 0.0f};
+    if (a.colors_precomp == nullptr) {
+#pragma unroll
+      for (int c = 0; c < 3; c++) {
+        g.clamped[3 * (size_t)idx + c] = 0;
+        g.rgb[3 * (size_t)idx + c] = 0.0f;
+      }
+    }
   } else {
     col = ld3(a.colors_precomp + 3 * (size_t)idx);
   }
@@ -243,7 +252,7 @@
 
 void launch_preprocess_fwd(const FwdArgs& a, const GeomState& g, int* radii, hipStream_t s) {
   const int blocks = (a.P + kPreBlock - 1) / kPreBlock;
-  const size_t lds = a.colors_precomp ? 0 : (size_t)kPreBlock * sh_stride(a.M) * sizeof(float);
+  const size_t lds = (a.colors_precomp || a.color_unread) ? 0 : (size_t)kPreBlock * sh_stride(a.M) * sizeof(float);
   hipLaunchKernelGGL(preprocess_fwd_kernel, dim3(blocks), dim3(kPreBlock), lds, s, a, g, radii);
 }
 
diff --git a/gi-gs_amd/diff_gaussian_rasterization/__init__.py b/gi-gs_amd/diff_gaussian_rasterization/__init__.py
--- a/gi-gs_amd/diff_gaussian_rasterization/__init__.py
+++ b/gi-gs_amd/diff_gaussian_rasterization/__init__.py
@@ -61,6 +61,7 @@
     grad_sink = None
     async_ = None
     view = None
+    gi_table = None
 
 
 _st = _Scopes()
@@ -434,6 +435,7 @@
 def _SSAO(width, height, focal_x, focal_y, radius, bias, thick, delta, step, start, out_normal, out_pos):
     _need_gpu(out_normal, "out_normal")
     dev = out_normal.device
+    _st.gi_table = None
     if _st.view is not None:
         slot, mode = _st.view
         if slot.occlusion is None or tuple(slot.occlusion.shape) != (1, height, width):
@@ -449,6 +451,9 @@
     ps, k1 = _fptr(out_pos, "out_pos")
     scratch = _gi_scratch(int(width), int(height), dev)
     with torch.cuda.device(dev):
+        if (scratch is not None and int(start) < int(step) and isinstance(out_pos, torch.Tensor) and ps == out_pos.data_ptr()
+                and tuple(out_pos.shape) == (3, int(height), int(width))):
+            _st.gi_table = _GiTable(scratch, out_pos, _gi_table_key(width, height, bias, thick, step, start, dev))
         gigs_lib.check(_lib.gigs_ssao_ex(gigs_lib.ctx_ptr(), int(width), int(height), float(focal_x), float(focal_y), float(radius),
                                          float(bias), float(thick), float(delta), int(step), int(start), n, ps,
                                          occlusion.data_ptr(), None if scratch is None else scratch.data_ptr(), _stream()),
@@ -456,13 +461,50 @@
     return occlusion
 
 
+class _GiTable:
+
+    def __init__(self, scratch, pos, key):
+        import weakref
+        self.scratch, self.pos, self.key = scratch, weakref.ref(pos), key
+        self.storage, self.offset, self.version = pos.untyped_storage().data_ptr(), pos.storage_offset(), pos._version
+
+
+def _capture_id():
+    cid = C.c_ulonglong(0)
+    if _lib.gigs_stream_capture_id(_stream(), C.byref(cid)) < 0:
+        return None
+    return int(cid.value)
+
+
+def _gi_table_key(width, height, bias, thick, step, start, dev):
+    cur = gigs_lib.current()
+    return (int(width), int(height), float(bias), float(thick), int(step), int(start), cur.option("gi_march"),
+            cur.option("gi_cert"), str(dev), _stream(), _capture_id())
+
+
+def gi_table_for(depth_pos: torch.Tensor, width, height, bias, thick, step, start):
+    rec = _st.gi_table
+    if rec is None or not isinstance(depth_pos, torch.Tensor) or not depth_pos.is_cuda:
+        return None
+    pos = rec.pos()
+    if (pos is None or depth_pos.dtype != torch.float32 or not depth_pos.is_contiguous()
+            or tuple(depth_pos.shape) != (3, int(height), int(width))
+            or depth_pos.untyped_storage().data_ptr() != rec.storage or depth_pos.storage_offset() != rec.offset
+            or pos.untyped_storage().data_ptr() != rec.storage or pos._version != rec.version
+            or depth_pos._version != rec.version):
+        return None
+    if rec.key[-1] is None or rec.key != _gi_table_key(width, height, bias, thick, step, start, depth_pos.device):
+        return None
+    return rec.scratch
+
+
 def _gi_scratch(width: int, height: int, dev):
     nbytes = int(_lib.gigs_gi_scratch_bytes(width, height))
     return torch.empty(nbytes, dtype=torch.uint8, device=dev) if nbytes else None
 
 
 def _SSR(width, height, focal_x, focal_y, radius, bias, thick, delta, step, start, out_normal, out_pos,
-         out_rgb, out_albedo, out_roughness, out_metallic, out_F0):
+         out_rgb, out_albedo, out_roughness, out_metallic, out_F0, table=None):
     _need_gpu(out_roughness, "out_roughness")
     dev = out_roughness.device
     color = torch.empty((3, height, width), dtype=torch.float32, device=dev)
@@ -474,13 +516,14 @@
         ptr, k = _fptr(t, name)
         ptrs.append(ptr)
         keep.append(k)
-    scratch = _gi_scratch(int(width), int(height), dev)
+    scratch = table if table is not None else _gi_scratch(int(width), int(height), dev)
     sp = None if scratch is None else scratch.data_ptr()
+    lib_scope = gigs_lib.use(gigs_lib.current().derive(gi_table_current=True)) if table is not None else contextlib.nullcontext()
     W, H = int(width), int(height)
     a = (W, H, float(focal_x), float(focal_y), float(radius), float(bias), float(thick), float(delta), int(step), int(start))
     hit_list = (_st.view is not None and gigs_lib.current().option("gi_march") == 4 and int(start) < int(step)
                 and os.environ.get("GIGS_SSR_HIT_LIST", "1") == "1")
-    with torch.cuda.device(dev):
+    with torch.cuda.device(dev), lib_scope:
         if hit_list and _st.view[1] == "replay" and _st.view[0].ssr_loaded:
             slot = _st.view[0]
             normal_p, pos_p, rgb_p, albedo_p, _rough_p, metallic_p, F0_p = ptrs
@@ -704,8 +747,12 @@
         return visible
 
     def forward(self, means3D, means2D, opacities, normal, albedo, roughness, metallic, shs=None,
-                colors_precomp=None, scales=None, rotations=None, cov3D_precomp=None, derive_normal=True):
+                colors_precomp=None, scales=None, rotations=None, cov3D_precomp=None, derive_normal=True,
+                color_unread=False):
         raster_settings = self.raster_settings
+        positions_only = isinstance(derive_normal, str)
+        if positions_only and derive_normal != "positions":
+            raise ValueError("derive_normal: True, False or 'positions'")
 
         if (shs is None and colors_precomp is None) or (shs is not None and colors_precomp is not None):
             raise Exception("Please provide excatly one of either SHs or precomputed colors!")
@@ -744,10 +791,11 @@
         else:
             lib_scope = contextlib.nullcontext()
         with lib_scope:
-            (color, radii, opacity_map, depth, out_normal, albedo_map, roughness_map, metallic_map,
-             out_normal_view, _) = _RasterizeGaussians.apply(
-                means3D, means2D, opacities, normal, albedo, roughness, metallic, shs, colors_precomp, scales,
-                rotations, cov3D_precomp, raster_settings)
+            with gigs_lib.use(gigs_lib.current().derive(color_unread=True)) if color_unread else contextlib.nullcontext():
+                (color, radii, opacity_map, depth, out_normal, albedo_map, roughness_map, metallic_map,
+                 out_normal_view, _) = _RasterizeGaussians.apply(
+                    means3D, means2D, opacities, normal, albedo, roughness, metallic, shs, colors_precomp, scales,
+                    rotations, cov3D_precomp, raster_settings)
         for x in pre:
             x.prefetch(step_ev, blend_ev)
         if _st.after_blend is not None:
@@ -758,7 +806,7 @@
         W_, H_ = int(raster_settings.image_width), int(raster_settings.image_height)
         if derive_normal and W_ > 1 and H_ > 1 and os.environ.get("GIGS_FUSED_DERIVE", "1") == "1":
             normal_from_depth, depth_pos_filter = _derive_normal(W_, H_, focal_x, focal_y, raster_settings.viewmatrix,
-                                                                 depth.detach())
+                                                                 depth.detach(), positions_only=positions_only)
         else:
             if derive_normal:
                 depth_filter = filters.median_blur(depth.detach()[None, ...], (3, 3))[0]
@@ -769,28 +817,34 @@
                 normal_from_depth = torch.zeros_like(out_normal)
                 depth_pos = torch.zeros_like(out_normal)
 
-            normal_from_depth = filters.bilateral_blur(normal_from_depth[None, ...], (3, 3), 1, (3, 3))[0]
+            if positions_only:
+                normal_from_depth = None
+            else:
+                normal_from_depth = filters.bilateral_blur(normal_from_depth[None, ...], (3, 3), 1, (3, 3))[0]
 
             depth_pos_filter = filters.median_blur(depth_pos[None, ...], (3, 3))[0]
         occlusion = _C.SSAO(
             raster_settings.image_width, raster_settings.image_height, focal_x, focal_y,
             raster_settings.radius, raster_settings.bias, raster_settings.thick, raster_settings.delta,
             raster_settings.step, raster_settings.start, out_normal_view, depth_pos_filter)
+        if color_unread:
+            color = opacity_map = None
 
         return (color, radii, opacity_map, depth, normal_from_depth, out_normal, occlusion, albedo_map,
                 roughness_map, metallic_map, out_normal_view, depth_pos_filter)
 
 
-def _derive_normal(width, height, focal_x, focal_y, viewmatrix, depth):
+def _derive_normal(width, height, focal_x, focal_y, viewmatrix, depth, positions_only=False):
     _need_gpu(depth, "depth")
     d = depth.contiguous().float()
     dev = d.device
-    normal = _new("normal_from_depth", (3, height, width), dev)
+    normal = None if positions_only else _new("normal_from_depth", (3, height, width), dev)
     pos = _new("depth_pos", (3, height, width), dev)
     vptr, vkeep = _fptr(viewmatrix, "viewmatrix")
     with torch.cuda.device(dev):
         gigs_lib.check(_lib.gigs_derive_normal(width, height, float(focal_x), float(focal_y), vptr, d.data_ptr(), 1.0, 3.0, 3.0,
-                                               normal.data_ptr(), pos.data_ptr(), _stream()), "derive_normal")
+                                               None if normal is None else normal.data_ptr(), pos.data_ptr(), _stream()),
+                       "derive_normal")
     return normal, pos
 
 
diff --git a/gi-gs_amd/gigs_lib.py b/gi-gs_amd/gigs_lib.py
--- a/gi-gs_amd/gigs_lib.py
+++ b/gi-gs_amd/gigs_lib.py
@@ -136,6 +136,9 @@
     "gigs_ctx_set_reuse_binning": (_i, [C.c_void_p, _i]),
     "gigs_ctx_set_materials_only": (_i, [C.c_void_p, C.c_void_p]),
     "gigs_ctx_set_split_sh": (_i, [C.c_void_p, C.c_void_p]),
+    "gigs_ctx_set_gi_table_current": (_i, [C.c_void_p, _i]),
+    "gigs_ctx_set_color_unread": (_i, [C.c_void_p, _i]),
+    "gigs_stream_capture_id": (_i, [C.c_void_p, C.POINTER(C.c_ulonglong)]),
     "gigs_activate_fwd": (_i, [_i, _i, C.c_void_p, C.c_void_p, C.c_void_p]),
     "gigs_activate_bwd": (_i, [_i, _i, C.c_void_p, C.c_void_p, C.c_void_p, C.c_void_p]),
     "gigs_densify_stats": (_i, [_i, _f, _f, _f, _f, _f, _f, _f, C.c_void_p]),
@@ -286,7 +289,7 @@
     _lock = threading.Lock()
 
     def __init__(self, opts: tuple, async_capacity: int, async_counters, blend_event, reuse_binning: bool = False,
-                 materials_only=None, sh_rest=None):
+                 materials_only=None, sh_rest=None, gi_table_current: bool = False, color_unread: bool = False):
         l = lib()
         self.opts, self.async_capacity = tuple(opts), int(async_capacity)
         self.async_counters, self.blend_event = async_counters, blend_event
@@ -313,6 +316,11 @@
             check(l.gigs_ctx_set_materials_only(self.ptr, materials_only.data_ptr()), "gigs_ctx_set_materials_only")
         if sh_rest is not None:
             check(l.gigs_ctx_set_split_sh(self.ptr, sh_rest.data_ptr()), "gigs_ctx_set_split_sh")
+        self.gi_table_current, self.color_unread = bool(gi_table_current), bool(color_unread)
+        if self.gi_table_current:
+            check(l.gigs_ctx_set_gi_table_current(self.ptr, 1), "gigs_ctx_set_gi_table_current")
+        if self.color_unread:
+            check(l.gigs_ctx_set_color_unread(self.ptr, 1), "gigs_ctx_set_color_unread")
 
     def __del__(self):
         try:
@@ -324,17 +332,19 @@
 
     @classmethod
     def get(cls, opts: tuple, async_capacity: int = 0, async_counters=None, blend_event=None, reuse_binning=False,
-            materials_only=None, sh_rest=None) -> "Context":
+            materials_only=None, sh_rest=None, gi_table_current=False, color_unread=False) -> "Context":
         key = (tuple(int(v) for v in opts), int(async_capacity),
                None if async_counters is None else async_counters.data_ptr(), None if blend_event is None else id(blend_event),
                bool(reuse_binning), None if materials_only is None else materials_only.data_ptr(),
-               None if sh_rest is None else (sh_rest.data_ptr(), tuple(sh_rest.shape)))
+               None if sh_rest is None else (sh_rest.data_ptr(), tuple(sh_rest.shape)), bool(gi_table_current),
+               bool(color_unread))
         with cls._lock:
             c = cls._cache.get(key)
             if c is None:
                 if len(cls._cache) > 512:
                     cls._cache.clear()
-                c = cls._cache[key] = cls(key[0], async_capacity, async_counters, blend_event, reuse_binning, materials_only, sh_rest)
+                c = cls._cache[key] = cls(key[0], async_capacity, async_counters, blend_event, reuse_binning, materials_only, sh_rest,
+                                          gi_table_current, color_unread)
         return c
 
     @classmethod
@@ -346,7 +356,7 @@
                 del cls._cache[k]
 
     def derive(self, async_binning=None, blend_event="keep", reuse_binning=None, materials_only="keep", sh_rest="keep",
-               **options) -> "Context":
+               gi_table_current=None, color_unread=None, **options) -> "Context":
         opts = list(self.opts)
         for k, v in options.items():
             if k == "gi_march" and isinstance(v, str):
@@ -362,7 +372,9 @@
         ev = self.blend_event if isinstance(blend_event, str) else blend_event
         mo = self.materials_only if isinstance(materials_only, str) else materials_only
         rest = self.sh_rest if isinstance(sh_rest, str) else sh_rest
-        return Context.get(tuple(opts), cap, cnt, ev, self.reuse_binning if reuse_binning is None else reuse_binning, mo, rest)
+        return Context.get(tuple(opts), cap, cnt, ev, self.reuse_binning if reuse_binning is None else reuse_binning, mo, rest,
+                           self.gi_table_current if gi_table_current is None else gi_table_current,
+                           self.color_unread if color_unread is None else color_unread)
 
     def option(self, name: str) -> int:
         return self.opts[OPTION_NAMES.index(name)]
diff --git a/gi-gs_amd/pipeline.py b/gi-gs_amd/pipeline.py
--- a/gi-gs_amd/pipeline.py
+++ b/gi-gs_amd/pipeline.py
@@ -70,9 +70,12 @@
 
 def gbuffer_post(normal_map_from_depth: torch.Tensor, normal_map: torch.Tensor, out_normal_view: torch.Tensor,
                  viewmatrix: torch.Tensor, opacity_map: Optional[torch.Tensor] = None, pad_normal: bool = False):
-    normal_from_depth_mask = (normal_map_from_depth != 0).all(0)
+    have_nfd = normal_map_from_depth is not None
+    normal_from_depth_mask = (normal_map_from_depth != 0).all(0) if have_nfd else None
     normal_mask = (normal_map != 0).all(0, keepdim=True)
     if pad_normal:
+        if not have_nfd:
+            raise ValueError("pad_normal=True needs the depth normal")
         if opacity_map is None:
             raise ValueError("pad_normal=True needs the opacity map")
         opacity_map = torch.where(opacity_map < 0.004, torch.zeros_like(opacity_map), opacity_map)
@@ -81,8 +84,9 @@
         normal_map = normal_map * opacity_map + (1.0 - opacity_map) * normal_bg[:, None, None]
         mask_from_depth = (normal_map_from_depth == 0.0).all(0, keepdim=True).float()
         normal_map_from_depth = normal_map_from_depth * (1.0 - mask_from_depth) + mask_from_depth * normal_bg[:, None, None]
-    normal_map_from_depth = torch.where(torch.norm(normal_map_from_depth, dim=0, keepdim=True) > 0,
-                                        F.normalize(normal_map_from_depth, dim=0, p=2), normal_map_from_depth)
+    if have_nfd:
+        normal_map_from_depth = torch.where(torch.norm(normal_map_from_depth, dim=0, keepdim=True) > 0,
+                                            F.normalize(normal_map_from_depth, dim=0, p=2), normal_map_from_depth)
     normal_map = torch.where(torch.norm(normal_map, dim=0, keepdim=True) > 0, F.normalize(normal_map, dim=0, p=2),
                              normal_map)
     normal_map = filters.median_blur(normal_map[None, ...], (3, 3))[0]
@@ -148,14 +152,15 @@
 
 
 def rasterize(cam: Dict, g: Dict[str, torch.Tensor], sh_degree: int, bg: torch.Tensor, gi: Dict,
-              inference: bool = False, derive_normal: bool = True, debug=False, means2D: Optional[torch.Tensor] = None):
+              inference: bool = False, derive_normal=True, debug=False, means2D: Optional[torch.Tensor] = None,
+              color_unread: bool = False):
     means3D = g["means3D"]
     screenspace_points = means2D if means2D is not None else torch.zeros_like(means3D, requires_grad=True)
     st = make_settings(cam, sh_degree, bg, gi, means3D.device, inference=inference, debug=debug)
     out = GaussianRasterizer(st)(
         means3D=means3D, means2D=screenspace_points, opacities=g["opacities"], normal=g["normal"], shs=g["shs"],
         albedo=g["albedo"], roughness=g["roughness"], metallic=g["metallic"], scales=g["scales"],
-        rotations=g["rotations"], derive_normal=derive_normal)
+        rotations=g["rotations"], derive_normal=derive_normal, color_unread=color_unread)
     return out, screenspace_points, st
 
 
@@ -679,6 +684,16 @@
                 normal_mask.to(roughness_map.dtype))
 
 
+class _FrontWithoutDepthNormal(torch.nn.Module):
+
+    def __init__(self, front: Stage2Front):
+        super().__init__()
+        self.front = front
+
+    def forward(self, *planes):
+        return self.front(None, *planes)
+
+
 def stage2_loss(render_direct, IRR_linear, gt_image, normal_mask_f, roughness_map, metallic_map):
     IRR = linear_to_srgb(IRR_linear)
     IRR = filters.median_blur(IRR[None, ...], (3, 3))[0]
@@ -768,7 +783,7 @@
     def __init__(self, light, brdf_lut, gi: Dict, sh_degree: int, metallic: bool = True, indirect: bool = True,
                  gamma: bool = False, tone: bool = False, graphs: bool = False, fused: bool = False,
                  prepare=None, regularizer=None, optimizers=None, post_update=None, before_update=None,
-                 geometry_cache: bool = False, materials_only: bool = False):
+                 geometry_cache: bool = False, materials_only: bool = False, lean: bool = True):
         super().__init__()
         self.prepare, self.regularizer, self.optimizers = prepare, regularizer, list(optimizers or [])
         self.post_update, self.before_update = post_update, before_update
@@ -787,17 +802,22 @@
         self._static_bg = self._static_m2d = None
         self.geometry_cache, self.geom_cache = bool(geometry_cache), None
         self.materials_only = bool(materials_only)
+        self.lean = bool(lean)
 
     def _capture(self, front_args, loss_args):
         def clone(args):
             return tuple(a.detach().clone().requires_grad_(a.requires_grad) for a in args)
-        self.front = graphed(self.front, clone(front_args))
+        if front_args[0] is None:
+            graphed_front = graphed(_FrontWithoutDepthNormal(self.front), clone(front_args[1:]))
+            self.front = lambda _nfd, *planes: graphed_front(*planes)
+        else:
+            self.front = graphed(self.front, clone(front_args))
         self.loss_fn = graphed(self.loss_fn, clone(loss_args))
         self._captured = True
 
     def _make_inner(self):
         return Stage2Step(self.light, self.brdf_lut, self.gi, self.sh_degree, graphs=False, fused=True,
-                          regularizer=self.regularizer, **self.flags)
+                          regularizer=self.regularizer, lean=self.lean, **self.flags)
 
     def _leaves(self, g):
         out, seen = [], set()
@@ -865,7 +885,8 @@
             ev_ctx = (gigs_lib.use(gigs_lib.current().derive(blend_event=self.blend_begin)) if self.fused
                       else contextlib.nullcontext())
             with ev_ctx, (self.pool if self.pool is not None else contextlib.nullcontext()):
-                out = rasterize(cam, g, self.sh_degree, background, self.gi, means2D=self._static_m2d)
+                out = rasterize(cam, g, self.sh_degree, background, self.gi, means2D=self._static_m2d,
+                                derive_normal="positions" if self.lean else True, color_unread=self.lean)
         if abin is not None:
             abin.snapshot()
         ((_, radii, _, _, normal_map_from_depth, normal_map, occlusion_map, albedo_map, roughness_map, metallic_map,
@@ -957,7 +978,7 @@
                 occlusion_map.detach(), depth_pos.detach(), st.viewmatrix, view_dirs, gt_image, *lights)
         if self.back is None:
             cfg = dict(H=H, W=W, gi=self.gi, focal_x=W / (2.0 * cam["tanfovx"]), focal_y=H / (2.0 * cam["tanfovy"]),
-                       **self.flags)
+                       reuse_gi_table=self.lean, **self.flags)
             self.back = Stage2FusedBack(self.brdf_lut, cfg)
             if self.graphs:
                 pooled = set(t.untyped_storage().data_ptr() for t in self.pool.buffers.values()) if self.pool else set()
diff --git a/gi-gs_amd/relight.py b/gi-gs_amd/relight.py
--- a/gi-gs_amd/relight.py
+++ b/gi-gs_amd/relight.py
@@ -7,7 +7,7 @@
 
 import gigs_lib
 import pipeline
-from diff_gaussian_rasterization import Gaussian_SSR, _C as _ops, _gi_scratch, filters
+from diff_gaussian_rasterization import Gaussian_SSR, _C as _ops, _gi_scratch, filters, gi_table_for
 from pbr import CubemapLight, get_brdf_lut, pbr_shading
 from pbr.shade import _ptr_array
 
@@ -132,7 +132,8 @@
     def _gbuffer(self, cam, g):
         dev = g["means3D"].device
         background = torch.zeros(3, device=dev)
-        (out, _, st) = pipeline.rasterize(cam, g, self.sh_degree, background, self.gi, inference=True, derive_normal=True)
+        (out, _, st) = pipeline.rasterize(cam, g, self.sh_degree, background, self.gi, inference=True, derive_normal="positions",
+                                          color_unread=True)
         (_, radii, _, depth_map, _, normal_map, occlusion, albedo_map, roughness_map, metallic_map, out_normal_view,
          depth_pos) = out
         H, W = cam["image_height"], cam["image_width"]
@@ -309,7 +310,8 @@
                 p(render_direct), p(diffuse_rgb), p(specular_rgb), None, C.addressof(ext), s), "shade_fwd_ex")
             IRR, _ = _ops.SSR(W, H, W / (2.0 * cam["tanfovx"]), H / (2.0 * cam["tanfovy"]), gi["radius"], gi["bias"],
                               gi["thick"], gi["delta"], gi["step"], gi["start"], onv, depth_pos, linear_rgb, albedo_map,
-                              roughness_map, metallic_in, F0)
+                              roughness_map, metallic_in, F0,
+                              table=gi_table_for(depth_pos, W, H, gi["bias"], gi["thick"], gi["step"], gi["start"]))
             gigs_lib.check(_lib.gigs_stage2_loss_fwd(H, W, p(render_direct), p(IRR), p(render_direct), p(mask_f),
                                                      p(roughness_map), p(metallic_in), p(render_rgb), p(acc), p(loss), s),
                            "stage2_loss_fwd")
diff --git a/gi-gs_amd/stage2_fused.py b/gi-gs_amd/stage2_fused.py
--- a/gi-gs_amd/stage2_fused.py
+++ b/gi-gs_amd/stage2_fused.py
@@ -6,7 +6,7 @@
 import torch
 
 import gigs_lib
-from diff_gaussian_rasterization import _C as _ops
+from diff_gaussian_rasterization import _C as _ops, gi_table_for
 from pbr.shade import _ptr_array
 
 _lib = gigs_lib.lib()
@@ -59,8 +59,11 @@
                 spec_ptr, spec_res, _p(lut), int(lut.shape[-2]), int(lut.shape[-3]), int(bool(cfg["tone"])),
                 int(bool(cfg["gamma"])), _p(render_direct), None, None, None, C.addressof(ext), s), "shade_fwd_ex")
             metallic_f = metallic_map if use_metallic else torch.zeros_like(rough_f)
+            table = (gi_table_for(depth_pos, W, H, gi["bias"], gi["thick"], gi["step"], gi["start"])
+                     if cfg.get("reuse_gi_table", True) else None)
             IRR, abd = _ops.SSR(W, H, cfg["focal_x"], cfg["focal_y"], gi["radius"], gi["bias"], gi["thick"], gi["delta"],
-                                gi["step"], gi["start"], onv, depth_pos, linear_rgb, albedo_map, rough_f, metallic_f, F0)
+                                gi["step"], gi["start"], onv, depth_pos, linear_rgb, albedo_map, rough_f, metallic_f, F0,
+                                table=table)
             d_direct_u, d_irr_u = new(3, H, W), new(3, H, W)
             gigs_lib.check(_lib.gigs_stage2_loss_fwd_grad(H, W, _p(render_direct), _p(IRR), _p(gt_image), _p(mask_f),
                                                           _p(rough_f), _p(metallic_f), _p(render_rgb), _p(acc4), _p(loss),
diff --git a/include/gigs_hip.h b/include/gigs_hip.h
--- a/include/gigs_hip.h
+++ b/include/gigs_hip.h
@@ -394,6 +394,11 @@
 
 int gigs_ctx_set_split_sh(gigs_ctx* ctx, const float* sh_rest);
 
+int gigs_ctx_set_gi_table_current(gigs_ctx* ctx, int on);
+int gigs_ctx_set_color_unread(gigs_ctx* ctx, int on);
+
+int gigs_stream_capture_id(void* stream, unsigned long long* id);
+
 int gigs_ctx_set_blend_begin_event(gigs_ctx* ctx, void* hip_event);
 
 int gigs_stream_delay(unsigned nanoseconds, void* stream);
```

Result: no change. 356.7 renders/s (median of 6 runs) (+0.8%).
